# wearepal/qBOLD-VI

Measured on AMD Instinct MI355X. Metric: voxel-ELBO evals/sec, higher is better.
Workload: dtype f32; 1 GPU; 1048576 synthetic voxels/GPU x 11 tau, S=32 likelihood draws, K=70 KL draws, encoder U=60, L=2 (optimal.yaml), fused qbold_vi_fwd, tissue integral: table; encoder arithmetic: operands split in two f16 halves, three MFMA passes (hi.hi, hi.lo, lo.hi), f32 accumulate: float32-grade (~22 significant bits), |x| < 65504; sampling, forward model and ELBO sums: f32; global_voxels=1048576, parallelism=voxel-shard x1, collective=none

## Files before the change

### include/qbold_hip.h

```cpp
#ifndef QBOLD_HIP_H
#define QBOLD_HIP_H

#include <stdint.h>

#ifdef __cplusplus
extern "C" {
#endif

#define QBOLD_MAX_T 64
#define QBOLD_ABI_VERSION 5

typedef enum {
    QBOLD_OK = 0,
    QBOLD_ERR_INVALID = -1,
    QBOLD_ERR_HIP = -2,
    QBOLD_ERR_UNSUPPORTED = -3,
    QBOLD_ERR_NO_DEVICE = -4
} qbold_status;

typedef struct {
    double gamma, b0, dchi, te, r2t, tr, ti, t1b, hct;
    double tau_start, tau_end, tau_step;
    int32_t full_model;
    int32_t include_blood;
// ... 73 lines not shown
#define QBOLD_KSEL_ALL (4 | 8 | 256 | 512 | 2048 | 4096 | 8192 | 16384 | 32768 | 65536 | 131072 | 262144 | 524288 | 1048576 | 2097152 | 4194304 | 8388608)
int qbold_ctx_set_kernel_selection(qbold_ctx* ctx, int mask);
int qbold_ctx_table_eval(const qbold_ctx* ctx, const float* host_x, float* host_F, float* host_dF,
                         int64_t n);

int qbold_signal_fwd(const qbold_ctx* ctx, const float* oef_dbv, float* signal, int64_t V,
                     void* stream);
int qbold_signal_fwd_ex(const qbold_ctx* ctx, const float* oef_dbv, const float* hct,
                        const float* alt_oef_dbv, const int32_t* from_index, float* signal, int64_t V,
                        void* stream);
int qbold_signal_bwd(const qbold_ctx* ctx, const float* oef_dbv, const float* grad_signal,
                     float* grad_oef_dbv, int64_t V, void* stream);

int64_t qbold_encoder_num_params(const qbold_encoder_shape* shape);
int64_t qbold_encoder_packed_floats(const qbold_encoder_shape* shape);
int qbold_encoder_pack(const qbold_ctx* ctx, const qbold_encoder_shape* shape,
                       const float* weights, float* packed, void* stream);
int qbold_encoder_fwd(const qbold_ctx* ctx, const qbold_encoder_shape* shape, const float* packed,
                      const float* x, float* out1, float* out2, float* sigma, int64_t N,
                      void* stream);

int64_t qbold_encoder_wide_packed_floats(const qbold_encoder_shape* shape);
int64_t qbold_encoder_wide_workspace_floats(const qbold_encoder_shape* shape, int64_t N);
int qbold_encoder_wide_pack(const qbold_ctx* ctx, const qbold_encoder_shape* shape, const float* weights,
                            float* packed, void* stream);
int qbold_encoder_wide_fwd(const qbold_ctx* ctx, const qbold_encoder_shape* shape, const float* packed,
                           const float* x, int stream_sel, float* workspace, float* out_q,
                           float* out_log_sigma, int64_t N, void* stream);

int64_t qbold_encoder_fused_packed_floats(const qbold_encoder_shape* shape);
int qbold_encoder_fused_pack(const qbold_ctx* ctx, const qbold_encoder_shape* shape, const float* weights,
                             float* packed, void* stream);
int qbold_encoder_fused_fwd(const qbold_ctx* ctx, const qbold_encoder_shape* shape, const float* packed,
                            const float* x, float* out_q, float* out_log_sigma, int64_t N, void* stream);

int qbold_reparam(const qbold_ctx* ctx, const float* q, const float* z, float* oef_dbv, int64_t N,
                  void* stream);
int qbold_logit_mvn_nlogp(const qbold_ctx* ctx, const float* y, const float* params, float* out,
                          int64_t N, void* stream);
int qbold_kl_mog(const qbold_ctx* ctx, const float* q, const float* comps, int M, const float* z, uint64_t seed,
                 int64_t voxel0, float* kl, int64_t N, void* stream);
int qbold_squared_whitened_residual(const float* obs, const float* mean, const float* oef_log_std,
                                    const float* dbv_log_std, const float* oef_dbv_cov, float* out, int64_t N,
                                    void* stream);
int qbold_posterior_moments(const qbold_ctx* ctx, const float* q, const float* z, int n_samples,
                            uint64_t seed, int64_t voxel0, float* means, float* vars, int64_t N,
                            void* stream);

int qbold_normalise(const qbold_ctx* ctx, const float* x, float* out, int64_t N, void* stream);

int qbold_wls_fit(const qbold_ctx* ctx, const float* signals, double tau_min, float* out, int64_t N,
                  void* stream);

typedef enum {
    QBOLD_TRANSFORM_STD = 0,
    QBOLD_TRANSFORM_OFFDIAG = 1,
    QBOLD_INV_TRANSFORM_STD = 2,
    QBOLD_FORWARD_TRANSFORM = 3,
    QBOLD_BACKWARDS_TRANSFORM = 4,
    QBOLD_BACKWARDS_TRANSFORM_LOGIT = 5,
    QBOLD_EXP = 6
} qbold_transform_op;
int qbold_transform(const qbold_ctx* ctx, int op, const float* in, float* out, int64_t n,
                    void* stream);

int qbold_nll_fwd(const qbold_ctx* ctx, const float* x, const float* mask, const float* pred,
                  const float* sigma, float* nll, int64_t N, int S, void* stream);

int qbold_kl_fwd(const qbold_ctx* ctx, const float* q, const float* prior, const float* zk, int K,
                 uint64_t seed, int64_t voxel0, float* kl, int64_t N, void* stream);
int qbold_kl_closed(const qbold_ctx* ctx, const float* q, const float* prior, float* kl, int64_t N,
                    void* stream);
int qbold_kl_diag(const qbold_ctx* ctx, const float* q, const float* prior, const float* mask, float* kl_v,
                  float* g_q, double* sums, void* workspace, int64_t N, void* stream);

int qbold_normals(const qbold_ctx* ctx, uint64_t seed, uint32_t stream_id, int64_t voxel0, int n,
                  float* z, int64_t N, void* stream);

int64_t qbold_noise_workspace_bytes(const qbold_ctx* ctx);
int qbold_signal_add_noise(const qbold_ctx* ctx, float* signal, const float* norm_snr_host,
                           float snr_lo, float snr_hi, uint64_t seed, int64_t voxel0,
                           void* workspace, int64_t V, void* stream);

int64_t qbold_elbo_workspace_bytes(const qbold_ctx* ctx);

int qbold_elbo_fwd(const qbold_ctx* ctx, const float* x, const float* mask, const float* q,
                   const float* prior, const float* sigma, const float* zs, const float* zk, int S,
                   int K, uint64_t seed, int64_t voxel0, float* nll_kl, double* sums,
                   void* workspace, int64_t N, void* stream);

int qbold_elbo_fwd_logsigma(const qbold_ctx* ctx, const float* x, const float* mask, const float* q,
                            const float* prior, const float* log_sigma, int S, int K, uint64_t seed, int64_t voxel0,
                            float* nll_kl, double* sums, void* workspace, int64_t N, void* stream);

int64_t qbold_vi_workspace_bytes(const qbold_ctx* ctx, const qbold_encoder_shape* shape, int64_t N);
int qbold_vi_fwd(const qbold_ctx* ctx, const qbold_encoder_shape* shape, const float* packed,
                 const float* x, const float* mask, const float* prior, int S, int K, uint64_t seed,
                 int64_t voxel0, float* q_out, float* nll_kl, double* sums, void* workspace,
                 int64_t N, void* stream);

#define QBOLD_IW_MAX_K (1 << 30)
int qbold_log_evidence_fwd(const qbold_ctx* ctx, const float* x, const float* mask, const float* q,
                           const float* prior, const float* sigma, const float* z, int K, uint64_t seed,
                           int64_t voxel0, float* out, float* is_means, double* sums, void* workspace,
                           int64_t N, void* stream);

int qbold_log_evidence_bwd(const qbold_ctx* ctx, const float* x, const float* mask, const float* q,
                           const float* prior, const float* log_sigma, const float* z, int K, uint64_t seed,
                           int64_t voxel0, float* g_q, float* g_log_sigma, float* out, double* sums,
                           void* workspace, int64_t N, void* stream);

int qbold_log_evidence_draws(const qbold_ctx* ctx, const float* x, const float* mask, const float* q,
                             const float* prior, const float* sigma, const float* z, int K, uint64_t seed,
                             int64_t voxel0, float* log_w, float* theta, int64_t N, void* stream);

#define QBOLD_PSIS_MIN_K 25
#define QBOLD_PSIS_MAX_K 1024
#define QBOLD_PSIS_MAX_C 8
int qbold_psis(const qbold_ctx* ctx, const float* log_w, const float* theta, int C, const float* mask, int K,
               float* out, float* means, float* weights, int64_t N, void* stream);

typedef struct {
    int optimizer;
    float lr, lr_final, beta1, beta2, eps;
} qbold_refine_cfg;
int qbold_refine_posterior(const qbold_ctx* ctx, const float* x, const float* mask, const float* q_in,
                           const float* prior, const float* sigma, const float* z, int steps, int S,
                           const qbold_refine_cfg* cfg, uint64_t seed, int64_t voxel0,
                           float* q_out, float* loss, int64_t N, void* stream);

int64_t qbold_refine_spatial_workspace_bytes(const qbold_ctx* ctx, const qbold_geometry* geom);
int qbold_refine_posterior_spatial(const qbold_ctx* ctx, const float* x, const float* mask, const float* q_in,
                                   const float* prior, const float* sigma, const float* z,
                                   const qbold_geometry* geom, float tv_weight, int steps, int S,
                                   const qbold_refine_cfg* cfg, uint64_t seed, int64_t voxel0,
                                   float* q_out, float* loss, void* workspace, void* stream);

typedef struct {
    int coarse, fine, locate, gh;
    float span, cut, level_lo, level_hi;
} qbold_grid_cfg;
#define QBOLD_GRID_OUT 17
int qbold_posterior_grid(const qbold_ctx* ctx, const float* x, const float* mask, const float* prior,
                         const float* sigma, const float* q, const qbold_grid_cfg* cfg, float* out, float* box,
                         double* sums, void* workspace, int64_t N, void* stream);

#define QBOLD_PPC_OUT 6
int qbold_posterior_predictive(const qbold_ctx* ctx, const float* x, const float* mask, const float* q,
                               const float* sigma, const float* z, int L, uint64_t seed, int64_t voxel0,
                               float* out, float* curves, double* sums, void* workspace, int64_t N, void* stream);

int qbold_elbo_bwd(const qbold_ctx* ctx, const float* x, const float* mask, const float* q,
                   const float* prior, const float* log_sigma, int S, int K, uint64_t seed,
                   int64_t voxel0, float* g_q, float* g_log_sigma, float* nll_kl, double* sums,
                   void* workspace, int64_t N, void* stream);

int64_t qbold_train_workspace_floats(const qbold_encoder_shape* shape, int64_t N);
int qbold_encoder_train_fwd(const qbold_ctx* ctx, const qbold_encoder_shape* shape, const float* weights,
                            const float* x, int stream_sel, float* workspace, float* out_q,
                            float* out_log_sigma, int64_t N, void* stream);
int qbold_encoder_train_fwd_fused(const qbold_ctx* ctx, const qbold_encoder_shape* shape, const float* packed,
                                  const float* x, int save_all, float* workspace, float* out_q,
                                  float* out_log_sigma, int64_t N, void* stream);
int qbold_encoder_train_bwd_recomputes(const qbold_ctx* ctx, const qbold_encoder_shape* shape, int64_t N);
int qbold_encoder_spatial_fwd(const qbold_ctx* ctx, const qbold_encoder_shape* shape, const float* weights,
                              const float* x, const qbold_geometry* geom, float* workspace, float* out_q,
// ... 26 lines not shown
```

### qbold_vi_amd/csrc/ctx.hip

```cpp
#include <math.h>
#include <stdlib.h>
#include <string.h>

#include <mutex>

#include "qbold_ctx.h"

namespace qb {
static thread_local std::string g_err;
void set_error(const std::string& msg) { g_err = msg; }
int hip_fail(hipError_t e, const char* what) {
    g_err = std::string(what) + ": " + hipGetErrorString(e);
    return QBOLD_ERR_HIP;
}
}

extern "C" int qbold_abi_version(void) { return QBOLD_ABI_VERSION; }
extern "C" const char* qbold_last_error(void) { return qb::g_err.c_str(); }

namespace {

struct Simpson {
    double u[QB_NNODE], w[QB_NNODE], pre[QB_NNODE];
    double h3;
// ... 154 lines not shown
        g[i] = simpson.dF(i * h) * h;
    }
    ctx->h_tab.resize(4 * QB_TAB_SEG);
    for (int i = 0; i < QB_TAB_SEG; ++i) {
        ctx->h_tab[4 * i + 0] = (float)f[i];
        ctx->h_tab[4 * i + 1] = (float)g[i];
        ctx->h_tab[4 * i + 2] = (float)(3.0 * (f[i + 1] - f[i]) - 2.0 * g[i] - g[i + 1]);
        ctx->h_tab[4 * i + 3] = (float)(2.0 * (f[i] - f[i + 1]) + g[i] + g[i + 1]);
    }

    {
        const int se = d.se_idx;
        const float tol = 4e-6f * fabsf(tstep);
        bool mirrors = se >= 0 && se < T && fabsf(d.taus[se]) <= tol;
        for (int j = 1; mirrors && se - j >= 0 && se + j < T; ++j) {
            const float ta = fabsf(d.taus[se - j]), tb = fabsf(d.taus[se + j]);
            const float ba = d.blood_B[se - j], bb = d.blood_B[se + j];
            mirrors = fabsf(ta - tb) <= tol && fabsf(ba - bb) <= 4e-6f * fmaxf(fabsf(ba), fabsf(bb));
        }
        ctx->grid_mirrors = mirrors;
    }

    {
        const int nseg = qb::gtab_segs(T), se = d.se_idx;
        const bool proto = (T == 11 && se == 2) || (T == 24 && se == 7) || (T == 64 && se == 12);
        if (nseg > 0 && proto && ctx->grid_mirrors && P->full_model) {
            const int J = qb::gtab_taus(T, se);
            ctx->h_gtab.resize((size_t)4 * J * nseg);
            const double hh = (double)QB_GT_OEF_RANGE / nseg;
            std::vector<double> gf(nseg + 1), gg(nseg + 1);
            for (int j = 1; j <= J; ++j) {
                const double tau = fabs((double)(se + j < T ? d.taus[se + j] : d.taus[se - j]));
                const double k = tau * (double)d.dw_coef;
                for (int i = 0; i <= nseg; ++i) {
                    const double oef = (double)QB_GT_OEF_MIN + hh * i;
                    gf[i] = simpson.F(k * oef);
                    gg[i] = simpson.dF(k * oef) * k * hh;
                }
                const double* cf[4] = {nullptr, nullptr, nullptr, nullptr};
                std::vector<double> c0(nseg), c1(nseg), c2(nseg), c3(nseg);
                for (int i = 0; i < nseg; ++i) {
                    c0[i] = gf[i];
                    c1[i] = gg[i];
                    c2[i] = 3.0 * (gf[i + 1] - gf[i]) - 2.0 * gg[i] - gg[i + 1];
                    c3[i] = 2.0 * (gf[i] - gf[i + 1]) + gg[i] + gg[i + 1];
                }
                cf[0] = c0.data(); cf[1] = c1.data(); cf[2] = c2.data(); cf[3] = c3.data();
                if (qb::gtab_paired(T, se)) {
                    const int p = (j - 1) / 2, m = (j - 1) & 1;
                    float* rowA = &ctx->h_gtab[(size_t)4 * (2 * p) * nseg];
                    float* rowB = &ctx->h_gtab[(size_t)4 * (2 * p + 1) * nseg];
                    for (int i = 0; i < nseg; ++i) {
                        rowA[4 * i + 0 + m] = (float)cf[0][i];
                        rowA[4 * i + 2 + m] = (float)cf[1][i];
                        rowB[4 * i + 0 + m] = (float)cf[2][i];
                        rowB[4 * i + 2 + m] = (float)cf[3][i];
                    }
                } else {
                    float* row = &ctx->h_gtab[(size_t)4 * (j - 1) * nseg];
                    for (int i = 0; i < nseg; ++i)
                        for (int q = 0; q < 4; ++q) row[4 * i + q] = (float)cf[q][i];
                }
            }
            ctx->gtab_ok = true;
        }
    }

    if (device < 0) {
        *out = ctx;
        return QBOLD_OK;
    }
    int prev_device = -1;
    (void)hipGetDevice(&prev_device);
    hipError_t e = hipSetDevice(device);
    if (e == hipSuccess) e = hipMalloc((void**)&ctx->d_tab, sizeof(float) * 4 * QB_TAB_SEG);
    if (e == hipSuccess)
        e = hipMemcpy(ctx->d_tab, ctx->h_tab.data(), sizeof(float) * 4 * QB_TAB_SEG,
                      hipMemcpyHostToDevice);
    if (e == hipSuccess && ctx->gtab_ok) {
        e = hipMalloc((void**)&ctx->d_gtab, sizeof(float) * ctx->h_gtab.size());
        if (e == hipSuccess)
            e = hipMemcpy(ctx->d_gtab, ctx->h_gtab.data(), sizeof(float) * ctx->h_gtab.size(), hipMemcpyHostToDevice);
    }
    if (e == hipSuccess) {
        hipDeviceProp_t prop;
        if (hipGetDeviceProperties(&prop, device) == hipSuccess && prop.multiProcessorCount > 0)
            ctx->num_cus = prop.multiProcessorCount;
    }
    if (prev_device >= 0 && prev_device != device) (void)hipSetDevice(prev_device);
    if (e != hipSuccess) {
        if (ctx->d_tab) (void)hipFree(ctx->d_tab);
        if (ctx->d_gtab) (void)hipFree(ctx->d_gtab);
        delete ctx;
        return qb::hip_fail(e, "qbold_ctx_create: device setup");
    }
    *out = ctx;
    return QBOLD_OK;
}

extern "C" void qbold_ctx_destroy(qbold_ctx* ctx) {
    if (!ctx) return;
    if (ctx->d_tab) (void)hipFree(ctx->d_tab);
    if (ctx->d_gtab) (void)hipFree(ctx->d_gtab);
    delete ctx;
}

extern "C" int qbold_ctx_num_taus(const qbold_ctx* ctx) { return ctx ? ctx->dev.T : QBOLD_ERR_INVALID; }
extern "C" int qbold_ctx_se_idx(const qbold_ctx* ctx) { return ctx ? ctx->dev.se_idx : QBOLD_ERR_INVALID; }

extern "C" int qbold_ctx_taus(const qbold_ctx* ctx, float* host_out) {
    QB_REQUIRE(ctx && host_out, "qbold_ctx_taus: null argument");
    memcpy(host_out, ctx->dev.taus, sizeof(float) * ctx->dev.T);
    return QBOLD_OK;
}

extern "C" int qbold_ctx_set_tissue_mode(qbold_ctx* ctx, int mode) {
    QB_REQUIRE(ctx, "qbold_ctx_set_tissue_mode: null ctx");
    QB_REQUIRE(mode == QBOLD_TISSUE_TABLE || mode == QBOLD_TISSUE_LITERAL,
               "qbold_ctx_set_tissue_mode: unknown mode");
    ctx->dev.tissue_mode = mode;
    return QBOLD_OK;
}
extern "C" int qbold_ctx_set_grad_node0(qbold_ctx* ctx, int on) {
    QB_REQUIRE(ctx, "qbold_ctx_set_grad_node0: null ctx");
    ctx->dev.dF_node0 = on ? ctx->dF_node0_ref : 0.0f;
    return QBOLD_OK;
}
extern "C" int qbold_ctx_set_kernel_selection(qbold_ctx* ctx, int mask) {
    QB_REQUIRE(ctx, "qbold_ctx_set_kernel_selection: null ctx");
    QB_REQUIRE((mask & ~QBOLD_KSEL_ALL) == 0, "qbold_ctx_set_kernel_selection: unknown bit");
    ctx->kernel_sel = mask;
    return QBOLD_OK;
}
extern "C" int qbold_ctx_tissue_mode(const qbold_ctx* ctx) {
    return ctx ? ctx->dev.tissue_mode : QBOLD_ERR_INVALID;
}

extern "C" int qbold_ctx_table_eval(const qbold_ctx* ctx, const float* hx, float* hF, float* hdF,
                                    int64_t n) {
    QB_REQUIRE(ctx && hx && hF, "qbold_ctx_table_eval: null argument");
    const QbDev& c = ctx->dev;
    for (int64_t k = 0; k < n; ++k) {
        float ax = fabsf(hx[k]);
        if (ax > c.tab_xmax) ax = c.tab_xmax;
        float u = ax * c.tab_inv_h;
        int i = (int)u;
        if (i > QB_TAB_SEG - 1) i = QB_TAB_SEG - 1;
        float f = u - (float)i;
        const float* q = &ctx->h_tab[4 * i];
        hF[k] = fmaf(fmaf(fmaf(q[3], f, q[2]), f, q[1]), f, q[0]);
        if (hdF) {
            float dd = fmaf(fmaf(3.0f * q[3], f, 2.0f * q[2]), f, q[1]) * c.tab_inv_h + c.dF_node0 * ax;
            hdF[k] = hx[k] < 0 ? -dd : dd;
        }
    }
    return QBOLD_OK;
}
```

### qbold_vi_amd/csrc/elbo_bwd_kernels.hip

```cpp
#include "elbo_core.h"
#include "qbold_ctx.h"
#ifndef QB_BWD_WHITENED
#define QB_BWD_WHITENED 1
#endif

namespace qb {
bool elbo_fast_path(const qbold_ctx* ctx);
int elbo_grid(const qbold_ctx* ctx);
}

namespace {

constexpr int kBlock = 256;

struct FwdGrad {
    float s, ds_doef, ds_ddbv;
};

__device__ __forceinline__ FwdGrad fwd_signal_grad(const qb::FwdLds* L, const QbDev& c,
                                                   const qb::FwdFast& v, float oef, float dbv, int t) {
    const float us = fmaf((float)t, v.ub, v.ua);
    const float u = fabsf(us);
    const int i = min((int)u, QB_TAB_SEG - 1);
    const float f = u - (float)i;
    const float4 k = L->tab[i];
    const float F = fmaf(fmaf(fmaf(k.w, f, k.z), f, k.y), f, k.x);
    const float ax = u * (1.0f / c.tab_inv_h);
    const float dF = fmaf(fmaf(3.0f * k.w, f, 2.0f * k.z), f, k.y) * c.tab_inv_h + c.dF_node0 * ax;
    const float e1 = qb::exp2f_(v.nd * F);
    const float e2 = qb::exp2f_(v.ng * c.blood_B[t]);
    const float tissue = v.tissue_w * e1, blood = v.blood_w * e2;
    FwdGrad g;
    g.s = tissue + blood;
    const float inv_oef = qb::rcpf_(oef);
    g.ds_doef = -dbv * dF * ax * inv_oef * tissue +
                (2.0f * QB_LN2) * v.ng * c.blood_B[t] * inv_oef * blood;
    const float dbw = c.include_blood ? c.m_bld_nb : 1.0f;
    g.ds_ddbv = -F * tissue - dbw * c.e_te_r2t * e1 + (c.include_blood ? dbw * c.e_r2b_te * e2 : 0.0f);
    return g;
}

template <int T, int SE, int LPV>
__global__ __launch_bounds__(kBlock) void elbo_bwd_kernel(
    QbDev c, const float4* __restrict__ g_tab, const float* __restrict__ x,
    const float* __restrict__ mask, const float* __restrict__ q, const float* __restrict__ prior,
    const float* __restrict__ log_sigma, int S, int K, uint64_t seed, int64_t voxel0,
    float* __restrict__ g_q, float* __restrict__ g_ls, float2* __restrict__ nll_kl,
    double* __restrict__ partials, int64_t N) {
    __shared__ qb::FwdLds L;
    __shared__ double red[3 * (kBlock / 64)];
    qb::fwd_lds_fill(&L, g_tab, false);
    __syncthreads();

    constexpr int kVoxPerBlock = kBlock / LPV, kVoxPerWave = 64 / LPV;
    const int lane = threadIdx.x & 63, wave = threadIdx.x >> 6;
    const int part = LPV == 1 ? 0 : lane >> 4;
    auto voxel_sum = [](float x) { return LPV == 1 ? x : qb::voxel_sum(x); };
    float s_nll = 0.0f, s_kl = 0.0f, s_m = 0.0f;
    const int64_t ntile = (N + kVoxPerBlock - 1) / kVoxPerBlock;
    for (int64_t tile = blockIdx.x; tile < ntile; tile += gridDim.x) {
        const int64_t v = tile * kVoxPerBlock + wave * kVoxPerWave + (LPV == 1 ? lane : lane & 15);
        if (v < N) {
            float xv[T], lsv[T], qv[5], pv[5];
#pragma unroll
            for (int t = 0; t < T; ++t) {
                xv[t] = x[v * T + t];
                lsv[t] = log_sigma[v * T + t];
            }
#pragma unroll
            for (int i = 0; i < 5; ++i) {
                qv[i] = q[v * 5 + i];
                pv[i] = prior[v * 5 + i];
            }
            const float m = mask ? mask[v] : 1.0f;
            qb::VoxelLik<T> lik;
            qb::prepare_lik<T, SE, true>(c, xv, lsv, m, lik);
            const qb::LogitMvn qm = qb::make_mvn(qv), pm = qb::make_mvn(pv);
            const uint64_t vox = (uint64_t)(voxel0 + v);

            float g_mu_o = 0.0f, g_so = 0.0f, g_mu_d = 0.0f, g_sd = 0.0f, g_c = 0.0f;
            float gls[T];
#pragma unroll
            for (int t = 0; t < T; ++t) gls[t] = 0.0f;
            float nll_sum = 0.0f, kl_sum = 0.0f;
            int n_lik = 0, n_kl = 0;

            for (int g = part; 4 * g < S; g += LPV) {
                const int cnt = S - 4 * g < 4 ? S - 4 * g : 4;
                n_lik += cnt;
                qb::DrawQuad dq;
                dq.load(seed, vox, (uint32_t)g, qb::STREAM_LIK);
#pragma unroll 1
                for (int d = 0; d < cnt; ++d) {
                    float z0, z1;
                    dq.next(z0, z1);
                    float a, b;
                    qb::reparam_logits(qm, z0, z1, a, b);
                    const float sa = qb::sigmoidf_(a), sb = qb::sigmoidf_(b);
                    const float oef = sa * QB_OEF_RANGE + QB_MIN_OEF;
                    const float dbv = sb * QB_DBV_RANGE + QB_MIN_DBV;
                    const qb::FwdFast fv = qb::fwd_fast(c, oef, dbv);
                    float sig[T];
#pragma unroll
                    for (int t = 0; t < T; ++t) sig[t] = qb::fwd_signal_fast(&L, c, fv, t);
                    const float inv_np = qb::rcpf_(qb::se_norm<T, SE>(c, sig));
                    float acc = 0.0f, a1 = 0.0f;
                    float gy[T];
#pragma unroll
                    for (int t = 0; t < T; ++t) {
                        float yp = sig[t] * inv_np, dyp = 1.0f;
                        if (c.predict_log) {
                            dyp = m > 0.0f ? qb::rcpf_(yp) : 0.0f;
                            yp = m > 0.0f ? __logf(yp) : 0.0f;
                        }
                        const float r = (lik.yt[t] - yp) * lik.inv_s[t];
                        float dr = r;
                        if (c.use_student_t) {
                            const float w = (c.st_df + 1.0f) * qb::rcpf_(fmaf(r, r, c.st_df));
                            acc += (c.st_df + 1.0f) * log1pf(r * r * qb::rcpf_(c.st_df)) - 2.0f * c.st_const;
                            dr = w * r;
                        } else {
                            acc = fmaf(r, r, acc);
                        }
                        gls[t] += 1.0f - dr * r;
                        gy[t] = -dr * lik.inv_s[t] * dyp;
                        a1 = fmaf(gy[t], sig[t], a1);
                    }
                    nll_sum += acc;
                    a1 *= inv_np * inv_np;
                    float g_oef = 0.0f, g_dbv = 0.0f;
#pragma unroll
// ... 54 lines not shown
                const float nk = (float)n_kl;
                const float dmu_o = qm.mu_o - pm.mu_o, dmu_d = qm.mu_d - pm.mu_d;
                const float d0 = dmu_o * pm.i_so, m00 = qm.e_so * pm.i_so;
                const float d1 = fmaf(dmu_d, pm.i_sd, dmu_o * pm.i_bl);
                const float m10 = fmaf(qm.c, pm.i_sd, qm.e_so * pm.i_bl), m11 = qm.e_sd * pm.i_sd;
                const float sw0 = nk * d0 * d0 + 2.0f * d0 * m00 * s0 + m00 * m00 * s00;
                const float sw1 = nk * d1 * d1 + 2.0f * d1 * (m10 * s0 + m11 * s1) + m10 * m10 * s00 +
                                  2.0f * m10 * m11 * s01 + m11 * m11 * s11;
                kl_sum = (sw0 + sw1) - (s00 + s11);
                const float A0 = d0 * pm.i_so + d1 * pm.i_bl;
                const float A1 = m00 * pm.i_so + m10 * pm.i_bl - qm.i_so;
                const float A2 = m11 * pm.i_bl - qm.i_bl;
                const float B0 = d1 * pm.i_sd, B1 = m10 * pm.i_sd, B2 = m11 * pm.i_sd - qm.i_sd;
                k_mu_o = A0 * nk + A1 * s0 + A2 * s1;
                k_so = (A0 * s0 + A1 * s00 + A2 * s01) * qm.e_so;
                k_mu_d = B0 * nk + B1 * s0 + B2 * s1;
                k_c = B0 * s0 + B1 * s00 + B2 * s01;
                k_sd = (B0 * s1 + B1 * s01 + B2 * s11) * qm.e_sd;
            } else
            for (int g = part; 4 * g < K; g += LPV) {
                const int cnt = K - 4 * g < 4 ? K - 4 * g : 4;
                n_kl += cnt;
                qb::DrawQuad dq;
                dq.load(seed, vox, (uint32_t)g, qb::STREAM_KL);
#pragma unroll 1
                for (int d = 0; d < cnt; ++d) {
                    float z0, z1;
                    dq.next(z0, z1);
                    float a, b;
                    qb::reparam_logits(qm, z0, z1, a, b);
                    const float l0 = qb::clampf_(a, -QB_LOGIT_CLIP, QB_LOGIT_CLIP);
                    const float l1 = qb::clampf_(b, -QB_LOGIT_CLIP, QB_LOGIT_CLIP);
                    const float rq0 = l0 - qm.mu_o, rq1 = l1 - qm.mu_d;
                    const float rp0 = l0 - pm.mu_o, rp1 = l1 - pm.mu_d;
                    const float wq0 = rq0 * qm.i_so, wq1 = fmaf(rq1, qm.i_sd, rq0 * qm.i_bl);
                    const float wp0 = rp0 * pm.i_so, wp1 = fmaf(rp1, pm.i_sd, rp0 * pm.i_bl);
                    kl_sum += fmaf(wp0, wp0, wp1 * wp1) - fmaf(wq0, wq0, wq1 * wq1);
                    const float ga = (wp0 * pm.i_so + wp1 * pm.i_bl) - (wq0 * qm.i_so + wq1 * qm.i_bl);
                    const float gb = wp1 * pm.i_sd - wq1 * qm.i_sd;
                    k_mu_o += ga;
                    k_so = fmaf(ga, z0 * qm.e_so, k_so);
                    k_mu_d += gb;
                    k_c = fmaf(gb, z0, k_c);
                    k_sd = fmaf(gb, z1 * qm.e_sd, k_sd);
                }
            }
            kl_sum = fmaf(0.5f, kl_sum, (float)n_kl * ((pm.s_o + pm.s_d) - (qm.s_o + qm.s_d)));
            if (K > 0) {
                const float wk = (m > 0.0f ? 1.0f : 0.0f) / (float)K;
                g_mu_o = fmaf(wk, k_mu_o, g_mu_o);
                g_so = fmaf(wk, k_so, g_so);
                g_mu_d = fmaf(wk, k_mu_d, g_mu_d);
                g_sd = fmaf(wk, k_sd, g_sd);
                g_c = fmaf(wk, k_c, g_c);
            }
            g_mu_o = voxel_sum(g_mu_o);
            g_so = voxel_sum(g_so);
            g_mu_d = voxel_sum(g_mu_d);
            g_sd = voxel_sum(g_sd);
            g_c = voxel_sum(g_c);
#pragma unroll
            for (int t = 0; t < T; ++t) gls[t] = voxel_sum(gls[t]);
            const float nll = voxel_sum(nll_sum) * inv_S;
            const float kl = K > 0 ? voxel_sum(kl_sum) / (float)K : 0.0f;
            if (part == 0) {
                const float th1 = (qm.s_o + 1.0f) * (1.0f / 3.0f), th3 = (qm.s_d + 1.0f) * (1.0f / 3.0f);
                const float th4 = qm.c * 7.38905609893065f;
                g_q[v * 5 + 0] = g_mu_o;
                g_q[v * 5 + 1] = g_so * 3.0f * (1.0f - th1 * th1);
                g_q[v * 5 + 2] = g_mu_d;
                g_q[v * 5 + 3] = g_sd * 3.0f * (1.0f - th3 * th3);
                g_q[v * 5 + 4] = g_c * 0.1353352832366127f * (1.0f - th4 * th4);
                if (nll_kl) nll_kl[v] = make_float2(nll, kl);
                s_nll += nll * m;
                s_kl += m > 0.0f ? kl : 0.0f;
                s_m += m;
            }
            if (part == (LPV == 1 ? 0 : 1)) {
#pragma unroll
                for (int t = 0; t < T; ++t) g_ls[v * T + t] = gls[t];
            }
        }
    }
    qb::block_partials(red, s_nll, s_kl, s_m, partials);
}

constexpr int kGenBlock = 128;
constexpr int gen_rows(int lpv) { return lpv == 1 ? 2 : 3; }
static_assert(sizeof(qb::FwdLds) + sizeof(float) * gen_rows(QB_LANES_PER_VOXEL) * QB_MAX_T * kGenBlock <= 160 * 1024,
              "elbo_bwd_generic_kernel: table + rows exceed the LDS");

struct GenSig {
    float s, F, e1, e2, u, f, B;
    float4 k;
};
__device__ __forceinline__ GenSig gen_signal(const qb::FwdLds* L, const qb::FwdFast& v, int t) {
    GenSig g;
    g.u = fabsf(fmaf((float)t, v.ub, v.ua));
    const int i = (int)g.u;
    g.f = __builtin_amdgcn_fractf(g.u);
    g.k = L->tab[i];
    g.F = fmaf(fmaf(fmaf(g.k.w, g.f, g.k.z), g.f, g.k.y), g.f, g.k.x);
    g.e1 = qb::exp2f_(v.nd * g.F);
    g.B = L->blood_B[t];
    g.e2 = qb::exp2f_(v.ng * g.B);
    g.s = fmaf(v.tissue_w, g.e1, v.blood_w * g.e2);
    return g;
}

template <int LPV>
__global__ __launch_bounds__(kGenBlock) void elbo_bwd_generic_kernel(
    QbDev c, const float4* __restrict__ g_tab, const float* __restrict__ x,
    const float* __restrict__ mask, const float* __restrict__ q, const float* __restrict__ prior,
    const float* __restrict__ log_sigma, int S, int K, int kl_per_wave, uint64_t seed, int64_t voxel0,
    float* __restrict__ g_q, float* __restrict__ g_ls, float2* __restrict__ nll_kl,
    double* __restrict__ partials, int64_t N) {
    extern __shared__ __align__(16) unsigned char smem[];
    qb::FwdLds* L = reinterpret_cast<qb::FwdLds*>(smem);
    __shared__ double red[3 * (kGenBlock / 64)];
    const int T = c.T, se = c.se_idx;
    float* yt = reinterpret_cast<float*>(smem + sizeof(qb::FwdLds)) + threadIdx.x;
    float* is = yt + T * kGenBlock;
    float* gl = is + T * kGenBlock;
    qb::fwd_lds_fill(L, g_tab, false);
    if (threadIdx.x < QB_MAX_T) L->blood_B[threadIdx.x] = c.blood_B[threadIdx.x];
    __syncthreads();

    constexpr int kVoxPerBlock = kGenBlock / LPV, kVoxPerWave = 64 / LPV;
    const int lane = threadIdx.x & 63, wave = threadIdx.x >> 6;
    const int part = LPV == 1 ? 0 : lane >> 4;
    auto voxel_sum = [](float x) { return LPV == 1 ? x : qb::voxel_sum(x); };
    const int w_lo = c.multi_norm ? se - 1 : se, w_hi = c.multi_norm ? se + 1 : se;
    const float w_se = c.multi_norm ? 1.0f / 3.0f : 1.0f;
    const float dbw = c.include_blood ? c.m_bld_nb : 1.0f;
    const float n0 = c.dF_node0 / (c.tab_inv_h * c.tab_inv_h);
    float s_nll = 0.0f, s_kl = 0.0f, s_m = 0.0f;
    const int64_t ntile = (N + kVoxPerBlock - 1) / kVoxPerBlock;
    for (int64_t tile = blockIdx.x; tile < ntile; tile += gridDim.x) {
        const int64_t v = tile * kVoxPerBlock + wave * kVoxPerWave + (LPV == 1 ? lane : lane & 15);
        if (v < N) {
            const float* xv = x + v * T;
            const float* lv = log_sigma + v * T;
            float qv[5], pv[5];
#pragma unroll
            for (int i = 0; i < 5; ++i) {
                qv[i] = q[v * 5 + i];
                pv[i] = prior[v * 5 + i];
            }
            const float m = mask ? mask[v] : 1.0f;
            const float nt = c.multi_norm ? (xv[se - 1] + xv[se] + xv[se + 1]) / 3.0f + 1e-3f : xv[se] + 1e-3f;
            const float inv_nt = qb::rcpf_(nt);
            float ls = 0.0f;
            for (int t = 0; t < T; ++t) {
                const float l = lv[t];
                yt[t * kGenBlock] = xv[t] * inv_nt;
                is[t * kGenBlock] = qb::exp2f_(-QB_LOG2E * l);
                if (LPV > 1) gl[t * kGenBlock] = 0.0f;
                ls += l;
            }
            const float log_s_sum = ls + (float)T * 0.9189385332046727f;
            const qb::LogitMvn qm = qb::make_mvn(qv), pm = qb::make_mvn(pv);
            const uint64_t vox = (uint64_t)(voxel0 + v);
            const float inv_S = 1.0f / (float)S;
            const float wn = m * inv_S;
            float* gv = g_ls + v * T;

            float g_mu_o = 0.0f, g_so = 0.0f, g_mu_d = 0.0f, g_sd = 0.0f, g_c = 0.0f;
            float nll_sum = 0.0f, kl_sum = 0.0f;
            int n_lik = 0, n_kl = 0;

            for (int g = part; 4 * g < S; g += LPV) {
                const int cnt = S - 4 * g < 4 ? S - 4 * g : 4;
                n_lik += cnt;
                qb::DrawQuad dq;
                dq.load(seed, vox, (uint32_t)g, qb::STREAM_LIK);
#pragma unroll 1
                for (int d = 0; d < cnt; ++d) {
                    float z0, z1;
                    dq.next(z0, z1);
                    float a, b;
                    qb::reparam_logits(qm, z0, z1, a, b);
                    const float sa = qb::sigmoidf_(a), sb = qb::sigmoidf_(b);
                    const float oef = sa * QB_OEF_RANGE + QB_MIN_OEF;
                    const float dbv = sb * QB_DBV_RANGE + QB_MIN_DBV;
                    const qb::FwdFast fv = qb::fwd_fast(c, oef, dbv);
                    const float inv_oef = qb::rcpf_(oef);
                    float np_ = gen_signal(L, fv, se).s;
                    if (c.multi_norm) np_ = (gen_signal(L, fv, se - 1).s + np_ + gen_signal(L, fv, se + 1).s) / 3.0f;
                    const float inv_np = qb::rcpf_(np_ + 1e-3f);
                    const float ko = -dbv * inv_oef, kb = (2.0f * QB_LN2) * fv.ng * inv_oef;
                    const float kd1 = dbw * c.e_te_r2t, kd2 = c.include_blood ? dbw * c.e_r2b_te : 0.0f;
                    float acc = 0.0f, a1 = 0.0f, go = 0.0f, gd = 0.0f, wo = 0.0f, wd = 0.0f;
                    for (int t = 0; t < T; ++t) {
                        const GenSig sg = gen_signal(L, fv, t);
                        const float inv_s = is[t * kGenBlock];
                        float r;
                        {
#pragma clang fp contract(off)
                            const float yp = sg.s * inv_np;
// ... 61 lines not shown
                const float nk = (float)n_kl;
                const float dmu_o = qm.mu_o - pm.mu_o, dmu_d = qm.mu_d - pm.mu_d;
                const float d0 = dmu_o * pm.i_so, m00 = qm.e_so * pm.i_so;
                const float d1 = fmaf(dmu_d, pm.i_sd, dmu_o * pm.i_bl);
                const float m10 = fmaf(qm.c, pm.i_sd, qm.e_so * pm.i_bl), m11 = qm.e_sd * pm.i_sd;
                const float sw0 = nk * d0 * d0 + 2.0f * d0 * m00 * s0 + m00 * m00 * s00;
                const float sw1 = nk * d1 * d1 + 2.0f * d1 * (m10 * s0 + m11 * s1) + m10 * m10 * s00 +
                                  2.0f * m10 * m11 * s01 + m11 * m11 * s11;
                kl_sum = (sw0 + sw1) - (s00 + s11);
                const float A0 = d0 * pm.i_so + d1 * pm.i_bl;
                const float A1 = m00 * pm.i_so + m10 * pm.i_bl - qm.i_so;
                const float A2 = m11 * pm.i_bl - qm.i_bl;
                const float B0 = d1 * pm.i_sd, B1 = m10 * pm.i_sd, B2 = m11 * pm.i_sd - qm.i_sd;
                k_mu_o = A0 * nk + A1 * s0 + A2 * s1;
                k_so = (A0 * s0 + A1 * s00 + A2 * s01) * qm.e_so;
                k_mu_d = B0 * nk + B1 * s0 + B2 * s1;
                k_c = B0 * s0 + B1 * s00 + B2 * s01;
                k_sd = (B0 * s1 + B1 * s01 + B2 * s11) * qm.e_sd;
            } else
            for (int g = part; 4 * g < K; g += LPV) {
                const int cnt = K - 4 * g < 4 ? K - 4 * g : 4;
                n_kl += cnt;
                qb::DrawQuad dq;
                dq.load(seed, vox, (uint32_t)g, qb::STREAM_KL);
#pragma unroll 1
                for (int d = 0; d < cnt; ++d) {
                    float z0, z1;
                    dq.next(z0, z1);
                    float a, b;
                    qb::reparam_logits(qm, z0, z1, a, b);
                    const float l0 = qb::clampf_(a, -QB_LOGIT_CLIP, QB_LOGIT_CLIP);
                    const float l1 = qb::clampf_(b, -QB_LOGIT_CLIP, QB_LOGIT_CLIP);
                    const float rq0 = l0 - qm.mu_o, rq1 = l1 - qm.mu_d;
                    const float rp0 = l0 - pm.mu_o, rp1 = l1 - pm.mu_d;
                    const float wq0 = rq0 * qm.i_so, wq1 = fmaf(rq1, qm.i_sd, rq0 * qm.i_bl);
                    const float wp0 = rp0 * pm.i_so, wp1 = fmaf(rp1, pm.i_sd, rp0 * pm.i_bl);
                    kl_sum += fmaf(wp0, wp0, wp1 * wp1) - fmaf(wq0, wq0, wq1 * wq1);
                    const float ga = (wp0 * pm.i_so + wp1 * pm.i_bl) - (wq0 * qm.i_so + wq1 * qm.i_bl);
                    const float gb = wp1 * pm.i_sd - wq1 * qm.i_sd;
                    k_mu_o += ga;
                    k_so = fmaf(ga, z0 * qm.e_so, k_so);
                    k_mu_d += gb;
                    k_c = fmaf(gb, z0, k_c);
                    k_sd = fmaf(gb, z1 * qm.e_sd, k_sd);
                }
            }
            kl_sum = fmaf(0.5f, kl_sum, (float)n_kl * ((pm.s_o + pm.s_d) - (qm.s_o + qm.s_d)));
            if (K > 0) {
                const float wk = (m > 0.0f ? 1.0f : 0.0f) / (float)K;
                g_mu_o = fmaf(wk, k_mu_o, g_mu_o);
                g_so = fmaf(wk, k_so, g_so);
                g_mu_d = fmaf(wk, k_mu_d, g_mu_d);
                g_sd = fmaf(wk, k_sd, g_sd);
                g_c = fmaf(wk, k_c, g_c);
            }
            g_mu_o = voxel_sum(g_mu_o);
            g_so = voxel_sum(g_so);
            g_mu_d = voxel_sum(g_mu_d);
            g_sd = voxel_sum(g_sd);
            g_c = voxel_sum(g_c);
            if (LPV > 1) {
                for (int t = 0; t < T; ++t) {
                    const float gt = voxel_sum(gl[t * kGenBlock] * wn);
                    if ((t & (LPV - 1)) == part) gv[t] = gt;
                }
            }
            const float nll = voxel_sum(nll_sum) * inv_S;
            const float kl = K > 0 ? voxel_sum(kl_sum) / (float)K : 0.0f;
            if (part == 0) {
                const float th1 = (qm.s_o + 1.0f) * (1.0f / 3.0f), th3 = (qm.s_d + 1.0f) * (1.0f / 3.0f);
                const float th4 = qm.c * 7.38905609893065f;
                g_q[v * 5 + 0] = g_mu_o;
                g_q[v * 5 + 1] = g_so * 3.0f * (1.0f - th1 * th1);
                g_q[v * 5 + 2] = g_mu_d;
                g_q[v * 5 + 3] = g_sd * 3.0f * (1.0f - th3 * th3);
                g_q[v * 5 + 4] = g_c * 0.1353352832366127f * (1.0f - th4 * th4);
                if (nll_kl) nll_kl[v] = make_float2(nll, kl);
                s_nll += nll * m;
                s_kl += m > 0.0f ? kl : 0.0f;
                s_m += m;
            }
        }
    }
    qb::block_partials(red, s_nll, s_kl, s_m, partials);
}

}

extern "C" int qbold_elbo_bwd(const qbold_ctx* ctx, const float* x, const float* mask, const float* q,
                              const float* prior, const float* log_sigma, int S, int K, uint64_t seed,
                              int64_t voxel0, float* g_q, float* g_log_sigma, float* nll_kl,
                              double* sums, void* workspace, int64_t N, void* stream) {
    QB_NEED_DEVICE(ctx);
    QB_REQUIRE(N >= 0 && S >= 1 && K >= 0, "qbold_elbo_bwd: need N >= 0, S >= 1, K >= 0");
    QB_REQUIRE(sums && workspace, "qbold_elbo_bwd: null sums/workspace");
    QB_REQUIRE(N == 0 || (x && q && prior && log_sigma && g_q && g_log_sigma),
               "qbold_elbo_bwd: null buffer");
    if (!(ctx->dev.full_model && ctx->dev.tissue_mode == QBOLD_TISSUE_TABLE)) {
        qb::set_error("qbold_elbo_bwd: gradients are built for the full signal model in table mode "
                      "(Gaussian or Student-t likelihood, linear or log data, either normalisation)");
        return QBOLD_ERR_UNSUPPORTED;
    }
    hipStream_t s = (hipStream_t)stream;
    double* partials = reinterpret_cast<double*>(workspace);
    const int lpv = S <= 2 ? 1 : QB_LANES_PER_VOXEL;
    const int vpb = kBlock / lpv;
    const int64_t ntile = (N + vpb - 1) / vpb;
    const int grid = (int)(ntile < qb::elbo_grid(ctx) ? (ntile > 0 ? ntile : 1) : qb::elbo_grid(ctx));
    float2* out = reinterpret_cast<float2*>(nll_kl);
    const bool spec_T = ctx->dev.T == 11 || ctx->dev.T == 24;
    if (!spec_T && !qb::elbo_fast_path(ctx)) {
        qb::set_error("qbold_elbo_bwd: for T other than 11 / 24 only the optimal.yaml configuration (table mode, "
                      "Gaussian likelihood, linear data) is built");
        return QBOLD_ERR_UNSUPPORTED;
    }
    if (!spec_T || ((ctx->kernel_sel & QBOLD_KSEL_ELBO_BWD_GENERIC) && qb::elbo_fast_path(ctx))) {
        const int T = ctx->dev.T;
        QB_REQUIRE(T >= 1 && T <= QB_MAX_T, "qbold_elbo_bwd: need 1 <= T <= 64");
        const int gvpb = kGenBlock / lpv;
        const int64_t gtile = (N + gvpb - 1) / gvpb;
        const int ggrid = (int)(gtile < qb::elbo_grid(ctx) ? (gtile > 0 ? gtile : 1) : qb::elbo_grid(ctx));
        const size_t smem = sizeof(qb::FwdLds) + sizeof(float) * gen_rows(lpv) * (size_t)T * kGenBlock;
        auto kern = lpv == 1 ? elbo_bwd_generic_kernel<1> : elbo_bwd_generic_kernel<QB_LANES_PER_VOXEL>;
        if (smem > 64 * 1024)
            QB_HIP(hipFuncSetAttribute(reinterpret_cast<const void*>(kern), hipFuncAttributeMaxDynamicSharedMemorySize,
                                       (int)smem));
        hipLaunchKernelGGL(kern, dim3(ggrid), dim3(kGenBlock), smem, s, ctx->dev, ctx->d_tab, x, mask, q, prior, log_sigma,
                           S, K, spec_T ? 1 : 0, seed, voxel0, g_q, g_log_sigma, out, partials, N);
        QB_HIP(hipGetLastError());
        hipLaunchKernelGGL(qb::reduce_partials_kernel, dim3(1), dim3(192), 0, s, partials, ggrid, sums);
        QB_HIP(hipGetLastError());
        return QBOLD_OK;
    }
#define QB_LAUNCH_BWD(TT, SEC)                                                                                          \
    do {                                                                                                                \
        if (lpv == 1)                                                                                                   \
            hipLaunchKernelGGL((elbo_bwd_kernel<TT, SEC, 1>), dim3(grid), dim3(kBlock), 0, s, ctx->dev, ctx->d_tab, x,   \
                               mask, q, prior, log_sigma, S, K, seed, voxel0, g_q, g_log_sigma, out, partials, N);      \
        else                                                                                                            \
            hipLaunchKernelGGL((elbo_bwd_kernel<TT, SEC, QB_LANES_PER_VOXEL>), dim3(grid), dim3(kBlock), 0, s, ctx->dev, \
                               ctx->d_tab, x, mask, q, prior, log_sigma, S, K, seed, voxel0, g_q, g_log_sigma, out,     \
                               partials, N);                                                                            \
    } while (0)
    if (ctx->dev.T == 24) {
        QB_LAUNCH_BWD(24, -1);
    } else if (ctx->dev.T != 11) {
        qb::set_error("qbold_elbo_bwd: kernels are built for T = 11 or 24 taus");
        return QBOLD_ERR_UNSUPPORTED;
    } else if (ctx->dev.se_idx == 2 && !ctx->dev.multi_norm) {
        QB_LAUNCH_BWD(11, 2);
    } else {
        QB_LAUNCH_BWD(11, -1);
    }
#undef QB_LAUNCH_BWD
    QB_HIP(hipGetLastError());
    hipLaunchKernelGGL(qb::reduce_partials_kernel, dim3(1), dim3(192), 0, s, partials, grid, sums);
    QB_HIP(hipGetLastError());
    return QBOLD_OK;
}
```

### qbold_vi_amd/csrc/elbo_core.h

```cpp
#pragma once
#ifndef QB_PRIO_LIK
#define QB_PRIO_LIK 1
#endif
#ifndef QB_LIK_BARRIER
#define QB_LIK_BARRIER 2
#endif
#ifndef QB_GT_DEPTH
#define QB_GT_DEPTH 8
#endif
#ifndef QB_GT_DEPTH_LONG
#define QB_GT_DEPTH_LONG 2
#endif
#ifndef QB_X_DEPTH
#define QB_X_DEPTH 2
#endif
#ifndef QB_PRIO_KL
#define QB_PRIO_KL 2
#endif
#ifndef QB_PRIO_AFTER
#define QB_PRIO_AFTER 0
#endif

#include "qbold_dev.h"

// ... 372 lines not shown
                    dq.load(seed, vox, g, STREAM_LIK);
                    g += QB_LANES_PER_VOXEL;
                }
                dq.next(z0, z1);
            }
            float a, b, oef = 0.0f, dbv = 0.0f;
            reparam_logits(q, z0, z1, a, b);
            if constexpr (!(FAST && IsGtLds<LDS>::value)) forward_transform(a, b, oef, dbv);
            if constexpr (FAST && IsGtLds<LDS>::value) {
                static_assert(!IsGtLds<LDS>::value || MIR, "the per-tau table scores merged mirror pairs");
                nll_sum += sample_sq_fast<T, SE>(L, c, lik, sigmoidf_(a), sigmoidf_(b));
            } else if constexpr (FAST) {
                nll_sum += sample_sq_fast<T, SE, MIR>(L, c, lik, oef, dbv);
            } else {
                nll_sum += sample_nll<T, SE, LITERAL>(L, c, lik, oef, dbv);
            }
        }
    }
    if (FAST) {
        nll_sum = fmaf(0.5f, nll_sum, (float)n_lik * lik.log_s_sum);
    }
    float pv[5];
#pragma unroll
    for (int k = 0; k < 5; ++k) pv[k] = prior_row[k];
    const LogitMvn prior = make_mvn(pv);
    __builtin_amdgcn_s_setprio(QB_PRIO_KL);
    if constexpr (FAST) {
        LogitMvn qk;
        qk.mu_o = q.mu_o; qk.mu_d = q.mu_d; qk.c = q.c; qk.e_so = q.e_so; qk.e_sd = q.e_sd;
        qk.s_o = q_s_sum; qk.s_d = 0.0f;
        qk.i_so = rcpf_(q.e_so);
        qk.i_sd = rcpf_(q.e_sd);
        qk.i_bl = -(qk.i_so * qk.i_sd) * q.c;
        kl_sum = kl_draws_fast(qk, prior, K, zk, seed, vox, part, n_kl);
    } else {
        for (int j = part; 2 * j < K; j += QB_LANES_PER_VOXEL) {
            float z[4];
            const bool two = 2 * j + 1 < K;
            n_kl += two ? 2 : 1;
            if (zk) {
                z[0] = zk[4 * j];
                z[1] = zk[4 * j + 1];
                z[2] = two ? zk[4 * j + 2] : 0.0f;
                z[3] = two ? zk[4 * j + 3] : 0.0f;
            } else {
                normals4(seed, vox, (uint32_t)j, STREAM_KL, z);
            }
#pragma unroll
            for (int d = 0; d < 2; ++d) {
                if (d == 1 && !two) break;
                float a, b, oef, dbv;
                reparam_logits(q, z[2 * d], z[2 * d + 1], a, b);
                forward_transform(a, b, oef, dbv);
                const LogitObs o = make_obs(oef, dbv);
                kl_sum += nlogp(o, prior) - nlogp(o, q);
            }
        }
    }
    __builtin_amdgcn_s_setprio(QB_PRIO_AFTER);
    if (FAST) {
        kl_sum = fmaf(0.5f, kl_sum, (float)n_kl * ((prior.s_o + prior.s_d) - q_s_sum));
    }
}

__device__ __forceinline__ void block_partials(double* red, float s_nll, float s_kl, float s_m,
                                               double* __restrict__ partials) {
    const int lane = threadIdx.x & 63, wave = threadIdx.x >> 6, nw = blockDim.x >> 6;
    s_nll = wave_sum(s_nll);
    s_kl = wave_sum(s_kl);
    s_m = wave_sum(s_m);
    if (lane == 0) {
        red[3 * wave + 0] = (double)s_nll;
        red[3 * wave + 1] = (double)s_kl;
        red[3 * wave + 2] = (double)s_m;
    }
    __syncthreads();
    if (threadIdx.x < 3) {
        double a = 0.0;
        for (int w = 0; w < nw; ++w) a += red[3 * w + threadIdx.x];
        partials[3 * blockIdx.x + threadIdx.x] = a;
    }
}

static __global__ void reduce_partials_kernel(const double* __restrict__ partials, int nblocks,
                                       double* __restrict__ sums) {
    __shared__ double sh[192];
    const int k = threadIdx.x / 64, lane = threadIdx.x & 63;
    double a = 0.0;
    for (int b = lane; b < nblocks; b += 64) a += partials[3 * b + k];
    sh[threadIdx.x] = a;
    __syncthreads();
    if (lane == 0) {
        double t = 0.0;
        for (int i = 0; i < 64; ++i) t += sh[64 * k + i];
        sums[k] = t;
    }
}

}
```

### qbold_vi_amd/csrc/elbo_kernels.hip

```cpp
#include <cmath>

#include "elbo_core.h"
#include "qbold_ctx.h"

namespace {

constexpr int kBlock = 256;
constexpr int kVoxPerBlock = kBlock / QB_LANES_PER_VOXEL;

template <int T, int SE, bool GT>
struct ElboLds { using type = qb::FwdLds; };
template <int T, int SE>
struct ElboLds<T, SE, true> { using type = qb::GtLds<T, SE>; };

template <int T, int SE, bool FAST, bool LITERAL, bool GT = false, bool MIR = false>
__global__ __launch_bounds__(kBlock) void elbo_fwd_kernel(
    QbDev c, const float4* __restrict__ g_tab, const float* __restrict__ x,
    const float* __restrict__ mask, const float* __restrict__ q, const float* __restrict__ prior,
    const float* __restrict__ sigma, const float* __restrict__ zs, const float* __restrict__ zk,
    int S, int K, uint64_t seed, int64_t voxel0, float2* __restrict__ nll_kl,
    double* __restrict__ partials, int64_t N) {
    static_assert(!GT || (FAST && SE >= 0 && qb::gtab_segs(T) > 0), "GT needs the fast path with a compile-time spin echo");
    static_assert(!MIR || (FAST && SE >= 0), "merged mirror pairs: fast path with a compile-time spin echo");
    constexpr bool kMir = GT || MIR;
    using Lds = typename ElboLds<T, SE, GT>::type;
    __shared__ Lds L;
    __shared__ double red[3 * (kBlock / 64)];
    if constexpr (qb::IsGtLds<Lds>::value) {
        qb::gt_lds_fill(&L, g_tab, c);
    } else {
        qb::fwd_lds_fill(&L, g_tab, true);
        if (threadIdx.x < QB_MAX_T) L.blood_B[threadIdx.x] = c.blood_B[threadIdx.x];
    }
    __syncthreads();

    const int lane = threadIdx.x & 63, wave = threadIdx.x >> 6;
    const int part = lane >> 4;
    float s_nll = 0.0f, s_kl = 0.0f, s_m = 0.0f;
    const int64_t ntile = (N + kVoxPerBlock - 1) / kVoxPerBlock;
    for (int64_t tile = blockIdx.x; tile < ntile; tile += gridDim.x) {
        const int64_t v = tile * kVoxPerBlock + wave * QB_VOX_PER_WAVE + (lane & 15);
        if (v < N) {
            float xv[T], sv[T], qv[5];
#pragma unroll
            for (int t = 0; t < T; ++t) {
                xv[t] = x[v * T + t];
                sv[t] = sigma[v * T + t];
            }
#pragma unroll
            for (int i = 0; i < 5; ++i) qv[i] = q[v * 5 + i];
            const float m = mask ? mask[v] : 1.0f;
            qb::VoxelLik<T> lik;
            qb::prepare_lik<T, SE, false, (FAST && SE >= 0), FAST, kMir>(c, xv, sv, m, lik);
            const qb::LogitMvn qm = qb::make_mvn(qv);
            float nll_part, kl_part;
            qb::voxel_mc_sums<T, SE, FAST, LITERAL, kMir>(&L, c, lik, qm, prior + v * 5, S, K, zs ? zs + v * S * 2 : nullptr,
                                          zk ? zk + v * K * 2 : nullptr, seed,
                                          (uint64_t)(voxel0 + v), part, nll_part, kl_part);
            const float nll = qb::voxel_sum(nll_part) / (float)S;
            const float kl = K > 0 ? qb::voxel_sum(kl_part) / (float)K : 0.0f;
            if (part == 0) {
                if (nll_kl) nll_kl[v] = make_float2(nll, kl);
                s_nll += nll * m;
                s_kl += m > 0.0f ? kl : 0.0f;
                s_m += m;
            }
        }
    }
    qb::block_partials(red, s_nll, s_kl, s_m, partials);
}

constexpr int kGenBlock = 128;
constexpr int kGenVox = kGenBlock / QB_LANES_PER_VOXEL;

__device__ __forceinline__ double wave_sum_d(double v) {
#pragma unroll
    for (int o = 32; o > 0; o >>= 1) v += __shfl_xor(v, o, 64);
    return v;
}
__device__ __forceinline__ void block_partials_d(double* red, double a, double b, double m,
                                                 double* __restrict__ partials) {
    const int lane = threadIdx.x & 63, wave = threadIdx.x >> 6, nw = blockDim.x >> 6;
    a = wave_sum_d(a);
    b = wave_sum_d(b);
    m = wave_sum_d(m);
    if (lane == 0) {
        red[3 * wave + 0] = a;
        red[3 * wave + 1] = b;
        red[3 * wave + 2] = m;
    }
    __syncthreads();
    if (threadIdx.x < 3) {
        double acc = 0.0;
        for (int w = 0; w < nw; ++w) acc += red[3 * w + threadIdx.x];
        partials[3 * blockIdx.x + threadIdx.x] = acc;
    }
}

__global__ __launch_bounds__(kGenBlock) void elbo_fwd_generic_kernel(
    QbDev c, const float4* __restrict__ g_tab, const float* __restrict__ x,
    const float* __restrict__ mask, const float* __restrict__ q, const float* __restrict__ prior,
    const float* __restrict__ sigma, const float* __restrict__ zs, const float* __restrict__ zk,
    int S, int K, uint64_t seed, int64_t voxel0, float2* __restrict__ nll_kl,
    double* __restrict__ partials, int64_t N) {
    extern __shared__ __align__(16) unsigned char smem[];
    qb::FwdLds* L = reinterpret_cast<qb::FwdLds*>(smem);
    float* yt = reinterpret_cast<float*>(smem + sizeof(qb::FwdLds));
    float* is = yt + QB_MAX_T * kGenVox;
    __shared__ double red[3 * (kGenBlock / 64)];
    qb::fwd_lds_fill(L, g_tab, false);
    if (threadIdx.x < QB_MAX_T) L->blood_B[threadIdx.x] = c.blood_B[threadIdx.x];
    __syncthreads();

    const int T = c.T, se = c.se_idx;
    const bool mirrored = !c.multi_norm && fmaf((float)se, c.tauh_step, c.tauh0) == 0.0f;
    const int lane = threadIdx.x & 63, wave = threadIdx.x >> 6;
    const int part = lane >> 4;
    const int vl = wave * QB_VOX_PER_WAVE + (lane & 15);
    double s_nll = 0.0, s_kl = 0.0, s_m = 0.0;
    const int64_t ntile = (N + kGenVox - 1) / kGenVox;
    for (int64_t tile = blockIdx.x; tile < ntile; tile += gridDim.x) {
        const int64_t v = tile * kGenVox + vl;
        const bool live = v < N;
        const int64_t vc = live ? v : N - 1;
        const float* xv = x + vc * T;
        const float* sv = sigma + vc * T;
        const float nt = c.multi_norm ? (xv[se - 1] + xv[se] + xv[se + 1]) / 3.0f + 1e-3f : xv[se] + 1e-3f;
        const float inv_nt = qb::rcpf_(nt);
        float ls = 0.0f;
        __syncthreads();
        for (int t = part; t < T; t += QB_LANES_PER_VOXEL) {
            yt[t * kGenVox + vl] = xv[t] * inv_nt;
            is[t * kGenVox + vl] = qb::rcpf_(sv[t]);
            ls += QB_LN2 * qb::log2f_(sv[t]);
        }
        const float log_s_sum = qb::voxel_sum(ls) + (float)T * 0.9189385332046727f;
        __syncthreads();
        if (live) {
            float qv[5];
#pragma unroll
            for (int i = 0; i < 5; ++i) qv[i] = q[v * 5 + i];
            const float m = mask ? mask[v] : 1.0f;
            const qb::LogitMvn qm = qb::make_mvn(qv);
            const uint64_t vox = (uint64_t)(voxel0 + v);
            const float* zsv = zs ? zs + v * S * 2 : nullptr;
            const float* zkv = zk ? zk + v * K * 2 : nullptr;
            float nll_sum = 0.0f, kl_sum = 0.0f;
            int n_lik = 0, n_kl = 0;
            for (int g = part; 4 * g < S; g += QB_LANES_PER_VOXEL) {
                const int cnt = S - 4 * g < 4 ? S - 4 * g : 4;
                n_lik += cnt;
                qb::DrawQuad dq;
                if (!zsv) dq.load(seed, vox, (uint32_t)g, qb::STREAM_LIK);
#pragma unroll 1
                for (int d = 0; d < cnt; ++d) {
                    float z0, z1;
                    if (zsv) {
                        z0 = zsv[2 * (4 * g + d)];
                        z1 = zsv[2 * (4 * g + d) + 1];
                    } else {
                        dq.next(z0, z1);
                    }
                    float a, b, oef, dbv;
                    qb::reparam_logits(qm, z0, z1, a, b);
                    qb::forward_transform(a, b, oef, dbv);
                    const qb::FwdFast fv = qb::fwd_fast(c, oef, dbv);
                    if (mirrored) {
                        const float s_se = fmaf(fv.tissue_w, 1.0f, fv.blood_w * qb::exp2f_(fv.ng * L->blood_B[se]));
                        const float inv_np = qb::rcpf_(s_se + 1e-3f);
                        const float lt = qb::log2f_(fv.tissue_w * inv_np), lb = qb::log2f_(fv.blood_w * inv_np);
                        auto signal = [&](int t) {
                            const float u = fabsf(fmaf((float)t, fv.ub, fv.ua));
                            const float4 kk = L->tab[(int)u];
                            const float f = __builtin_amdgcn_fractf(u);
                            const float F = fmaf(fmaf(fmaf(kk.w, f, kk.z), f, kk.y), f, kk.x);
                            return qb::exp2f_(fmaf(fv.nd, F, lt)) + qb::exp2f_(fmaf(fv.ng, L->blood_B[t], lb));
                        };
                        float acc = 0.0f;
                        auto residual = [&](int t, float yh) {
                            const float r = (yt[t * kGenVox + vl] - yh) * is[t * kGenVox + vl];
                            acc = fmaf(r, r, acc);
                        };
                        residual(se, s_se * inv_np);
                        for (int t = se + 1; t < T; ++t) {
                            const float yh = signal(t);
                            residual(t, yh);
                            if (2 * se - t >= 0) residual(2 * se - t, yh);
                        }
                        for (int t = 0; t < 2 * se - (T - 1); ++t) residual(t, signal(t));
                        nll_sum += acc;
                        continue;
                    }
                    float np_ = qb::fwd_signal_fast(L, c, fv, se);
                    if (c.multi_norm)
                        np_ = (np_ + qb::fwd_signal_fast(L, c, fv, se - 1) + qb::fwd_signal_fast(L, c, fv, se + 1)) / 3.0f;
                    const float inv_np = qb::rcpf_(np_ + 1e-3f);
                    float acc = 0.0f;
                    for (int t = 0; t < T; ++t) {
                        const float st = qb::fwd_signal_fast(L, c, fv, t);
                        const float r = fmaf(-st, inv_np, yt[t * kGenVox + vl]) * is[t * kGenVox + vl];
                        acc = fmaf(r, r, acc);
                    }
                    nll_sum += acc;
                }
            }
            nll_sum = fmaf(0.5f, nll_sum, (float)n_lik * log_s_sum);
            float pv[5];
#pragma unroll
            for (int i = 0; i < 5; ++i) pv[i] = prior[v * 5 + i];
            const qb::LogitMvn pm = qb::make_mvn(pv);
            kl_sum = qb::kl_draws_fast(qm, pm, K, zkv, seed, vox, part, n_kl);
            kl_sum = fmaf(0.5f, kl_sum, (float)n_kl * ((pm.s_o + pm.s_d) - (qm.s_o + qm.s_d)));
            const float nll = qb::voxel_sum(nll_sum) / (float)S;
            const float kl = K > 0 ? qb::voxel_sum(kl_sum) / (float)K : 0.0f;
            if (part == 0) {
                if (nll_kl) nll_kl[v] = make_float2(nll, kl);
                s_nll += (double)nll * (double)m;
                s_kl += m > 0.0f ? (double)kl : 0.0;
                s_m += (double)m;
            }
        }
    }
    block_partials_d(red, s_nll, s_kl, s_m, partials);
}

#ifndef QB_LDS_PIPE
#define QB_LDS_PIPE 1
#endif
#ifndef QB_LDS_DEPTH
#define QB_LDS_DEPTH 2
#endif
constexpr int kLdsBlock = 256;
constexpr int kLdsVox = kLdsBlock / QB_LANES_PER_VOXEL;

template <int T, int SE, bool LOGSIG>
__global__ __launch_bounds__(kLdsBlock) void elbo_fwd_lds_kernel(
    QbDev c, const float4* __restrict__ g_tab, const float* __restrict__ x,
    const float* __restrict__ mask, const float* __restrict__ q, const float* __restrict__ prior,
    const float* __restrict__ sigma, const float* __restrict__ zs, const float* __restrict__ zk,
    int S, int K, uint64_t seed, int64_t voxel0, float2* __restrict__ nll_kl,
    double* __restrict__ partials, int64_t N) {
    static_assert(T % 16 == 0 && SE >= 0 && SE < T, "a lane owns T / 4 taus as float4 loads");
    __shared__ qb::FwdLds L;
    __shared__ float2 dat[T * kLdsVox];
    __shared__ double red[3 * (kLdsBlock / 64)];
    qb::fwd_lds_fill(&L, g_tab, false);
    if (threadIdx.x < QB_MAX_T) L.blood_B[threadIdx.x] = c.blood_B[threadIdx.x];

    const int lane = threadIdx.x & 63, wave = threadIdx.x >> 6;
    const int part = lane >> 4;
    const int vl = wave * QB_VOX_PER_WAVE + (lane & 15);
    float2* my = dat + vl;
    float s_nll = 0.0f, s_kl = 0.0f, s_m = 0.0f;
    const int64_t ntile = (N + kLdsVox - 1) / kLdsVox;
    for (int64_t tile = blockIdx.x; tile < ntile; tile += gridDim.x) {
        const int64_t v = tile * kLdsVox + vl;
        const bool live = v < N;
        const int64_t vc = live ? v : N - 1;
        const float4* xq = reinterpret_cast<const float4*>(x + vc * T) + (T / 16) * part;
        const float4* sq = reinterpret_cast<const float4*>(sigma + vc * T) + (T / 16) * part;
        const float inv_nt = qb::rcpf_(x[vc * T + SE] + 1e-3f);
        float ls = 0.0f;
        __syncthreads();
#pragma unroll
        for (int k4 = 0; k4 < T / 16; ++k4) {
            const float4 xx = xq[k4], ss = sq[k4];
            const float xa[4] = {xx.x, xx.y, xx.z, xx.w}, sa[4] = {ss.x, ss.y, ss.z, ss.w};
#pragma unroll
            for (int e = 0; e < 4; ++e) {
                float is;
                if (LOGSIG) {
                    is = qb::exp2f_(-QB_LOG2E * sa[e]);
                    ls += sa[e];
                } else {
                    is = qb::rcpf_(sa[e]);
                    ls += QB_LN2 * qb::log2f_(sa[e]);
                }
                my[((T / 4) * part + 4 * k4 + e) * kLdsVox] = make_float2(xa[e] * inv_nt * is, is);
            }
        }
        __syncthreads();
        float dsum = 0.0f;
#pragma unroll
        for (int j = 1; j <= SE && SE + j < T; ++j) {
            if (((j - 1) & 3) == part) {
                const float2 p1 = my[(SE + j) * kLdsVox], p2 = my[(SE - j) * kLdsVox];
                const float pp = fmaf(p1.y, p1.y, p2.y * p2.y);
                const float ip = __builtin_amdgcn_rsqf(pp);
                const float cr = fmaf(p1.x, p2.y, -(p2.x * p1.y)) * ip;
                my[(SE + j) * kLdsVox] = make_float2(fmaf(p1.x, p1.y, p2.x * p2.y) * ip, pp * ip);
                dsum = fmaf(cr, cr, dsum);
            }
        }
        const float log_s_sum = qb::voxel_sum(fmaf(0.5f, dsum, ls)) + (float)T * 0.9189385332046727f;
        __syncthreads();
        if (live) {
            float qv[5];
#pragma unroll
            for (int i = 0; i < 5; ++i) qv[i] = q[v * 5 + i];
            const float m = mask ? mask[v] : 1.0f;
            const qb::LogitMvn qm = qb::make_mvn(qv);
            const uint64_t vox = (uint64_t)(voxel0 + v);
            const float* zsv = zs ? zs + v * S * 2 : nullptr;
            const float* zkv = zk ? zk + v * K * 2 : nullptr;
            float nll_sum = 0.0f, kl_sum = 0.0f;
            int n_lik = 0, n_kl = 0;
            __builtin_amdgcn_s_setprio(QB_PRIO_LIK);
            for (int g = part; 4 * g < S; g += QB_LANES_PER_VOXEL) {
                const int cnt = S - 4 * g < 4 ? S - 4 * g : 4;
                n_lik += cnt;
                qb::DrawQuad dq;
                if (!zsv) dq.load(seed, vox, (uint32_t)g, qb::STREAM_LIK);
#pragma unroll 1
                for (int d = 0; d < cnt; ++d) {
                    float z0, z1;
                    if (zsv) {
                        z0 = zsv[2 * (4 * g + d)];
                        z1 = zsv[2 * (4 * g + d) + 1];
                    } else {
                        dq.next(z0, z1);
                    }
                    float a, b, oef, dbv;
                    qb::reparam_logits(qm, z0, z1, a, b);
                    qb::forward_transform(a, b, oef, dbv);
// ... 5 lines not shown
#if QB_LDS_PIPE
                    struct Stage {
                        float4 kk;
                        float f, bb;
                        float2 d0;
                    };
                    auto issue = [&](int t) -> Stage {
                        Stage st;
                        const float u = fabsf(fmaf((float)t, fv.ub, fv.ua));
                        st.kk = L.tab[(int)u];
                        st.f = __builtin_amdgcn_fractf(u);
                        st.bb = L.blood_B[t];
                        st.d0 = my[t * kLdsVox];
                        return st;
                    };
                    auto finish = [&](int t, const Stage& st) {
                        const float F = fmaf(fmaf(fmaf(st.kk.w, st.f, st.kk.z), st.f, st.kk.y), st.f, st.kk.x);
                        const float yh = qb::exp2f_(fmaf(fv.nd, F, lt)) + qb::exp2f_(fmaf(fv.ng, st.bb, lb));
                        const float r = fmaf(-yh, st.d0.y, st.d0.x);
                        acc = fmaf(r, r, acc);
                    };
                    {
                        const float2 dd = my[SE * kLdsVox];
                        const float r = fmaf(-(s_se * inv_np), dd.y, dd.x);
                        acc = fmaf(r, r, acc);
                    }
                    static_assert(2 * SE - (T - 1) <= 0, "the pipelined form covers protocols whose taus below the "
                                                         "spin echo all have a mirror partner");
                    constexpr int D = QB_LDS_DEPTH;
                    Stage ring[D + 1];
#pragma unroll
                    for (int k = 0; k < D; ++k) ring[k] = issue(SE + 1 + k);
#pragma unroll
                    for (int t = SE + 1; t < T; ++t) {
                        if (t + D < T) ring[(t - SE - 1 + D) % (D + 1)] = issue(t + D);
                        __builtin_amdgcn_sched_barrier(0);
                        finish(t, ring[(t - SE - 1) % (D + 1)]);
                        __builtin_amdgcn_sched_barrier(0);
                    }
#else
                    auto signal = [&](int t) -> float {
                        const float u = fabsf(fmaf((float)t, fv.ub, fv.ua));
                        const float4 kk = L.tab[(int)u];
                        const float f = __builtin_amdgcn_fractf(u);
                        const float F = fmaf(fmaf(fmaf(kk.w, f, kk.z), f, kk.y), f, kk.x);
                        return qb::exp2f_(fmaf(fv.nd, F, lt)) + qb::exp2f_(fmaf(fv.ng, L.blood_B[t], lb));
                    };
                    auto residual = [&](int t, float yh) {
                        const float2 dd = my[t * kLdsVox];
                        const float r = fmaf(-yh, dd.y, dd.x);
                        acc = fmaf(r, r, acc);
                    };
                    residual(SE, s_se * inv_np);
#pragma unroll
                    for (int t = SE + 1; t < T; ++t) {
                        residual(t, signal(t));
                        if (((t - SE) % QB_LIK_BARRIER) == 0) asm volatile("" ::: "memory");
                    }
#pragma unroll
                    for (int t = 0; t < 2 * SE - (T - 1); ++t) residual(t, signal(t));
#endif
                    nll_sum += acc;
                }
            }
            nll_sum = fmaf(0.5f, nll_sum, (float)n_lik * log_s_sum);
            float pv[5];
#pragma unroll
            for (int i = 0; i < 5; ++i) pv[i] = prior[v * 5 + i];
            const qb::LogitMvn pm = qb::make_mvn(pv);
            __builtin_amdgcn_s_setprio(QB_PRIO_KL);
            kl_sum = qb::kl_draws_fast(qm, pm, K, zkv, seed, vox, part, n_kl);
            __builtin_amdgcn_s_setprio(QB_PRIO_AFTER);
            kl_sum = fmaf(0.5f, kl_sum, (float)n_kl * ((pm.s_o + pm.s_d) - (qm.s_o + qm.s_d)));
            const float nll = qb::voxel_sum(nll_sum) / (float)S;
            const float kl = K > 0 ? qb::voxel_sum(kl_sum) / (float)K : 0.0f;
            if (part == 0) {
                if (nll_kl) nll_kl[v] = make_float2(nll, kl);
                s_nll += nll * m;
                s_kl += m > 0.0f ? kl : 0.0f;
                s_m += m;
            }
        }
    }
    qb::block_partials(red, s_nll, s_kl, s_m, partials);
}

constexpr int kGtBlock = 1024;
constexpr int kGtVox = kGtBlock / QB_LANES_PER_VOXEL;

template <int T, int SE, bool LOGSIG>
__global__ __launch_bounds__(kGtBlock) void elbo_fwd_gt64_kernel(
    QbDev c, const float4* __restrict__ g_gtab, const float* __restrict__ x,
    const float* __restrict__ mask, const float* __restrict__ q, const float* __restrict__ prior,
    const float* __restrict__ sigma, int S, int K, uint64_t seed, int64_t voxel0, float2* __restrict__ nll_kl,
    double* __restrict__ partials, int64_t N) {
    static_assert(T == 64 && SE == 12, "lane ownership of the taus below is written out for the 64-tau protocol");
    constexpr int NSEG = qb::gtab_segs(T), J = qb::gtab_taus(T, SE), NROW = T - SE;
    static_assert(J == NROW - 1 && NSEG > 0, "one table row set per evaluated tau above the spin echo");
    extern __shared__ __align__(16) unsigned char smem[];
    float4* gtab = reinterpret_cast<float4*>(smem);
    float* bloodB = reinterpret_cast<float*>(smem + sizeof(float4) * J * NSEG);
    float2* dat = reinterpret_cast<float2*>(smem + sizeof(float4) * J * NSEG + sizeof(float) * T);
    double* red = reinterpret_cast<double*>(smem + sizeof(float4) * J * NSEG + sizeof(float) * T +
                                            sizeof(float2) * NROW * kGtVox);
    for (int i = threadIdx.x; i < J * NSEG; i += kGtBlock) gtab[i] = g_gtab[i];
    if (threadIdx.x < T) bloodB[threadIdx.x] = c.blood_B[threadIdx.x];

    const int lane = threadIdx.x & 63, wave = threadIdx.x >> 6;
    const int part = lane >> 4;
    const int vl = wave * QB_VOX_PER_WAVE + (lane & 15);
    float2* my = dat + vl;
    float s_nll = 0.0f, s_kl = 0.0f, s_m = 0.0f;
    const int64_t ntile = (N + kGtVox - 1) / kGtVox;
    for (int64_t tile = blockIdx.x; tile < ntile; tile += gridDim.x) {
        const int64_t v = tile * kGtVox + vl;
        const bool live = v < N;
        const int64_t vc = live ? v : N - 1;
        const float inv_nt = qb::rcpf_(x[vc * T + SE] + 1e-3f);
        float a[16], sg[16], ls = 0.0f;
        {
            const float4* xq = reinterpret_cast<const float4*>(x + vc * T) + 4 * part;
            const float4* sq = reinterpret_cast<const float4*>(sigma + vc * T) + 4 * part;
#pragma unroll
            for (int k4 = 0; k4 < 4; ++k4) {
                const float4 xx = xq[k4], ss = sq[k4];
                const float xa[4] = {xx.x, xx.y, xx.z, xx.w}, sa[4] = {ss.x, ss.y, ss.z, ss.w};
#pragma unroll
                for (int e = 0; e < 4; ++e) {
                    float is;
                    if (LOGSIG) {
                        is = qb::exp2f_(-QB_LOG2E * sa[e]);
                        ls += sa[e];
                    } else {
                        is = qb::rcpf_(sa[e]);
                        ls += QB_LN2 * qb::log2f_(sa[e]);
                    }
                    a[4 * k4 + e] = xa[e] * inv_nt * is;
                    sg[4 * k4 + e] = is;
                }
            }
        }
        float am[9], sm[9];
        if (part == 1) {
#pragma unroll
            for (int t = 0; t < 9; ++t) {
                const float sv = sigma[vc * T + t];
                const float is = LOGSIG ? qb::exp2f_(-QB_LOG2E * sv) : qb::rcpf_(sv);
                am[t] = x[vc * T + t] * inv_nt * is;
                sm[t] = is;
            }
        }
        __syncthreads();
        float dsum = 0.0f;
        auto merged = [&](float a1, float s1, float a2, float s2) {
            const float pp = fmaf(s1, s1, s2 * s2);
            const float ip = __builtin_amdgcn_rsqf(pp);
            const float cr = fmaf(a1, s2, -(a2 * s1)) * ip;
            dsum = fmaf(cr, cr, dsum);
            return make_float2(fmaf(a1, s1, a2 * s2) * ip, pp * ip);
        };
        if (part == 0) {
            my[0 * kGtVox] = make_float2(a[12], sg[12]);
#pragma unroll
            for (int j = 1; j <= 3; ++j) my[j * kGtVox] = merged(a[12 + j], sg[12 + j], a[12 - j], sg[12 - j]);
        } else if (part == 1) {
#pragma unroll
            for (int k = 0; k < 16; ++k) {
                const int t = 16 + k;
                my[(t - SE) * kGtVox] = t <= 2 * SE ? merged(a[k], sg[k], am[2 * SE - t >= 0 && 2 * SE - t < 9 ? 2 * SE - t : 0],
                                                             sm[2 * SE - t >= 0 && 2 * SE - t < 9 ? 2 * SE - t : 0])
                                                    : make_float2(a[k], sg[k]);
            }
        } else {
#pragma unroll
            for (int k = 0; k < 16; ++k) my[(16 * part + k - SE) * kGtVox] = make_float2(a[k], sg[k]);
        }
        const float log_s_sum = qb::voxel_sum(fmaf(0.5f, dsum, ls)) + (float)T * 0.9189385332046727f;
        __syncthreads();
// ... 7 lines not shown
            int n_kl = 0;
            __builtin_amdgcn_s_setprio(QB_PRIO_LIK);
            const int calls = S > 4 * part ? (S - 4 * part + 15) / 16 : 0;
            const int last = calls > 0 ? S - 4 * (part + 4 * (calls - 1)) : 0;
            const int n_lik = calls > 0 ? 4 * (calls - 1) + (last < 4 ? last : 4) : 0;
            qb::DrawQuad dq;
            uint32_t g = (uint32_t)part;
#pragma unroll 1
            for (int i = 0; i < n_lik; ++i) {
                if ((i & 3) == 0) {
                    dq.load(seed, vox, g, qb::STREAM_LIK);
                    g += QB_LANES_PER_VOXEL;
                }
                float z0, z1, la, lb_;
                dq.next(z0, z1);
                qb::reparam_logits(qm, z0, z1, la, lb_);
                const float sa = qb::sigmoidf_(la), sb = qb::sigmoidf_(lb_);
                const qb::FwdFast fv = qb::fwd_fast_sig(c, sa, sb);
                const float s_se = fmaf(fv.tissue_w, 1.0f, fv.blood_w * qb::exp2f_(fv.ng * bloodB[SE]));
                const float inv_np = qb::rcpf_(s_se + 1e-3f);
                const float lt = qb::log2f_(fv.tissue_w * inv_np), lb = qb::log2f_(fv.blood_w * inv_np);
                const float cg = fminf(sa * (float)NSEG, (float)NSEG - 0.0009765625f);
                const float f = __builtin_amdgcn_fractf(cg);
                const float4* row = gtab + (int)cg;
                float acc;
                {
                    const float2 dd = my[0];
                    const float r = fmaf(-(s_se * inv_np), dd.y, dd.x);
                    acc = r * r;
                }
                struct Stage {
                    float4 kk;
                    float bb;
                    float2 d0;
                };
                auto issue = [&](int e) -> Stage {
                    Stage st;
                    st.kk = row[(e - 1) * NSEG];
                    st.bb = bloodB[SE + e];
                    st.d0 = my[e * kGtVox];
                    return st;
                };
                auto finish = [&](const Stage& st) {
                    const float F = fmaf(fmaf(fmaf(st.kk.w, f, st.kk.z), f, st.kk.y), f, st.kk.x);
                    const float yh = qb::exp2f_(fmaf(fv.nd, F, lt)) + qb::exp2f_(fmaf(fv.ng, st.bb, lb));
                    const float r = fmaf(-yh, st.d0.y, st.d0.x);
                    acc = fmaf(r, r, acc);
                };
                if (qb_phase_fence()) {
                    constexpr int D = QB_LDS_DEPTH;
                    Stage ring[D + 1];
#pragma unroll
                    for (int k = 0; k < D; ++k) ring[k] = issue(1 + k);
#pragma unroll
                    for (int e = 1; e < NROW; ++e) {
                        if (e + D < NROW) ring[(e - 1 + D) % (D + 1)] = issue(e + D);
                        __builtin_amdgcn_sched_barrier(0);
                        finish(ring[(e - 1) % (D + 1)]);
                        __builtin_amdgcn_sched_barrier(0);
                    }
                }
                nll_sum += acc;
            }
            nll_sum = fmaf(0.5f, nll_sum, (float)n_lik * log_s_sum);
            float pv[5];
#pragma unroll
            for (int i = 0; i < 5; ++i) pv[i] = prior[v * 5 + i];
            const qb::LogitMvn pm = qb::make_mvn(pv);
            __builtin_amdgcn_s_setprio(QB_PRIO_KL);
            kl_sum = qb::kl_draws_fast(qm, pm, K, nullptr, seed, vox, part, n_kl);
            __builtin_amdgcn_s_setprio(QB_PRIO_AFTER);
            kl_sum = fmaf(0.5f, kl_sum, (float)n_kl * ((pm.s_o + pm.s_d) - (qm.s_o + qm.s_d)));
            const float nll = qb::voxel_sum(nll_sum) / (float)S;
            const float kl = K > 0 ? qb::voxel_sum(kl_sum) / (float)K : 0.0f;
            if (part == 0) {
                const float m = mask ? mask[v] : 1.0f;
                if (nll_kl) nll_kl[v] = make_float2(nll, kl);
                s_nll += nll * m;
                s_kl += m > 0.0f ? kl : 0.0f;
                s_m += m;
            }
        }
    }
    qb::block_partials(red, s_nll, s_kl, s_m, partials);
}

__global__ void reparam_kernel(const float* __restrict__ q, const float2* __restrict__ z,
                               float2* __restrict__ out, int64_t N) {
    for (int64_t i = blockIdx.x * (int64_t)blockDim.x + threadIdx.x; i < N;
         i += (int64_t)gridDim.x * blockDim.x) {
        float p[5];
#pragma unroll
        for (int k = 0; k < 5; ++k) p[k] = q[i * 5 + k];
        const qb::LogitMvn m = qb::make_mvn(p);
        const float2 zz = z[i];
        float a, b, oef, dbv;
        qb::reparam_logits(m, zz.x, zz.y, a, b);
        qb::forward_transform(a, b, oef, dbv);
        out[i] = make_float2(oef, dbv);
    }
}

__global__ void nlogp_kernel(const float2* __restrict__ y, const float* __restrict__ params,
                             float* __restrict__ out, int64_t N) {
    for (int64_t i = blockIdx.x * (int64_t)blockDim.x + threadIdx.x; i < N;
         i += (int64_t)gridDim.x * blockDim.x) {
        float p[5];
#pragma unroll
        for (int k = 0; k < 5; ++k) p[k] = params[i * 5 + k];
        const qb::LogitMvn m = qb::make_mvn(p);
        const float2 yy = y[i];
        out[i] = qb::nlogp(qb::make_obs(yy.x, yy.y), m);
    }
}

__global__ void moments_kernel(QbDev c, const float* __restrict__ q, const float* __restrict__ z,
                               int n, uint64_t seed, int64_t voxel0, float* __restrict__ means,
                               float* __restrict__ vars, int64_t N) {
    for (int64_t i = blockIdx.x * (int64_t)blockDim.x + threadIdx.x; i < N;
         i += (int64_t)gridDim.x * blockDim.x) {
        float p[5];
#pragma unroll
        for (int k = 0; k < 5; ++k) p[k] = q[i * 5 + k];
        const qb::LogitMvn m = qb::make_mvn(p);
        const float* zi = z ? z + i * n * 2 : nullptr;
        float mo = 0.0f, md = 0.0f, mr = 0.0f, vo = 0.0f, vd = 0.0f, vr = 0.0f;
        for (int pass = 0; pass < 2; ++pass) {
            float ao = 0.0f, ad = 0.0f, ar = 0.0f;
            for (int j = 0; 2 * j < n; ++j) {
                float zz[4];
                const bool two = 2 * j + 1 < n;
                if (zi) {
                    zz[0] = zi[4 * j];
                    zz[1] = zi[4 * j + 1];
                    zz[2] = two ? zi[4 * j + 2] : 0.0f;
                    zz[3] = two ? zi[4 * j + 3] : 0.0f;
                } else {
                    qb::normals4(seed, (uint64_t)(voxel0 + i), (uint32_t)j, qb::STREAM_MOMENTS, zz);
                }
                for (int d = 0; d < (two ? 2 : 1); ++d) {
                    float a, b, oef, dbv;
                    qb::reparam_logits(m, zz[2 * d], zz[2 * d + 1], a, b);
                    qb::forward_transform(a, b, oef, dbv);
                    const float r2p = (c.dw_coef * oef) * dbv;
                    if (pass == 0) {
                        ao += oef;
                        ad += dbv;
                        ar += r2p;
                    } else {
                        ao += (oef - mo) * (oef - mo);
                        ad += (dbv - md) * (dbv - md);
                        ar += (r2p - mr) * (r2p - mr);
                    }
                }
            }
            const float inv = 1.0f / (float)n;
            if (pass == 0) {
                mo = ao * inv;
                md = ad * inv;
                mr = ar * inv;
                if (!vars) break;
            } else {
                vo = ao * inv;
                vd = ad * inv;
                vr = ar * inv;
            }
        }
// ... 37 lines not shown
                    qb::normals4(seed, (uint64_t)(voxel0 + i), (uint32_t)j, qb::STREAM_R2P, zz);
                }
                for (int d = 0; d < (two ? 2 : 1); ++d) {
                    const float z0 = zz[2 * d], z1 = zz[2 * d + 1];
                    float a, b, oef, dbv;
                    qb::reparam_logits(m, z0, z1, a, b);
                    qb::forward_transform(a, b, oef, dbv);
                    const float r = (c.dw_coef * oef) * dbv;
                    if (pass == 0) {
                        acc += r;
                    } else if (pass == 1) {
                        acc += (r - mean) * (r - mean);
                    } else {
                        const float gr = A + B * (r - mean);
                        const float uo = oef - QB_MIN_OEF, ud = dbv - QB_MIN_DBV;
                        const float da = gr * c.dw_coef * dbv * uo * (1.0f - uo * (1.0f / QB_OEF_RANGE));
                        const float db = gr * c.dw_coef * oef * ud * (1.0f - ud * (1.0f / QB_DBV_RANGE));
                        G[0] += da;
                        G[1] += da * z0 * m.e_so;
                        G[2] += db;
                        G[3] += db * z1 * m.e_sd;
                        G[4] += db * z0;
                    }
                }
            }
            if (pass == 0) {
                mean = acc * inv_n;
            } else if (pass == 1) {
                var = acc * inv_n;
                const float iv = 1.0f / var, dy = y - mean;
                A = -dy * iv * inv_n;
                B = (1.0f - dy * dy * iv) * iv * inv_n;
                if (loss_v) loss_v[i] += 0.5f * __logf(var) + 0.5f * dy * dy * iv;
                if (!g_q) break;
            }
        }
        if (g_q) {
            const float th1 = (m.s_o + 1.0f) * (1.0f / 3.0f), th3 = (m.s_d + 1.0f) * (1.0f / 3.0f);
            const float th4 = m.c * 7.38905609893065f;
            float* g = g_q + i * 5;
            g[0] += scale * G[0];
            g[1] += scale * G[1] * 3.0f * (1.0f - th1 * th1);
            g[2] += scale * G[2];
            g[3] += scale * G[3] * 3.0f * (1.0f - th3 * th3);
            g[4] += scale * G[4] * 0.1353352832366127f * (1.0f - th4 * th4);
        }
    }
}

int ew_grid(const qbold_ctx* ctx, int64_t N, int block) {
    int64_t nb = (N + block - 1) / block;
    int64_t cap = (int64_t)ctx->num_cus * 8;
    return (int)(nb < cap ? (nb > 0 ? nb : 1) : cap);
}

}

namespace qb {
int elbo_grid(const qbold_ctx* ctx) { return ctx->num_cus * 4; }
bool elbo_fast_path(const qbold_ctx* ctx) {
    const QbDev& d = ctx->dev;
    return d.full_model && d.tissue_mode == QBOLD_TISSUE_TABLE && !d.predict_log && !d.use_student_t;
}
}

extern "C" int64_t qbold_elbo_workspace_bytes(const qbold_ctx* ctx) {
    if (!ctx) return QBOLD_ERR_INVALID;
    return (int64_t)sizeof(double) * 3 * (int64_t)qb::elbo_grid(ctx);
}

namespace qb {
bool elbo_logsigma_path(const qbold_ctx* ctx) {
    return ctx->dev.T == 64 && elbo_fast_path(ctx) && ctx->dev.se_idx == 12 && !ctx->dev.multi_norm &&
           !(ctx->kernel_sel & 4) && std::fabs(std::fmaf(12.0f, ctx->dev.tauh_step, ctx->dev.tauh0)) < 1e-6f;
}
}

namespace qb {
int elbo_fwd_launch(const qbold_ctx* ctx, const float* x, const float* mask, const float* q,
                    const float* prior, const float* sigma, bool sigma_is_log, const float* zs,
                    const float* zk, int S, int K, uint64_t seed, int64_t voxel0, float* nll_kl,
                    double* sums, void* workspace, int64_t N, hipStream_t s) {
    double* partials = reinterpret_cast<double*>(workspace);
    const int64_t ntile = (N + kVoxPerBlock - 1) / kVoxPerBlock;
    int grid = (int)(ntile < qb::elbo_grid(ctx) ? (ntile > 0 ? ntile : 1) : qb::elbo_grid(ctx));
    const bool lit = ctx->dev.tissue_mode == QBOLD_TISSUE_LITERAL;
    float2* out = reinterpret_cast<float2*>(nll_kl);
#define QB_LAUNCH_ELBO(TT, SE, FAST, LIT)                                                        \
    hipLaunchKernelGGL((elbo_fwd_kernel<TT, SE, FAST, LIT>), dim3(grid), dim3(kBlock), 0, s,      \
                       ctx->dev, ctx->d_tab, x, mask, q, prior, sigma, zs, zk, S, K, seed, voxel0, \
                       out, partials, N)
#define QB_LAUNCH_ELBO_MIR(TT, SE)                                                               \
    hipLaunchKernelGGL((elbo_fwd_kernel<TT, SE, true, false, false, true>), dim3(grid), dim3(kBlock), 0, s, \
                       ctx->dev, ctx->d_tab, x, mask, q, prior, sigma, zs, zk, S, K, seed, voxel0, \
                       out, partials, N)
#define QB_LAUNCH_ELBO_GT(TT, SE)                                                                \
    hipLaunchKernelGGL((elbo_fwd_kernel<TT, SE, true, false, (qb::gtab_segs(TT) > 0)>), dim3(grid), dim3(kBlock), 0, s, \
                       ctx->dev, ctx->d_gtab, x, mask, q, prior, sigma, zs, zk, S, K, seed, voxel0, \
                       out, partials, N)
    const bool gt = ctx->gtab_ok && !(ctx->kernel_sel & 8) && qb::gtab_segs(ctx->dev.T) > 0;
    const bool fast = qb::elbo_fast_path(ctx);
    const bool lds64 = qb::elbo_logsigma_path(ctx);
    if (sigma_is_log && !lds64) {
        qb::set_error("elbo_fwd_launch: log-sigma input is built for the 64-tau protocol with tau = 0 at index 12 "
                      "(table mode, Gaussian likelihood, one-image normalisation)");
        return QBOLD_ERR_UNSUPPORTED;
    }
    if (lds64) {
        QB_REQUIRE(reinterpret_cast<uintptr_t>(x) % 16 == 0 && reinterpret_cast<uintptr_t>(sigma) % 16 == 0,
                   "qbold_elbo_fwd (64-tau protocol): x and sigma must be 16-byte aligned");
        if (ctx->gtab_ok && qb::gtab_segs(64) > 0 && !(ctx->kernel_sel & 8) && !zs && !zk) {
            constexpr size_t smem = sizeof(float4) * qb::gtab_taus(64, 12) * qb::gtab_segs(64) + sizeof(float) * 64 +
                                    sizeof(float2) * (64 - 12) * kGtVox + sizeof(double) * 3 * (kGtBlock / 64);
            static_assert(smem <= 160 * 1024, "table + data rows exceed the LDS");
            const int64_t nt = (N + kGtVox - 1) / kGtVox;
            grid = (int)(nt < ctx->num_cus ? (nt > 0 ? nt : 1) : ctx->num_cus);
            auto kern = sigma_is_log ? elbo_fwd_gt64_kernel<64, 12, true> : elbo_fwd_gt64_kernel<64, 12, false>;
            QB_HIP(hipFuncSetAttribute(reinterpret_cast<const void*>(kern), hipFuncAttributeMaxDynamicSharedMemorySize,
                                       (int)smem));
            hipLaunchKernelGGL(kern, dim3(grid), dim3(kGtBlock), smem, s, ctx->dev, ctx->d_gtab, x, mask, q, prior, sigma,
                               S, K, seed, voxel0, out, partials, N);
            QB_HIP(hipGetLastError());
            hipLaunchKernelGGL(qb::reduce_partials_kernel, dim3(1), dim3(192), 0, s, partials, grid, sums);
            QB_HIP(hipGetLastError());
            return QBOLD_OK;
        }
        const int64_t gt = (N + kLdsVox - 1) / kLdsVox;
        grid = (int)(gt < qb::elbo_grid(ctx) ? (gt > 0 ? gt : 1) : qb::elbo_grid(ctx));
        if (sigma_is_log)
            hipLaunchKernelGGL((elbo_fwd_lds_kernel<64, 12, true>), dim3(grid), dim3(kLdsBlock), 0, s, ctx->dev,
                               ctx->d_tab, x, mask, q, prior, sigma, zs, zk, S, K, seed, voxel0, out, partials, N);
        else
            hipLaunchKernelGGL((elbo_fwd_lds_kernel<64, 12, false>), dim3(grid), dim3(kLdsBlock), 0, s, ctx->dev,
                               ctx->d_tab, x, mask, q, prior, sigma, zs, zk, S, K, seed, voxel0, out, partials, N);
    } else switch (ctx->dev.T) {
        case 11:
            if (fast && ctx->dev.se_idx == 2 && !ctx->dev.multi_norm && gt) QB_LAUNCH_ELBO_GT(11, 2);
            else if (fast && ctx->dev.se_idx == 2 && !ctx->dev.multi_norm && ctx->grid_mirrors) QB_LAUNCH_ELBO_MIR(11, 2);
            else if (fast && ctx->dev.se_idx == 2 && !ctx->dev.multi_norm) QB_LAUNCH_ELBO(11, 2, true, false);
            else if (fast) QB_LAUNCH_ELBO(11, -1, true, false);
            else if (lit && ctx->dev.se_idx == 2 && !ctx->dev.multi_norm) QB_LAUNCH_ELBO(11, 2, false, true);
            else if (lit) QB_LAUNCH_ELBO(11, -1, false, true);
            else QB_LAUNCH_ELBO(11, -1, false, false);
            break;
        case 24:
            if (fast && ctx->dev.se_idx == 7 && !ctx->dev.multi_norm && gt) QB_LAUNCH_ELBO_GT(24, 7);
            else if (fast && ctx->dev.se_idx == 7 && !ctx->dev.multi_norm && ctx->grid_mirrors) QB_LAUNCH_ELBO_MIR(24, 7);
            else if (fast && ctx->dev.se_idx == 7 && !ctx->dev.multi_norm) QB_LAUNCH_ELBO(24, 7, true, false);
            else if (fast) QB_LAUNCH_ELBO(24, -1, true, false);
            else if (lit && ctx->dev.se_idx == 7 && !ctx->dev.multi_norm) QB_LAUNCH_ELBO(24, 7, false, true);
            else if (lit) QB_LAUNCH_ELBO(24, -1, false, true);
            else QB_LAUNCH_ELBO(24, -1, false, false);
            break;
        default: {
            if (!fast) {
                qb::set_error("qbold_elbo_fwd: for T other than 11 / 24 only the optimal.yaml "
                              "configuration (table mode, Gaussian likelihood, linear data) is built");
                return QBOLD_ERR_UNSUPPORTED;
            }
            const int64_t gt = (N + kGenVox - 1) / kGenVox;
            grid = (int)(gt < qb::elbo_grid(ctx) ? (gt > 0 ? gt : 1) : qb::elbo_grid(ctx));
            const size_t smem = sizeof(qb::FwdLds) + sizeof(float) * 2 * QB_MAX_T * kGenVox;
            hipLaunchKernelGGL(elbo_fwd_generic_kernel, dim3(grid), dim3(kGenBlock), smem, s, ctx->dev,
                               ctx->d_tab, x, mask, q, prior, sigma, zs, zk, S, K, seed, voxel0, out,
                               partials, N);
        }
    }
#undef QB_LAUNCH_ELBO
#undef QB_LAUNCH_ELBO_MIR
#undef QB_LAUNCH_ELBO_GT
    QB_HIP(hipGetLastError());
    hipLaunchKernelGGL(qb::reduce_partials_kernel, dim3(1), dim3(192), 0, s, partials, grid, sums);
    QB_HIP(hipGetLastError());
    return QBOLD_OK;
}
}

extern "C" int qbold_elbo_fwd(const qbold_ctx* ctx, const float* x, const float* mask, const float* q,
                              const float* prior, const float* sigma, const float* zs,
                              const float* zk, int S, int K, uint64_t seed, int64_t voxel0,
                              float* nll_kl, double* sums, void* workspace, int64_t N, void* stream) {
    QB_NEED_DEVICE(ctx);
    QB_REQUIRE(N >= 0 && S >= 1 && K >= 0, "qbold_elbo_fwd: need N >= 0, S >= 1, K >= 0");
    QB_REQUIRE(sums && workspace, "qbold_elbo_fwd: null sums/workspace");
    QB_REQUIRE(N == 0 || (x && q && prior && sigma), "qbold_elbo_fwd: null input buffer");
    return qb::elbo_fwd_launch(ctx, x, mask, q, prior, sigma, false, zs, zk, S, K, seed, voxel0, nll_kl, sums,
                               workspace, N, (hipStream_t)stream);
}

extern "C" int qbold_elbo_fwd_logsigma(const qbold_ctx* ctx, const float* x, const float* mask, const float* q,
                                       const float* prior, const float* log_sigma, int S, int K, uint64_t seed,
                                       int64_t voxel0, float* nll_kl, double* sums, void* workspace, int64_t N,
                                       void* stream) {
    QB_NEED_DEVICE(ctx);
    QB_REQUIRE(N >= 0 && S >= 1 && K >= 0, "qbold_elbo_fwd_logsigma: need N >= 0, S >= 1, K >= 0");
    QB_REQUIRE(sums && workspace, "qbold_elbo_fwd_logsigma: null sums/workspace");
    QB_REQUIRE(N == 0 || (x && q && prior && log_sigma), "qbold_elbo_fwd_logsigma: null input buffer");
    return qb::elbo_fwd_launch(ctx, x, mask, q, prior, log_sigma, true, nullptr, nullptr, S, K, seed, voxel0, nll_kl,
                               sums, workspace, N, (hipStream_t)stream);
}

__global__ __launch_bounds__(256) void kl_diag_kernel(const float* __restrict__ q, const float* __restrict__ prior,
                                                      const float* __restrict__ mask, float* __restrict__ kl_v,
                                                      float* __restrict__ g_q, double* __restrict__ partials,
                                                      int64_t N) {
    __shared__ double red[3 * 4];
    float s_kl = 0.0f, s_m = 0.0f;
    for (int64_t v = blockIdx.x * (int64_t)blockDim.x + threadIdx.x; v < N;
         v += (int64_t)gridDim.x * blockDim.x) {
        float qv[5], pv[5];
#pragma unroll
        for (int k = 0; k < 5; ++k) {
            qv[k] = q[v * 5 + k];
            pv[k] = prior[v * 5 + k];
        }
        const float m = mask ? mask[v] : 1.0f;
        const float sqo = qb::transform_std(qv[1]), sqd = qb::transform_std(qv[3]);
        const float spo = qb::transform_std(pv[1]), spd = qb::transform_std(pv[3]);
        const float ipo = __expf(-spo), ipd = __expf(-spd);
        const float do_ = sqo - spo, dd = sqd - spd;
        const float ro = (qv[0] - pv[0]) * ipo, rd = (qv[2] - pv[2]) * ipd;
        const float eo = expm1f(2.0f * do_), ed = expm1f(2.0f * dd);
        const float kl = (0.5f * ro * ro + 0.5f * eo - do_) + (0.5f * rd * rd + 0.5f * ed - dd);
        if (kl_v) kl_v[v] = kl;
        if (m > 0.0f) s_kl += kl;
        s_m += m;
        if (g_q && m > 0.0f) {
            const float to = (sqo + 1.0f) * (1.0f / 3.0f), td = (sqd + 1.0f) * (1.0f / 3.0f);
            g_q[v * 5 + 0] += ro * ipo;
            g_q[v * 5 + 1] += eo * 3.0f * (1.0f - to * to);
            g_q[v * 5 + 2] += rd * ipd;
            g_q[v * 5 + 3] += ed * 3.0f * (1.0f - td * td);
        }
    }
    qb::block_partials(red, 0.0f, s_kl, s_m, partials);
}

extern "C" int qbold_kl_diag(const qbold_ctx* ctx, const float* q, const float* prior, const float* mask,
                             float* kl_v, float* g_q, double* sums, void* workspace, int64_t N,
                             void* stream) {
    QB_NEED_DEVICE(ctx);
    QB_REQUIRE(N >= 0 && sums && workspace, "qbold_kl_diag: null sums/workspace");
    QB_REQUIRE(N == 0 || (q && prior), "qbold_kl_diag: null buffer");
    hipStream_t s = (hipStream_t)stream;
    double* partials = reinterpret_cast<double*>(workspace);
    const int64_t nb = (N + 255) / 256;
    const int grid = (int)(nb < qb::elbo_grid(ctx) ? (nb > 0 ? nb : 1) : qb::elbo_grid(ctx));
    hipLaunchKernelGGL(kl_diag_kernel, dim3(grid), dim3(256), 0, s, q, prior, mask, kl_v, g_q, partials, N);
    QB_HIP(hipGetLastError());
    hipLaunchKernelGGL(qb::reduce_partials_kernel, dim3(1), dim3(192), 0, s, partials, grid, sums);
    QB_HIP(hipGetLastError());
    return QBOLD_OK;
}

constexpr int kMaxMog = 16;
__global__ __launch_bounds__(256) void kl_mog_kernel(const float* __restrict__ q, const float* __restrict__ comps, int M,
                                                     const float* __restrict__ z, uint64_t seed, int64_t voxel0,
                                                     float* __restrict__ kl_v, int64_t N) {
    __shared__ float cm[kMaxMog][4];
    __shared__ float cs[kMaxMog];
    if (threadIdx.x < M) {
        const float so = qb::transform_std(comps[4 * threadIdx.x + 1]), sd = qb::transform_std(comps[4 * threadIdx.x + 3]);
        cm[threadIdx.x][0] = comps[4 * threadIdx.x + 0];
        cm[threadIdx.x][1] = __expf(-so);
        cm[threadIdx.x][2] = comps[4 * threadIdx.x + 2];
        cm[threadIdx.x][3] = __expf(-sd);
        cs[threadIdx.x] = so + sd;
    }
    __syncthreads();
    const float inv_m = 1.0f / (float)M;
    for (int64_t v = blockIdx.x * (int64_t)blockDim.x + threadIdx.x; v < N; v += (int64_t)gridDim.x * blockDim.x) {
        float z0, z1;
        if (z) {
            z0 = z[2 * v];
            z1 = z[2 * v + 1];
        } else {
            float zz[4];
            qb::normals4(seed, (uint64_t)(voxel0 + v), 0u, 4u, zz);
            z0 = zz[0];
            z1 = zz[1];
        }
        const float so = qb::transform_std(q[v * 5 + 1]), sd = qb::transform_std(q[v * 5 + 3]);
        const float xo = fmaf(z0, __expf(so), q[v * 5 + 0]), xd = fmaf(z1, __expf(sd), q[v * 5 + 2]);
        float acc = 0.0f;
        for (int c = 0; c < M; ++c) {
            const float ro = (xo - cm[c][0]) * cm[c][1], rd = (xd - cm[c][2]) * cm[c][3];
            acc += cs[c] + 0.5f * fmaf(ro, ro, rd * rd);
        }
        kl_v[v] = fmaf(acc, inv_m, -(so + sd));
    }
}

extern "C" int qbold_kl_mog(const qbold_ctx* ctx, const float* q, const float* comps, int M, const float* z,
                            uint64_t seed, int64_t voxel0, float* kl_v, int64_t N, void* stream) {
    QB_NEED_DEVICE(ctx);
    if (N == 0) return QBOLD_OK;
    QB_REQUIRE(N > 0 && q && comps && kl_v && M >= 1 && M <= kMaxMog, "qbold_kl_mog: bad argument (1 <= M <= 16)");
    hipLaunchKernelGGL(kl_mog_kernel, dim3(ew_grid(ctx, N, 256)), dim3(256), 0, (hipStream_t)stream, q, comps, M, z, seed,
                       voxel0, kl_v, N);
    QB_HIP(hipGetLastError());
    return QBOLD_OK;
}

extern "C" int qbold_reparam(const qbold_ctx* ctx, const float* q, const float* z, float* oef_dbv,
                             int64_t N, void* stream) {
    QB_NEED_DEVICE(ctx);
    if (N == 0) return QBOLD_OK;
    QB_REQUIRE(N > 0 && q && z && oef_dbv, "qbold_reparam: bad argument");
    hipLaunchKernelGGL(reparam_kernel, dim3(ew_grid(ctx, N, 256)), dim3(256), 0, (hipStream_t)stream,
                       q, reinterpret_cast<const float2*>(z), reinterpret_cast<float2*>(oef_dbv), N);
    QB_HIP(hipGetLastError());
    return QBOLD_OK;
}

extern "C" int qbold_logit_mvn_nlogp(const qbold_ctx* ctx, const float* y, const float* params,
                                     float* out, int64_t N, void* stream) {
    QB_NEED_DEVICE(ctx);
    if (N == 0) return QBOLD_OK;
    QB_REQUIRE(N > 0 && y && params && out, "qbold_logit_mvn_nlogp: bad argument");
    hipLaunchKernelGGL(nlogp_kernel, dim3(ew_grid(ctx, N, 256)), dim3(256), 0, (hipStream_t)stream,
                       reinterpret_cast<const float2*>(y), params, out, N);
    QB_HIP(hipGetLastError());
    return QBOLD_OK;
}

__global__ void swr_kernel(const float2* __restrict__ obs, const float2* __restrict__ mean, const float* __restrict__ so,
                           const float* __restrict__ sd, const float* __restrict__ cov, float* __restrict__ out,
                           int64_t N) {
    for (int64_t i = (int64_t)blockIdx.x * blockDim.x + threadIdx.x; i < N; i += (int64_t)gridDim.x * blockDim.x) {
        const float2 o = obs[i], m = mean[i];
        const float a = so[i], b = sd[i];
        const float inv_tl = __expf(-a), inv_br = __expf(-b);
        const float inv_bl = __expf(-a - b) * cov[i] * -1.0f;
// ... 45 lines not shown
```

### qbold_vi_amd/csrc/grid_kernels.hip

```cpp
#include <cmath>

#include "elbo_core.h"
#include "qbold_ctx.h"

namespace qb {
bool elbo_fast_path(const qbold_ctx* ctx);
int elbo_grid(const qbold_ctx* ctx);
}

namespace {

constexpr int kBlock = 256;
constexpr int kWaves = kBlock / QB_WAVE;
constexpr int kMaxN = 256;
constexpr int kMaxChunks = kMaxN / QB_WAVE;
constexpr int kMaxGh = 32;
constexpr float kLog2Pi = 1.8378770664093453f;

struct GhRule {
    int n;
    float t[kMaxGh], w[kMaxGh];
};

struct GridArgs {
// ... 353 lines not shown
    o.v[12] = dbv_of(qb1);
    o.v[13] = oef_of(fmaf((float)(bidx / n), ha, bx.a0));
    o.v[14] = dbv_of(fmaf((float)(bidx % n), hb, bx.b0));
    o.v[15] = Sr * iZ;
    o.v[16] = fabsf(logf(Z) - logf(4.0f * Se));
    o.v[1] = NAN;
    if (has_q && gh.n > 0) o.v[1] = -gh_expected_nll(ev, qm, gh) - kl_closed(qm, pm);
    o.box = bx;
}


template <int T, int SE, bool FAST, bool LITERAL, bool MIR, class LDS>
struct RegEval {
    const LDS* L;
    const QbDev* c;
    const qb::VoxelLik<T>* lik;
    __device__ __forceinline__ float log_lik(float a, float b) const {
        if constexpr (FAST && qb::IsGtLds<LDS>::value) {
            return -fmaf(0.5f, qb::sample_sq_fast<T, SE>(L, *c, *lik, qb::sigmoidf_(a), qb::sigmoidf_(b)),
                         lik->log_s_sum);
        } else {
            float oef, dbv;
            qb::forward_transform(a, b, oef, dbv);
            if constexpr (FAST) return -fmaf(0.5f, qb::sample_sq_fast<T, SE, MIR>(L, *c, *lik, oef, dbv), lik->log_s_sum);
            else return -qb::sample_nll<T, SE, LITERAL>(L, *c, *lik, oef, dbv);
        }
    }
};

template <int T, int SE, bool GT>
struct GridLds { using type = qb::FwdLds; };
template <int T, int SE>
struct GridLds<T, SE, true> { using type = qb::GtLds<T, SE>; };

__device__ __forceinline__ void store_voxel(const GridOut& o, bool live, int64_t v, float m, float* __restrict__ out,
                                            float* __restrict__ box, double& s_lp, double& s_el, double& s_m) {
    const int lane = threadIdx.x & 63;
    if (lane < QBOLD_GRID_OUT) {
        float val = NAN;
#pragma unroll
        for (int i = 0; i < QBOLD_GRID_OUT; ++i)
            if (i == lane) val = o.v[i];
        out[v * QBOLD_GRID_OUT + lane] = live ? val : NAN;
    }
    if (box && lane < 4) {
        const float bv = lane == 0 ? o.box.a0 : lane == 1 ? o.box.a1 : lane == 2 ? o.box.b0 : o.box.b1;
        box[v * 4 + lane] = live ? bv : NAN;
    }
    if (live && lane == 0) {
        s_lp += (double)m * -(double)o.v[0];
        if (o.v[1] == o.v[1]) s_el += (double)m * -(double)o.v[1];
        s_m += (double)m;
    }
}

__device__ __forceinline__ double wave_sum_d(double v) {
#pragma unroll
    for (int o = 32; o > 0; o >>= 1) v += __shfl_xor(v, o, 64);
    return v;
}
__device__ __forceinline__ void block_partials_d(double* red, double a, double b, double m,
                                                 double* __restrict__ partials) {
    const int lane = threadIdx.x & 63, wave = threadIdx.x >> 6;
    a = wave_sum_d(a);
    b = wave_sum_d(b);
    m = wave_sum_d(m);
    if (lane == 0) {
        red[3 * wave + 0] = a;
        red[3 * wave + 1] = b;
        red[3 * wave + 2] = m;
    }
    __syncthreads();
    if (threadIdx.x < 3) {
        double s = 0.0;
        for (int w = 0; w < kWaves; ++w) s += red[3 * w + threadIdx.x];
        partials[3 * blockIdx.x + threadIdx.x] = s;
    }
}

template <int T, int SE, bool FAST, bool LITERAL, bool GT = false, bool MIR = false>
__global__ __launch_bounds__(kBlock) void grid_kernel(
    QbDev c, const float4* __restrict__ g_tab, const float* __restrict__ x, const float* __restrict__ mask,
    const float* __restrict__ prior, const float* __restrict__ sigma, const float* __restrict__ q, GridArgs ga,
    GhRule gh, float* __restrict__ out, float* __restrict__ box, double* __restrict__ partials, int64_t N) {
    static_assert(!GT || (FAST && SE >= 0 && qb::gtab_segs(T) > 0), "GT needs the fast path with a compile-time spin echo");
    static_assert(!MIR || (FAST && SE >= 0), "merged mirror pairs: fast path with a compile-time spin echo");
    constexpr bool kMir = GT || MIR;
    using Lds = typename GridLds<T, SE, GT>::type;
    __shared__ Lds L;
    __shared__ float rows[kWaves][2][kMaxN];
    __shared__ double red[3 * kWaves];
    if constexpr (qb::IsGtLds<Lds>::value) {
        qb::gt_lds_fill(&L, g_tab, c);
    } else {
        qb::fwd_lds_fill(&L, g_tab, true);
        if (threadIdx.x < QB_MAX_T) L.blood_B[threadIdx.x] = c.blood_B[threadIdx.x];
    }
    __syncthreads();
    const int wave = threadIdx.x >> 6;
    double s_lp = 0.0, s_el = 0.0, s_m = 0.0;
    for (int64_t v = (int64_t)blockIdx.x * kWaves + wave; v < N; v += (int64_t)gridDim.x * kWaves) {
        const float m = mask ? mask[v] : 1.0f;
        const bool live = m > 0.0f;
        GridOut o;
        if (live) {
            float xv[T], sv[T], pv[5], qv[5];
#pragma unroll
            for (int t = 0; t < T; ++t) {
                xv[t] = x[v * T + t];
                sv[t] = sigma[v * T + t];
            }
#pragma unroll
            for (int i = 0; i < 5; ++i) {
                pv[i] = prior[v * 5 + i];
                qv[i] = q ? q[v * 5 + i] : 0.0f;
            }
            qb::VoxelLik<T> lik;
            qb::prepare_lik<T, SE, false, (FAST && SE >= 0), FAST, kMir>(c, xv, sv, m, lik);
            const qb::LogitMvn pm = qb::make_mvn(pv), qm = qb::make_mvn(qv);
            const RegEval<T, SE, FAST, LITERAL, kMir, Lds> ev{&L, &c, &lik};
            grid_voxel(ev, c, pm, qm, q != nullptr, ga, gh, rows[wave][0], rows[wave][1], o);
        }
        store_voxel(o, live, v, m, out, box, s_lp, s_el, s_m);
    }
    block_partials_d(red, s_lp, s_el, s_m, partials);
}

struct GenEval {
    const qb::FwdLds* L;
    const QbDev* c;
    const float* yt;
    const float* is;
    float log_s_sum;
    int T, se;
    bool mirrored;
    __device__ __forceinline__ float log_lik(float a, float b) const {
        float oef, dbv;
        qb::forward_transform(a, b, oef, dbv);
        const qb::FwdFast fv = qb::fwd_fast(*c, oef, dbv);
        float acc = 0.0f;
        if (mirrored) {
            const float s_se = fmaf(fv.tissue_w, 1.0f, fv.blood_w * qb::exp2f_(fv.ng * L->blood_B[se]));
            const float inv_np = qb::rcpf_(s_se + 1e-3f);
            const float lt = qb::log2f_(fv.tissue_w * inv_np), lb = qb::log2f_(fv.blood_w * inv_np);
            auto signal = [&](int t) {
                const float u = fabsf(fmaf((float)t, fv.ub, fv.ua));
                const float4 kk = L->tab[(int)u];
                const float f = __builtin_amdgcn_fractf(u);
                const float F = fmaf(fmaf(fmaf(kk.w, f, kk.z), f, kk.y), f, kk.x);
                return qb::exp2f_(fmaf(fv.nd, F, lt)) + qb::exp2f_(fmaf(fv.ng, L->blood_B[t], lb));
            };
            auto residual = [&](int t, float yh) {
                const float r = (yt[t] - yh) * is[t];
                acc = fmaf(r, r, acc);
            };
            residual(se, s_se * inv_np);
            for (int t = se + 1; t < T; ++t) {
                const float yh = signal(t);
                residual(t, yh);
                if (2 * se - t >= 0) residual(2 * se - t, yh);
            }
            for (int t = 0; t < 2 * se - (T - 1); ++t) residual(t, signal(t));
        } else {
            float np_ = qb::fwd_signal_fast(L, *c, fv, se);
            if (c->multi_norm)
                np_ = (np_ + qb::fwd_signal_fast(L, *c, fv, se - 1) + qb::fwd_signal_fast(L, *c, fv, se + 1)) / 3.0f;
            const float inv_np = qb::rcpf_(np_ + 1e-3f);
            for (int t = 0; t < T; ++t) {
                const float st = qb::fwd_signal_fast(L, *c, fv, t);
                const float r = fmaf(-st, inv_np, yt[t]) * is[t];
                acc = fmaf(r, r, acc);
            }
        }
        return -fmaf(0.5f, acc, log_s_sum);
    }
};

__global__ __launch_bounds__(kBlock) void grid_generic_kernel(
    QbDev c, const float4* __restrict__ g_tab, const float* __restrict__ x, const float* __restrict__ mask,
    const float* __restrict__ prior, const float* __restrict__ sigma, const float* __restrict__ q, GridArgs ga,
    GhRule gh, float* __restrict__ out, float* __restrict__ box, double* __restrict__ partials, int64_t N) {
    __shared__ qb::FwdLds L;
    __shared__ float rows[kWaves][2][kMaxN];
    __shared__ float yts[kWaves][2][QB_MAX_T];
    __shared__ double red[3 * kWaves];
    qb::fwd_lds_fill(&L, g_tab, false);
    if (threadIdx.x < QB_MAX_T) L.blood_B[threadIdx.x] = c.blood_B[threadIdx.x];
    __syncthreads();
    const int T = c.T, se = c.se_idx;
    const bool mirrored = !c.multi_norm && fmaf((float)se, c.tauh_step, c.tauh0) == 0.0f;
    const int lane = threadIdx.x & 63, wave = threadIdx.x >> 6;
    float* yt = yts[wave][0];
    float* is = yts[wave][1];
    double s_lp = 0.0, s_el = 0.0, s_m = 0.0;
    for (int64_t v = (int64_t)blockIdx.x * kWaves + wave; v < N; v += (int64_t)gridDim.x * kWaves) {
        const float m = mask ? mask[v] : 1.0f;
        const bool live = m > 0.0f;
        GridOut o;
        if (live) {
            const float* xv = x + v * T;
            const float* sv = sigma + v * T;
            const float nt = c.multi_norm ? (xv[se - 1] + xv[se] + xv[se + 1]) / 3.0f + 1e-3f : xv[se] + 1e-3f;
            const float inv_nt = qb::rcpf_(nt);
            float ls = 0.0f;
            if (lane < T) {
                yt[lane] = xv[lane] * inv_nt;
                is[lane] = qb::rcpf_(sv[lane]);
                ls = QB_LN2 * qb::log2f_(sv[lane]);
            }
            wave_lds_sync();
            const float log_s_sum = wave_sum(ls) + (float)T * 0.9189385332046727f;
            float pv[5], qv[5];
#pragma unroll
            for (int i = 0; i < 5; ++i) {
                pv[i] = prior[v * 5 + i];
                qv[i] = q ? q[v * 5 + i] : 0.0f;
            }
            const qb::LogitMvn pm = qb::make_mvn(pv), qm = qb::make_mvn(qv);
            const GenEval ev{&L, &c, yt, is, log_s_sum, T, se, mirrored};
            grid_voxel(ev, c, pm, qm, q != nullptr, ga, gh, rows[wave][0], rows[wave][1], o);
            wave_lds_sync();
        }
        store_voxel(o, live, v, m, out, box, s_lp, s_el, s_m);
    }
    block_partials_d(red, s_lp, s_el, s_m, partials);
}

void gauss_hermite(int n, GhRule& r) {
    r.n = n;
    const double pim4 = 0.7511255444649425;
    const int m = (n + 1) / 2;
    double z = 0.0;
    for (int i = 0; i < m; ++i) {
        if (i == 0) z = std::sqrt(2.0 * n + 1.0) - 1.85575 * std::pow(2.0 * n + 1.0, -0.16667);
        else if (i == 1) z -= 1.14 * std::pow((double)n, 0.426) / z;
        else if (i == 2) z = 1.86 * z - 0.86 * r.t[0];
        else if (i == 3) z = 1.91 * z - 0.91 * r.t[1];
        else z = 2.0 * z - r.t[i - 2];
        double pp = 0.0;
        for (int it = 0; it < 100; ++it) {
            double p1 = pim4, p2 = 0.0;
            for (int j = 1; j <= n; ++j) {
                const double p3 = p2;
                p2 = p1;
                p1 = z * std::sqrt(2.0 / j) * p2 - std::sqrt((j - 1.0) / j) * p3;
            }
            pp = std::sqrt(2.0 * n) * p2;
            const double z1 = z;
            z = z1 - p1 / pp;
            if (std::fabs(z - z1) <= 1e-15 * std::fmax(1.0, std::fabs(z))) {
                p1 = pim4;
                p2 = 0.0;
                for (int j = 1; j <= n; ++j) {
                    const double p3 = p2;
                    p2 = p1;
                    p1 = z * std::sqrt(2.0 / j) * p2 - std::sqrt((j - 1.0) / j) * p3;
                }
                pp = std::sqrt(2.0 * n) * p2;
                break;
            }
        }
        const double w = 2.0 / (pp * pp) / 1.7724538509055159;
        r.t[i] = (float)z;
        r.t[n - 1 - i] = (float)-z;
        r.w[i] = r.w[n - 1 - i] = (float)w;
    }
}

}

extern "C" int qbold_posterior_grid(const qbold_ctx* ctx, const float* x, const float* mask, const float* prior,
                                    const float* sigma, const float* q, const qbold_grid_cfg* cfg, float* out,
                                    float* box, double* sums, void* workspace, int64_t N, void* stream) {
    QB_NEED_DEVICE(ctx);
    QB_REQUIRE(cfg, "qbold_posterior_grid: null cfg");
    QB_REQUIRE(N >= 0, "qbold_posterior_grid: need N >= 0");
    QB_REQUIRE(cfg->coarse % 8 == 0 && cfg->coarse >= 16 && cfg->coarse <= 128,
               "qbold_posterior_grid: coarse must be a multiple of 8 in [16, 128]");
    QB_REQUIRE(cfg->fine % 8 == 0 && cfg->fine >= 16 && cfg->fine <= kMaxN,
               "qbold_posterior_grid: fine must be a multiple of 8 in [16, 256]");
    QB_REQUIRE(cfg->locate >= 1 && cfg->locate <= 4, "qbold_posterior_grid: locate must be in [1, 4]");
    QB_REQUIRE(cfg->gh == 0 || (cfg->gh >= 2 && cfg->gh <= kMaxGh), "qbold_posterior_grid: gh must be 0 or in [2, 32]");
    QB_REQUIRE(cfg->span > 0.0f && cfg->span < INFINITY, "qbold_posterior_grid: need span > 0");
    QB_REQUIRE(cfg->cut >= 10.0f && cfg->cut <= 80.0f, "qbold_posterior_grid: cut must be in [10, 80]");
    QB_REQUIRE(cfg->level_lo > 0.0f && cfg->level_lo < cfg->level_hi && cfg->level_hi < 1.0f,
               "qbold_posterior_grid: need 0 < level_lo < level_hi < 1");
    QB_REQUIRE(out && sums && workspace, "qbold_posterior_grid: null out/sums/workspace");
    QB_REQUIRE(N == 0 || (x && prior && sigma), "qbold_posterior_grid: null input buffer");
    const bool lit = ctx->dev.tissue_mode == QBOLD_TISSUE_LITERAL;
    const bool fast = qb::elbo_fast_path(ctx);
    const int T = ctx->dev.T;
    if (T != 11 && T != 24 && !fast) {
        qb::set_error("qbold_posterior_grid: for T other than 11 / 24 only the optimal.yaml configuration (table "
                      "mode, Gaussian likelihood, linear data) is built");
        return QBOLD_ERR_UNSUPPORTED;
    }
    GridArgs ga{cfg->coarse, cfg->fine, cfg->locate, cfg->span, cfg->cut, cfg->level_lo, cfg->level_hi};
    GhRule gh{};
    if (q && cfg->gh > 0) gauss_hermite(cfg->gh, gh);
    hipStream_t s = (hipStream_t)stream;
    double* partials = reinterpret_cast<double*>(workspace);
    const int64_t nblk = (N + kWaves - 1) / kWaves;
    const int grid = (int)(nblk < qb::elbo_grid(ctx) ? (nblk > 0 ? nblk : 1) : qb::elbo_grid(ctx));
    const bool gt = ctx->gtab_ok && !(ctx->kernel_sel & 8) && qb::gtab_segs(T) > 0;
#define QB_GRID_ARGS ctx->dev, ctx->d_tab, x, mask, prior, sigma, q, ga, gh, out, box, partials, N
#define QB_LAUNCH_GRID(TT, SE, FAST, LIT) \
    hipLaunchKernelGGL((grid_kernel<TT, SE, FAST, LIT>), dim3(grid), dim3(kBlock), 0, s, QB_GRID_ARGS)
#define QB_LAUNCH_GRID_MIR(TT, SE) \
    hipLaunchKernelGGL((grid_kernel<TT, SE, true, false, false, true>), dim3(grid), dim3(kBlock), 0, s, QB_GRID_ARGS)
#define QB_LAUNCH_GRID_GT(TT, SE)                                                                                    \
    hipLaunchKernelGGL((grid_kernel<TT, SE, true, false, (qb::gtab_segs(TT) > 0)>), dim3(grid), dim3(kBlock), 0, s, \
                       ctx->dev, ctx->d_gtab, x, mask, prior, sigma, q, ga, gh, out, box, partials, N)
    switch (T) {
        case 11:
            if (fast && ctx->dev.se_idx == 2 && !ctx->dev.multi_norm && gt) QB_LAUNCH_GRID_GT(11, 2);
            else if (fast && ctx->dev.se_idx == 2 && !ctx->dev.multi_norm && ctx->grid_mirrors) QB_LAUNCH_GRID_MIR(11, 2);
            else if (fast && ctx->dev.se_idx == 2 && !ctx->dev.multi_norm) QB_LAUNCH_GRID(11, 2, true, false);
            else if (fast) QB_LAUNCH_GRID(11, -1, true, false);
            else if (lit && ctx->dev.se_idx == 2 && !ctx->dev.multi_norm) QB_LAUNCH_GRID(11, 2, false, true);
            else if (lit) QB_LAUNCH_GRID(11, -1, false, true);
            else QB_LAUNCH_GRID(11, -1, false, false);
            break;
        case 24:
            if (fast && ctx->dev.se_idx == 7 && !ctx->dev.multi_norm && gt) QB_LAUNCH_GRID_GT(24, 7);
            else if (fast && ctx->dev.se_idx == 7 && !ctx->dev.multi_norm && ctx->grid_mirrors) QB_LAUNCH_GRID_MIR(24, 7);
            else if (fast && ctx->dev.se_idx == 7 && !ctx->dev.multi_norm) QB_LAUNCH_GRID(24, 7, true, false);
            else if (fast) QB_LAUNCH_GRID(24, -1, true, false);
            else if (lit && ctx->dev.se_idx == 7 && !ctx->dev.multi_norm) QB_LAUNCH_GRID(24, 7, false, true);
            else if (lit) QB_LAUNCH_GRID(24, -1, false, true);
            else QB_LAUNCH_GRID(24, -1, false, false);
            break;
        default:
            hipLaunchKernelGGL(grid_generic_kernel, dim3(grid), dim3(kBlock), 0, s, QB_GRID_ARGS);
    }
#undef QB_LAUNCH_GRID
#undef QB_LAUNCH_GRID_MIR
#undef QB_LAUNCH_GRID_GT
#undef QB_GRID_ARGS
    QB_HIP(hipGetLastError());
    hipLaunchKernelGGL(qb::reduce_partials_kernel, dim3(1), dim3(192), 0, s, partials, grid, sums);
    QB_HIP(hipGetLastError());
    return QBOLD_OK;
}
```

### qbold_vi_amd/csrc/iw_bwd_kernels.hip

```cpp
#include <cmath>

#include "elbo_core.h"
#include "qbold_ctx.h"

#ifndef QB_IW_BWD_LPV1_MAX_K
#define QB_IW_BWD_LPV1_MAX_K 32
#endif

namespace qb {
int elbo_grid(const qbold_ctx* ctx);
}

namespace {

constexpr uint32_t kStreamIw = 6u;
constexpr int kBlock = 256;

struct FwdGrad {
    float s, ds_doef, ds_ddbv;
};

__device__ __forceinline__ FwdGrad fwd_signal_grad(const qb::FwdLds* L, const QbDev& c,
                                                   const qb::FwdFast& v, float oef, float dbv, int t) {
    const float us = fmaf((float)t, v.ub, v.ua);
// ... 88 lines not shown
        if (c.predict_log) {
            dyp = m > 0.0f ? qb::rcpf_(yp) : 0.0f;
            yp = m > 0.0f ? __logf(yp) : 0.0f;
        }
        const float r = (lik.yt[t] - yp) * lik.inv_s[t];
        float dr = r;
        if (c.use_student_t) {
            const float w = (c.st_df + 1.0f) * qb::rcpf_(fmaf(r, r, c.st_df));
            sq += (c.st_df + 1.0f) * log1pf(r * r * qb::rcpf_(c.st_df)) - 2.0f * c.st_const;
            dr = w * r;
        } else {
            sq = fmaf(r, r, sq);
        }
        dls[t] = 1.0f - dr * r;
        gy[t] = -dr * lik.inv_s[t] * dyp;
        a1 = fmaf(gy[t], sig[t], a1);
    }
    a1 *= inv_np * inv_np;
    const float lw = -fmaf(0.5f, sq, lik.log_s_sum) - fmaf(0.5f, dswr, kl.cst);
    const float mn = fmaxf(acc.M, lw);
    const float r1 = qb::exp2f_((acc.M - mn) * QB_LOG2E);
    const float e1 = qb::exp2f_((lw - mn) * QB_LOG2E);
    const float r2 = r1 * r1, e2 = e1 * e1;
    acc.M = mn;
    acc.s1 = fmaf(acc.s1, r1, e1);
    acc.s2 = fmaf(acc.s2, r2, e2);
    acc.slw += lw;
#pragma unroll
    for (int t = 0; t < T; ++t) acc.gs[t] = fmaf(acc.gs[t], r1, e1 * dls[t]);
    float g_oef = 0.0f, g_dbv = 0.0f;
#pragma unroll
    for (int t = 0; t < T; ++t) {
        float gs = gy[t] * inv_np;
        if (SE >= 0) {
            if (t == SE) gs -= a1;
        } else if (c.multi_norm) {
            if (t >= c.se_idx - 1 && t <= c.se_idx + 1) gs -= a1 * (1.0f / 3.0f);
        } else if (t == c.se_idx) {
            gs -= a1;
        }
        const FwdGrad fg = fwd_signal_grad(L, c, fv, oef, dbv, t);
        g_oef = fmaf(gs, fg.ds_doef, g_oef);
        g_dbv = fmaf(gs, fg.ds_ddbv, g_dbv);
    }
    const float ha = fmaf(g_oef * QB_OEF_RANGE, sa * (1.0f - sa), ka);
    const float hb = fmaf(g_dbv * QB_DBV_RANGE, sb * (1.0f - sb), kb);
    const float wa = e2 * ha, wb = e2 * hb;
    acc.h[0] = fmaf(acc.h[0], r2, wa);
    acc.h[1] = fmaf(acc.h[1], r2, wa * z0);
    acc.h[2] = fmaf(acc.h[2], r2, wb);
    acc.h[3] = fmaf(acc.h[3], r2, wb * z1);
    acc.h[4] = fmaf(acc.h[4], r2, wb * z0);
}

__device__ __forceinline__ double wave_sum_d(double v) {
#pragma unroll
    for (int o = 32; o > 0; o >>= 1) v += __shfl_xor(v, o, 64);
    return v;
}
__device__ __forceinline__ void block_partials_d(double* red, double a, double b, double m,
                                                 double* __restrict__ partials) {
    const int lane = threadIdx.x & 63, wave = threadIdx.x >> 6, nw = blockDim.x >> 6;
    a = wave_sum_d(a);
    b = wave_sum_d(b);
    m = wave_sum_d(m);
    if (lane == 0) {
        red[3 * wave + 0] = a;
        red[3 * wave + 1] = b;
        red[3 * wave + 2] = m;
    }
    __syncthreads();
    if (threadIdx.x < 3) {
        double s = 0.0;
        for (int w = 0; w < nw; ++w) s += red[3 * w + threadIdx.x];
        partials[3 * blockIdx.x + threadIdx.x] = s;
    }
}

template <int T, int SE, int LPV>
__global__ __launch_bounds__(kBlock) void iw_bwd_kernel(
    QbDev c, const float4* __restrict__ g_tab, const float* __restrict__ x, const float* __restrict__ mask,
    const float* __restrict__ q, const float* __restrict__ prior, const float* __restrict__ log_sigma,
    const float* __restrict__ z, int K, uint64_t seed, int64_t voxel0, float* __restrict__ g_q,
    float* __restrict__ g_ls, float* __restrict__ out, double* __restrict__ partials, int64_t N) {
    __shared__ qb::FwdLds L;
    __shared__ double red[3 * (kBlock / 64)];
    qb::fwd_lds_fill(&L, g_tab, false);
    __syncthreads();

    constexpr int kVoxPerBlock = kBlock / LPV, kVoxPerWave = 64 / LPV;
    const int lane = threadIdx.x & 63, wave = threadIdx.x >> 6;
    const int part = LPV == 1 ? 0 : lane >> 4;
    auto voxel_sum = [](float v) { return LPV == 1 ? v : qb::voxel_sum(v); };
    double s_lp = 0.0, s_el = 0.0, s_m = 0.0;
    const int64_t ntile = (N + kVoxPerBlock - 1) / kVoxPerBlock;
    for (int64_t tile = blockIdx.x; tile < ntile; tile += gridDim.x) {
        const int64_t v = tile * kVoxPerBlock + wave * kVoxPerWave + (LPV == 1 ? lane : lane & 15);
        if (v >= N) continue;
        const float m = mask ? mask[v] : 1.0f;
        const bool in = m > 0.0f;
        if (!in && !out) {
            if (part == 0) {
#pragma unroll
                for (int i = 0; i < 5; ++i) g_q[v * 5 + i] = 0.0f;
            }
            if (part == (LPV == 1 ? 0 : 1)) {
#pragma unroll
                for (int t = 0; t < T; ++t) g_ls[v * T + t] = 0.0f;
            }
            continue;
        }
        float xv[T], lsv[T], qv[5], pv[5];
#pragma unroll
        for (int t = 0; t < T; ++t) {
            xv[t] = x[v * T + t];
            lsv[t] = log_sigma[v * T + t];
        }
#pragma unroll
        for (int i = 0; i < 5; ++i) {
            qv[i] = q[v * 5 + i];
            pv[i] = prior[v * 5 + i];
        }
        qb::VoxelLik<T> lik;
        qb::prepare_lik<T, SE, true>(c, xv, lsv, m, lik);
        const qb::LogitMvn qm = qb::make_mvn(qv), pm = qb::make_mvn(pv);
        const IwKl kl = make_iw_kl(qm, pm);
        const uint64_t vox = (uint64_t)(voxel0 + v);
        const float* zv = z ? z + v * (int64_t)K * 2 : nullptr;
        IwGradAcc<T> acc;
        acc.init();
#pragma unroll 1
        for (int g = part; 4 * g < K; g += LPV) {
            const int cnt = K - 4 * g < 4 ? K - 4 * g : 4;
            qb::DrawQuad dq;
            if (!zv) dq.load(seed, vox, (uint32_t)g, kStreamIw);
#pragma unroll 1
            for (int d = 0; d < cnt; ++d) {
                float z0, z1;
                if (zv) {
                    z0 = zv[2 * (4 * g + d)];
                    z1 = zv[2 * (4 * g + d) + 1];
                } else {
                    dq.next(z0, z1);
                }
                iw_bwd_draw<T, SE>(&L, c, lik, m, qm, pm, kl, z0, z1, acc);
            }
        }
        float Mx = acc.M;
        if (LPV > 1) {
            Mx = fmaxf(Mx, __shfl_xor(Mx, 16, 64));
            Mx = fmaxf(Mx, __shfl_xor(Mx, 32, 64));
        }
        const float f1 = LPV == 1 ? 1.0f : qb::exp2f_((acc.M - Mx) * QB_LOG2E);
        const float f2 = f1 * f1;
        const float s1 = voxel_sum(acc.s1 * f1), s2 = voxel_sum(acc.s2 * f2), slw = voxel_sum(acc.slw);
        float h[5];
#pragma unroll
        for (int i = 0; i < 5; ++i) h[i] = voxel_sum(acc.h[i] * f2);
        const float inv1 = 1.0f / s1;
        const float inv2 = inv1 * inv1;
        if (part == 0) {
            const float th1 = (qm.s_o + 1.0f) * (1.0f / 3.0f), th3 = (qm.s_d + 1.0f) * (1.0f / 3.0f);
            const float th4 = qm.c * 7.38905609893065f;
            const float wq = m * inv2;
            g_q[v * 5 + 0] = in ? wq * h[0] : 0.0f;
            g_q[v * 5 + 1] = in ? wq * (h[1] * qm.e_so) * 3.0f * (1.0f - th1 * th1) : 0.0f;
            g_q[v * 5 + 2] = in ? wq * h[2] : 0.0f;
            g_q[v * 5 + 3] = in ? wq * (h[3] * qm.e_sd) * 3.0f * (1.0f - th3 * th3) : 0.0f;
            g_q[v * 5 + 4] = in ? wq * h[4] * 0.1353352832366127f * (1.0f - th4 * th4) : 0.0f;
            const float lp = Mx + (logf(s1) - logf((float)K));
            const float el = slw / (float)K;
            if (out) {
                out[3 * v + 0] = lp;
                out[3 * v + 1] = el;
                out[3 * v + 2] = (s1 * s1) / s2;
            }
            if (in) {
                s_lp += (double)m * -(double)lp;
                s_el += (double)m * -(double)el;
                s_m += (double)m;
            }
        }
        float gsum[T];
#pragma unroll
        for (int t = 0; t < T; ++t) gsum[t] = voxel_sum(acc.gs[t] * f1);
        if (part == (LPV == 1 ? 0 : 1)) {
            const float ws = m * inv1;
#pragma unroll
            for (int t = 0; t < T; ++t) g_ls[v * T + t] = in ? ws * gsum[t] : 0.0f;
        }
    }
    block_partials_d(red, s_lp, s_el, s_m, partials);
}

}

extern "C" int qbold_log_evidence_bwd(const qbold_ctx* ctx, const float* x, const float* mask, const float* q,
                                      const float* prior, const float* log_sigma, const float* z, int K,
                                      uint64_t seed, int64_t voxel0, float* g_q, float* g_log_sigma, float* out,
                                      double* sums, void* workspace, int64_t N, void* stream) {
    QB_NEED_DEVICE(ctx);
    QB_REQUIRE(N >= 0 && K >= 1 && K <= QBOLD_IW_MAX_K,
               "qbold_log_evidence_bwd: need N >= 0 and 1 <= K <= QBOLD_IW_MAX_K");
    QB_REQUIRE(sums && workspace, "qbold_log_evidence_bwd: null sums/workspace");
    QB_REQUIRE(N == 0 || (x && q && prior && log_sigma && g_q && g_log_sigma),
               "qbold_log_evidence_bwd: null buffer");
    if (!(ctx->dev.full_model && ctx->dev.tissue_mode == QBOLD_TISSUE_TABLE)) {
        qb::set_error("qbold_log_evidence_bwd: gradients are built for the full signal model in table mode "
                      "(qbold_elbo_bwd's configurations)");
        return QBOLD_ERR_UNSUPPORTED;
    }
    if (ctx->dev.T != 11 && ctx->dev.T != 24) {
        qb::set_error("qbold_log_evidence_bwd: kernels are built for T = 11 or 24 taus");
        return QBOLD_ERR_UNSUPPORTED;
    }
    hipStream_t s = (hipStream_t)stream;
    double* partials = reinterpret_cast<double*>(workspace);
    const int lpv = K <= QB_IW_BWD_LPV1_MAX_K ? 1 : QB_LANES_PER_VOXEL;
    const int vpb = kBlock / lpv;
    const int64_t ntile = (N + vpb - 1) / vpb;
    const int grid = (int)(ntile < qb::elbo_grid(ctx) ? (ntile > 0 ? ntile : 1) : qb::elbo_grid(ctx));
#define QB_LAUNCH_IWB(TT, SEC)                                                                                       \
    do {                                                                                                             \
        if (lpv == 1)                                                                                                \
            hipLaunchKernelGGL((iw_bwd_kernel<TT, SEC, 1>), dim3(grid), dim3(kBlock), 0, s, ctx->dev, ctx->d_tab, x,  \
                               mask, q, prior, log_sigma, z, K, seed, voxel0, g_q, g_log_sigma, out, partials, N);   \
        else                                                                                                         \
            hipLaunchKernelGGL((iw_bwd_kernel<TT, SEC, QB_LANES_PER_VOXEL>), dim3(grid), dim3(kBlock), 0, s,         \
                               ctx->dev, ctx->d_tab, x, mask, q, prior, log_sigma, z, K, seed, voxel0, g_q,          \
                               g_log_sigma, out, partials, N);                                                       \
    } while (0)
    if (ctx->dev.T == 24) {
        QB_LAUNCH_IWB(24, -1);
    } else if (ctx->dev.se_idx == 2 && !ctx->dev.multi_norm) {
        QB_LAUNCH_IWB(11, 2);
    } else {
        QB_LAUNCH_IWB(11, -1);
    }
#undef QB_LAUNCH_IWB
    QB_HIP(hipGetLastError());
    hipLaunchKernelGGL(qb::reduce_partials_kernel, dim3(1), dim3(192), 0, s, partials, grid, sums);
    QB_HIP(hipGetLastError());
    return QBOLD_OK;
}
```

### qbold_vi_amd/csrc/iw_kernels.hip

```cpp
#include <cmath>

#include "elbo_core.h"
#include "qbold_ctx.h"

namespace qb {
bool elbo_fast_path(const qbold_ctx* ctx);
int elbo_grid(const qbold_ctx* ctx);
}

namespace {

constexpr uint32_t kStreamIw = 6u;

constexpr int kBlock = 256;
constexpr int kVoxPerBlock = kBlock / QB_LANES_PER_VOXEL;

template <int T, int SE, bool GT>
struct IwLds { using type = qb::FwdLds; };
template <int T, int SE>
struct IwLds<T, SE, true> { using type = qb::GtLds<T, SE>; };

struct IwAcc {
    float m, s1, s2, so, sd, sr, slw;
    __device__ __forceinline__ void init() {
// ... 74 lines not shown
        } else {
            qb::forward_transform(a, b, oef, dbv);
            if constexpr (FAST) nll = fmaf(0.5f, qb::sample_sq_fast<T, SE, MIR>(L, c, lik, oef, dbv), lik.log_s_sum);
            else nll = qb::sample_nll<T, SE, LITERAL>(L, c, lik, oef, dbv);
        }
        float dswr = iw_dswr(kl, z0, z1);
        if (!WHITEN && fmaxf(fabsf(a), fabsf(b)) > QB_LOGIT_CLIP) dswr = qb::kl_swr_diff(q, p, z0, z1);
        acc.add(-nll - fmaf(0.5f, dswr, kl.cst), oef, dbv, (c.dw_coef * oef) * dbv);
    }
}

__device__ __forceinline__ bool iw_whiten(const qb::LogitMvn& q, const float* zv) {
    const float reach = fmaxf(fabsf(q.mu_o) + QB_Z_MAX * q.e_so, fabsf(q.mu_d) + QB_Z_MAX * (fabsf(q.c) + q.e_sd));
    return zv == nullptr && __all(reach < QB_LOGIT_CLIP);
}

struct IwOut {
    float log_p, elbo, ess, mo, md, mr;
};
__device__ __forceinline__ IwOut iw_finish(IwAcc a, int K) {
    float M = fmaxf(a.m, __shfl_xor(a.m, 16, 64));
    M = fmaxf(M, __shfl_xor(M, 32, 64));
    const float f = qb::exp2f_((a.m - M) * QB_LOG2E);
    const float s1 = qb::voxel_sum(a.s1 * f), s2 = qb::voxel_sum(a.s2 * (f * f));
    const float so = qb::voxel_sum(a.so * f), sd = qb::voxel_sum(a.sd * f), sr = qb::voxel_sum(a.sr * f);
    const float slw = qb::voxel_sum(a.slw);
    IwOut o;
    o.log_p = M + (logf(s1) - logf((float)K));
    o.elbo = slw / (float)K;
    o.ess = (s1 * s1) / s2;
    const float inv = 1.0f / s1;
    o.mo = so * inv;
    o.md = sd * inv;
    o.mr = sr * inv;
    return o;
}

__device__ __forceinline__ double wave_sum_d(double v) {
#pragma unroll
    for (int o = 32; o > 0; o >>= 1) v += __shfl_xor(v, o, 64);
    return v;
}
__device__ __forceinline__ void block_partials_d(double* red, double a, double b, double m,
                                                 double* __restrict__ partials) {
    const int lane = threadIdx.x & 63, wave = threadIdx.x >> 6, nw = blockDim.x >> 6;
    a = wave_sum_d(a);
    b = wave_sum_d(b);
    m = wave_sum_d(m);
    if (lane == 0) {
        red[3 * wave + 0] = a;
        red[3 * wave + 1] = b;
        red[3 * wave + 2] = m;
    }
    __syncthreads();
    if (threadIdx.x < 3) {
        double s = 0.0;
        for (int w = 0; w < nw; ++w) s += red[3 * w + threadIdx.x];
        partials[3 * blockIdx.x + threadIdx.x] = s;
    }
}

__device__ __forceinline__ void iw_store(const IwOut& o, int64_t v, float m, float* __restrict__ out,
                                         float* __restrict__ is_means, double& s_lp, double& s_el, double& s_m) {
    out[3 * v + 0] = o.log_p;
    out[3 * v + 1] = o.elbo;
    out[3 * v + 2] = o.ess;
    if (is_means) {
        is_means[3 * v + 0] = o.mo;
        is_means[3 * v + 1] = o.md;
        is_means[3 * v + 2] = o.mr;
    }
    if (m > 0.0f) {
        s_lp += (double)m * -(double)o.log_p;
        s_el += (double)m * -(double)o.elbo;
    }
    s_m += (double)m;
}

template <int T, int SE, bool FAST, bool LITERAL, bool GT = false, bool MIR = false>
__global__ __launch_bounds__(kBlock) void iw_fwd_kernel(
    QbDev c, const float4* __restrict__ g_tab, const float* __restrict__ x, const float* __restrict__ mask,
    const float* __restrict__ q, const float* __restrict__ prior, const float* __restrict__ sigma,
    const float* __restrict__ z, int K, uint64_t seed, int64_t voxel0, float* __restrict__ out,
    float* __restrict__ is_means, double* __restrict__ partials, int64_t N) {
    static_assert(!GT || (FAST && SE >= 0 && qb::gtab_segs(T) > 0), "GT needs the fast path with a compile-time spin echo");
    static_assert(!MIR || (FAST && SE >= 0), "merged mirror pairs: fast path with a compile-time spin echo");
    constexpr bool kMir = GT || MIR;
    using Lds = typename IwLds<T, SE, GT>::type;
    __shared__ Lds L;
    __shared__ double red[3 * (kBlock / 64)];
    if constexpr (qb::IsGtLds<Lds>::value) {
        qb::gt_lds_fill(&L, g_tab, c);
    } else {
        qb::fwd_lds_fill(&L, g_tab, true);
        if (threadIdx.x < QB_MAX_T) L.blood_B[threadIdx.x] = c.blood_B[threadIdx.x];
    }
    __syncthreads();

    const int lane = threadIdx.x & 63, wave = threadIdx.x >> 6;
    const int part = lane >> 4;
    double s_lp = 0.0, s_el = 0.0, s_m = 0.0;
    const int64_t ntile = (N + kVoxPerBlock - 1) / kVoxPerBlock;
    for (int64_t tile = blockIdx.x; tile < ntile; tile += gridDim.x) {
        const int64_t v = tile * kVoxPerBlock + wave * QB_VOX_PER_WAVE + (lane & 15);
        if (v < N) {
            float xv[T], sv[T], qv[5], pv[5];
#pragma unroll
            for (int t = 0; t < T; ++t) {
                xv[t] = x[v * T + t];
                sv[t] = sigma[v * T + t];
            }
#pragma unroll
            for (int i = 0; i < 5; ++i) {
                qv[i] = q[v * 5 + i];
                pv[i] = prior[v * 5 + i];
            }
            const float m = mask ? mask[v] : 1.0f;
            qb::VoxelLik<T> lik;
            qb::prepare_lik<T, SE, false, (FAST && SE >= 0), FAST, kMir>(c, xv, sv, m, lik);
            const qb::LogitMvn qm = qb::make_mvn(qv), pm = qb::make_mvn(pv);
            const IwKl kl = make_iw_kl(qm, pm);
            const float* zv = z ? z + v * (int64_t)K * 2 : nullptr;
            IwAcc acc;
            acc.init();
            const uint64_t vox = (uint64_t)(voxel0 + v);
            __builtin_amdgcn_s_setprio(QB_PRIO_LIK);
            if (iw_whiten(qm, zv))
                iw_draws<T, SE, FAST, LITERAL, kMir, true>(&L, c, lik, qm, pm, kl, K, zv, seed, vox, part, acc);
            else
                iw_draws<T, SE, FAST, LITERAL, kMir, false>(&L, c, lik, qm, pm, kl, K, zv, seed, vox, part, acc);
            __builtin_amdgcn_s_setprio(QB_PRIO_AFTER);
            const IwOut o = iw_finish(acc, K);
            if (part == 0) iw_store(o, v, m, out, is_means, s_lp, s_el, s_m);
        }
    }
    block_partials_d(red, s_lp, s_el, s_m, partials);
}

constexpr int kGenBlock = 128;
constexpr int kGenVox = kGenBlock / QB_LANES_PER_VOXEL;

__device__ __forceinline__ float generic_half_sq(const qb::FwdLds* L, const QbDev& c, const qb::FwdFast& fv,
                                                 const float* yt, const float* is, int vl, int T, int se,
                                                 bool mirrored) {
    float acc = 0.0f;
    if (mirrored) {
        const float s_se = fmaf(fv.tissue_w, 1.0f, fv.blood_w * qb::exp2f_(fv.ng * L->blood_B[se]));
        const float inv_np = qb::rcpf_(s_se + 1e-3f);
        const float lt = qb::log2f_(fv.tissue_w * inv_np), lb = qb::log2f_(fv.blood_w * inv_np);
        auto signal = [&](int t) {
            const float u = fabsf(fmaf((float)t, fv.ub, fv.ua));
            const float4 kk = L->tab[(int)u];
            const float f = __builtin_amdgcn_fractf(u);
            const float F = fmaf(fmaf(fmaf(kk.w, f, kk.z), f, kk.y), f, kk.x);
            return qb::exp2f_(fmaf(fv.nd, F, lt)) + qb::exp2f_(fmaf(fv.ng, L->blood_B[t], lb));
        };
        auto residual = [&](int t, float yh) {
            const float r = (yt[t * kGenVox + vl] - yh) * is[t * kGenVox + vl];
            acc = fmaf(r, r, acc);
        };
        residual(se, s_se * inv_np);
        for (int t = se + 1; t < T; ++t) {
            const float yh = signal(t);
            residual(t, yh);
            if (2 * se - t >= 0) residual(2 * se - t, yh);
        }
        for (int t = 0; t < 2 * se - (T - 1); ++t) residual(t, signal(t));
        return 0.5f * acc;
    }
    float np_ = qb::fwd_signal_fast(L, c, fv, se);
    if (c.multi_norm)
        np_ = (np_ + qb::fwd_signal_fast(L, c, fv, se - 1) + qb::fwd_signal_fast(L, c, fv, se + 1)) / 3.0f;
    const float inv_np = qb::rcpf_(np_ + 1e-3f);
    for (int t = 0; t < T; ++t) {
        const float st = qb::fwd_signal_fast(L, c, fv, t);
        const float r = fmaf(-st, inv_np, yt[t * kGenVox + vl]) * is[t * kGenVox + vl];
        acc = fmaf(r, r, acc);
    }
    return 0.5f * acc;
}

__global__ __launch_bounds__(kGenBlock) void iw_fwd_generic_kernel(
    QbDev c, const float4* __restrict__ g_tab, const float* __restrict__ x, const float* __restrict__ mask,
    const float* __restrict__ q, const float* __restrict__ prior, const float* __restrict__ sigma,
    const float* __restrict__ z, int K, uint64_t seed, int64_t voxel0, float* __restrict__ out,
    float* __restrict__ is_means, double* __restrict__ partials, int64_t N) {
    extern __shared__ __align__(16) unsigned char smem[];
    qb::FwdLds* L = reinterpret_cast<qb::FwdLds*>(smem);
    float* yt = reinterpret_cast<float*>(smem + sizeof(qb::FwdLds));
    float* is = yt + QB_MAX_T * kGenVox;
    __shared__ double red[3 * (kGenBlock / 64)];
    qb::fwd_lds_fill(L, g_tab, false);
    if (threadIdx.x < QB_MAX_T) L->blood_B[threadIdx.x] = c.blood_B[threadIdx.x];
    __syncthreads();

    const int T = c.T, se = c.se_idx;
    const bool mirrored = !c.multi_norm && fmaf((float)se, c.tauh_step, c.tauh0) == 0.0f;
    const int lane = threadIdx.x & 63, wave = threadIdx.x >> 6;
    const int part = lane >> 4;
    const int vl = wave * QB_VOX_PER_WAVE + (lane & 15);
    double s_lp = 0.0, s_el = 0.0, s_m = 0.0;
    const int64_t ntile = (N + kGenVox - 1) / kGenVox;
    for (int64_t tile = blockIdx.x; tile < ntile; tile += gridDim.x) {
        const int64_t v = tile * kGenVox + vl;
        const bool live = v < N;
        const int64_t vc = live ? v : N - 1;
        const float* xv = x + vc * T;
        const float* sv = sigma + vc * T;
        const float nt = c.multi_norm ? (xv[se - 1] + xv[se] + xv[se + 1]) / 3.0f + 1e-3f : xv[se] + 1e-3f;
        const float inv_nt = qb::rcpf_(nt);
        float ls = 0.0f;
        __syncthreads();
        for (int t = part; t < T; t += QB_LANES_PER_VOXEL) {
            yt[t * kGenVox + vl] = xv[t] * inv_nt;
            is[t * kGenVox + vl] = qb::rcpf_(sv[t]);
            ls += QB_LN2 * qb::log2f_(sv[t]);
        }
        const float log_s_sum = qb::voxel_sum(ls) + (float)T * 0.9189385332046727f;
        __syncthreads();
        if (live) {
            float qv[5], pv[5];
#pragma unroll
            for (int i = 0; i < 5; ++i) {
                qv[i] = q[v * 5 + i];
                pv[i] = prior[v * 5 + i];
            }
            const float m = mask ? mask[v] : 1.0f;
            const qb::LogitMvn qm = qb::make_mvn(qv), pm = qb::make_mvn(pv);
            const IwKl kl = make_iw_kl(qm, pm);
            const float* zv = z ? z + v * (int64_t)K * 2 : nullptr;
            const bool whiten = iw_whiten(qm, zv);
            const uint64_t vox = (uint64_t)(voxel0 + v);
            IwAcc acc;
            acc.init();
            const int n = iw_lane_draws(K, part);
            qb::DrawQuad dq;
            uint32_t g = (uint32_t)part;
            for (int i = 0; i < n; ++i) {
                float z0, z1;
                if (zv) {
                    const int draw = 4 * (part + 4 * (i >> 2)) + (i & 3);
                    z0 = zv[2 * draw];
                    z1 = zv[2 * draw + 1];
                } else {
                    if ((i & 3) == 0) {
                        dq.load(seed, vox, g, kStreamIw);
                        g += QB_LANES_PER_VOXEL;
                    }
                    dq.next(z0, z1);
                }
                float a, b, oef, dbv;
                qb::reparam_logits(qm, z0, z1, a, b);
                qb::forward_transform(a, b, oef, dbv);
                const qb::FwdFast fv = qb::fwd_fast(c, oef, dbv);
                const float nll = generic_half_sq(L, c, fv, yt, is, vl, T, se, mirrored) + log_s_sum;
                float dswr = iw_dswr(kl, z0, z1);
                if (!whiten && fmaxf(fabsf(a), fabsf(b)) > QB_LOGIT_CLIP) dswr = qb::kl_swr_diff(qm, pm, z0, z1);
                acc.add(-nll - fmaf(0.5f, dswr, kl.cst), oef, dbv, (c.dw_coef * oef) * dbv);
            }
            const IwOut o = iw_finish(acc, K);
            if (part == 0) iw_store(o, v, m, out, is_means, s_lp, s_el, s_m);
        }
    }
    block_partials_d(red, s_lp, s_el, s_m, partials);
}

}

extern "C" int qbold_log_evidence_fwd(const qbold_ctx* ctx, const float* x, const float* mask, const float* q,
                                      const float* prior, const float* sigma, const float* z, int K, uint64_t seed,
                                      int64_t voxel0, float* out, float* is_means, double* sums, void* workspace,
                                      int64_t N, void* stream) {
    QB_NEED_DEVICE(ctx);
    QB_REQUIRE(N >= 0 && K >= 1 && K <= QBOLD_IW_MAX_K,
               "qbold_log_evidence_fwd: need N >= 0 and 1 <= K <= QBOLD_IW_MAX_K");
    QB_REQUIRE(out && sums && workspace, "qbold_log_evidence_fwd: null out/sums/workspace");
    QB_REQUIRE(N == 0 || (x && q && prior && sigma), "qbold_log_evidence_fwd: null input buffer");
    hipStream_t s = (hipStream_t)stream;
    double* partials = reinterpret_cast<double*>(workspace);
    const int64_t ntile = (N + kVoxPerBlock - 1) / kVoxPerBlock;
    int grid = (int)(ntile < qb::elbo_grid(ctx) ? (ntile > 0 ? ntile : 1) : qb::elbo_grid(ctx));
    const bool lit = ctx->dev.tissue_mode == QBOLD_TISSUE_LITERAL;
    const bool fast = qb::elbo_fast_path(ctx);
    const bool gt = ctx->gtab_ok && !(ctx->kernel_sel & 8) && qb::gtab_segs(ctx->dev.T) > 0;
#define QB_LAUNCH_IW(TT, SE, FAST, LIT)                                                                            \
    hipLaunchKernelGGL((iw_fwd_kernel<TT, SE, FAST, LIT>), dim3(grid), dim3(kBlock), 0, s, ctx->dev, ctx->d_tab, x, \
                       mask, q, prior, sigma, z, K, seed, voxel0, out, is_means, partials, N)
#define QB_LAUNCH_IW_MIR(TT, SE)                                                                                    \
    hipLaunchKernelGGL((iw_fwd_kernel<TT, SE, true, false, false, true>), dim3(grid), dim3(kBlock), 0, s, ctx->dev, \
                       ctx->d_tab, x, mask, q, prior, sigma, z, K, seed, voxel0, out, is_means, partials, N)
#define QB_LAUNCH_IW_GT(TT, SE)                                                                                     \
    hipLaunchKernelGGL((iw_fwd_kernel<TT, SE, true, false, (qb::gtab_segs(TT) > 0)>), dim3(grid), dim3(kBlock), 0, \
                       s, ctx->dev, ctx->d_gtab, x, mask, q, prior, sigma, z, K, seed, voxel0, out, is_means,       \
                       partials, N)
    switch (ctx->dev.T) {
        case 11:
            if (fast && ctx->dev.se_idx == 2 && !ctx->dev.multi_norm && gt) QB_LAUNCH_IW_GT(11, 2);
            else if (fast && ctx->dev.se_idx == 2 && !ctx->dev.multi_norm && ctx->grid_mirrors) QB_LAUNCH_IW_MIR(11, 2);
            else if (fast && ctx->dev.se_idx == 2 && !ctx->dev.multi_norm) QB_LAUNCH_IW(11, 2, true, false);
            else if (fast) QB_LAUNCH_IW(11, -1, true, false);
            else if (lit && ctx->dev.se_idx == 2 && !ctx->dev.multi_norm) QB_LAUNCH_IW(11, 2, false, true);
            else if (lit) QB_LAUNCH_IW(11, -1, false, true);
            else QB_LAUNCH_IW(11, -1, false, false);
            break;
        case 24:
            if (fast && ctx->dev.se_idx == 7 && !ctx->dev.multi_norm && gt) QB_LAUNCH_IW_GT(24, 7);
            else if (fast && ctx->dev.se_idx == 7 && !ctx->dev.multi_norm && ctx->grid_mirrors) QB_LAUNCH_IW_MIR(24, 7);
            else if (fast && ctx->dev.se_idx == 7 && !ctx->dev.multi_norm) QB_LAUNCH_IW(24, 7, true, false);
            else if (fast) QB_LAUNCH_IW(24, -1, true, false);
            else if (lit && ctx->dev.se_idx == 7 && !ctx->dev.multi_norm) QB_LAUNCH_IW(24, 7, false, true);
            else if (lit) QB_LAUNCH_IW(24, -1, false, true);
            else QB_LAUNCH_IW(24, -1, false, false);
            break;
        default: {
            if (!fast) {
                qb::set_error("qbold_log_evidence_fwd: for T other than 11 / 24 only the optimal.yaml "
                              "configuration (table mode, Gaussian likelihood, linear data) is built");
                return QBOLD_ERR_UNSUPPORTED;
            }
            const int64_t gtile = (N + kGenVox - 1) / kGenVox;
            grid = (int)(gtile < qb::elbo_grid(ctx) ? (gtile > 0 ? gtile : 1) : qb::elbo_grid(ctx));
            const size_t smem = sizeof(qb::FwdLds) + sizeof(float) * 2 * QB_MAX_T * kGenVox;
            hipLaunchKernelGGL(iw_fwd_generic_kernel, dim3(grid), dim3(kGenBlock), smem, s, ctx->dev, ctx->d_tab, x,
                               mask, q, prior, sigma, z, K, seed, voxel0, out, is_means, partials, N);
        }
    }
#undef QB_LAUNCH_IW
#undef QB_LAUNCH_IW_MIR
#undef QB_LAUNCH_IW_GT
    QB_HIP(hipGetLastError());
    hipLaunchKernelGGL(qb::reduce_partials_kernel, dim3(1), dim3(192), 0, s, partials, grid, sums);
    QB_HIP(hipGetLastError());
    return QBOLD_OK;
}

namespace {

struct IwRowSink {
    float* __restrict__ lw;
    float* __restrict__ th;
    bool vec;
    float l[4], t[12];
    __device__ __forceinline__ void push(float lwk, float oef, float dbv, float r2p) {
#pragma unroll
        for (int i = 0; i < 3; ++i) l[i] = l[i + 1];
#pragma unroll
        for (int i = 0; i < 9; ++i) t[i] = t[i + 3];
        l[3] = lwk;
        t[9] = oef;
        t[10] = dbv;
        t[11] = r2p;
    }
    __device__ __forceinline__ void flush(int d0, int cnt) {
        if (cnt == 4 && vec) {
            *reinterpret_cast<float4*>(lw + d0) = make_float4(l[0], l[1], l[2], l[3]);
            if (th) {
                float4* p = reinterpret_cast<float4*>(th + 3 * d0);
                p[0] = make_float4(t[0], t[1], t[2], t[3]);
                p[1] = make_float4(t[4], t[5], t[6], t[7]);
                p[2] = make_float4(t[8], t[9], t[10], t[11]);
            }
            return;
        }
#pragma unroll
        for (int i = 0; i < 4; ++i) {
            const int d = d0 + i - (4 - cnt);
            if (i >= 4 - cnt) {
                lw[d] = l[i];
                if (th) {
                    th[3 * d + 0] = t[3 * i + 0];
                    th[3 * d + 1] = t[3 * i + 1];
                    th[3 * d + 2] = t[3 * i + 2];
                }
            }
        }
    }
};

__device__ __forceinline__ void iw_nan_rows(int K, int part, float* __restrict__ lw, float* __restrict__ th) {
    const float nan = __uint_as_float(0x7fc00000u);
    for (int g = part; 4 * g < K; g += QB_LANES_PER_VOXEL)
        for (int d = 4 * g; d < 4 * g + 4 && d < K; ++d) {
            lw[d] = nan;
            if (th) th[3 * d + 0] = th[3 * d + 1] = th[3 * d + 2] = nan;
        }
}

template <int T, int SE, bool FAST, bool MIR, bool WHITEN, class LDS>
__device__ __forceinline__ void iw_draws_to_rows(const LDS* L, const QbDev& c, const qb::VoxelLik<T>& lik,
                                               const qb::LogitMvn& q, const qb::LogitMvn& p, const IwKl& kl, int K,
                                               const float* __restrict__ zv, uint64_t seed, uint64_t vox, int part,
                                               IwRowSink& sink) {
    const int n = iw_lane_draws(K, part);
    qb::DrawQuad dq;
    uint32_t g = (uint32_t)part;
#pragma unroll 1
    for (int i = 0; i < n; ++i) {
        float z0, z1;
        if (zv) {
            const int draw = 4 * (part + 4 * (i >> 2)) + (i & 3);
            z0 = zv[2 * draw];
            z1 = zv[2 * draw + 1];
        } else {
            if ((i & 3) == 0) {
                dq.load(seed, vox, g, kStreamIw);
                g += QB_LANES_PER_VOXEL;
            }
            dq.next(z0, z1);
        }
        float a, b, oef, dbv, nll;
        qb::reparam_logits(q, z0, z1, a, b);
        if constexpr (FAST && qb::IsGtLds<LDS>::value) {
            const float sa = qb::sigmoidf_(a), sb = qb::sigmoidf_(b);
            nll = fmaf(0.5f, qb::sample_sq_fast<T, SE>(L, c, lik, sa, sb), lik.log_s_sum);
// ... 217 lines not shown
```

### qbold_vi_amd/csrc/qbold_ctx.h

```cpp
#pragma once

#include <hip/hip_runtime.h>

#include <string>
#include <vector>

#include "../../include/qbold_hip.h"
#include "qbold_dev.h"

struct qbold_ctx {
    int device = 0;
    qbold_consts consts{};
    qbold_loss_cfg loss{};
    QbDev dev{};
    float4* d_tab = nullptr;
    std::vector<float> h_tab;
    float4* d_gtab = nullptr;
    std::vector<float> h_gtab;
    bool gtab_ok = false;
    bool grid_mirrors = false;
    int num_cus = 256;
    float dF_node0_ref = 0.0f;
    int kernel_sel = 0;
};

namespace qb {
void set_error(const std::string& msg);
int hip_fail(hipError_t e, const char* what);
}

#define QB_HIP(call)                                              \
    do {                                                          \
        hipError_t _e = (call);                                   \
        if (_e != hipSuccess) return qb::hip_fail(_e, #call);     \
    } while (0)

#define QB_NEED_DEVICE(ctx)                                                   \
    do {                                                                      \
        if (!(ctx) || (ctx)->device < 0) {                                    \
            qb::set_error("context has no device (host-only or null)");       \
            return QBOLD_ERR_NO_DEVICE;                                       \
        }                                                                     \
    } while (0)

#define QB_RELU_ONLY(shape, what)                                                                      \
    do {                                                                                               \
        if ((shape) && ((shape)->activation != QBOLD_ACT_RELU || (shape)->layer_norm)) {               \
            qb::set_error(what ": activation 'gelu' and use_layer_norm run through the layer-wise "    \
                               "entry points (qbold_encoder_train_fwd / _bwd, qbold_encoder_spatial_fwd / _bwd)");   \
            return QBOLD_ERR_UNSUPPORTED;                                                              \
        }                                                                                              \
    } while (0)

#define QB_REQUIRE(cond, msg)              \
    do {                                   \
        if (!(cond)) {                     \
            qb::set_error(msg);            \
            return QBOLD_ERR_INVALID;      \
        }                                  \
    } while (0)
```

### qbold_vi_amd/csrc/vi_kernels.hip

```cpp
#include "elbo_core.h"
#ifndef QB_PRIO_TILE_START
#define QB_PRIO_TILE_START 3
#endif
#define QB_ENC_BASE_PRIO 2
#include "encoder_core.h"
#include "qbold_ctx.h"

namespace qb {
int check_encoder_shape(const qbold_ctx* ctx, const qbold_encoder_shape* s);
bool elbo_fast_path(const qbold_ctx* ctx);
bool elbo_logsigma_path(const qbold_ctx* ctx);
int elbo_fwd_launch(const qbold_ctx* ctx, const float* x, const float* mask, const float* q, const float* prior,
                    const float* sigma, bool sigma_is_log, const float* zs, const float* zk, int S, int K,
                    uint64_t seed, int64_t voxel0, float* nll_kl, double* sums, void* workspace, int64_t N,
                    hipStream_t s);
bool wide_fused_supported(const qbold_encoder_shape* s);
int wide_fused_fwd(const qbold_ctx* ctx, const qbold_encoder_shape* shape, const float* packed, const float* x,
                   float* out_q, float* out_log_sigma, int64_t N, hipStream_t s);
}

namespace {

using qb::EncLayout;
using qb::f32x4;

constexpr int kBlock = 1024;
#ifndef QB_VI_BLOCK_24
#define QB_VI_BLOCK_24 768
#endif

template <int T, int SE, bool GT>
struct ViLds { using type = qb::FwdLds; };
template <int T, int SE>
struct ViLds<T, SE, true> { using type = qb::GtLds<T, SE>; };
constexpr size_t kLdsLimit = 160 * 1024;

template <int T, int NL, int SE, bool FAST, bool LITERAL, bool BF, bool GT = false, bool MIR = false, int BLK = kBlock>
__global__ __launch_bounds__(BLK) void vi_fwd_kernel(
    QbDev c, const float4* __restrict__ g_tab, const float* __restrict__ packed,
    const float* __restrict__ x, const float* __restrict__ mask, const float* __restrict__ prior,
    int S, int K, uint64_t seed, int64_t voxel0, float* __restrict__ q_out,
    float2* __restrict__ nll_kl, double* __restrict__ partials, int64_t N) {
    constexpr EncLayout e = qb::make_enc_layout(T, 64, NL);
    static_assert(!GT || (FAST && SE >= 0 && qb::gtab_segs(T) > 0), "GT needs the fast path with a compile-time spin echo");
    static_assert(!MIR || (FAST && SE >= 0), "merged mirror pairs: fast path with a compile-time spin echo");
    constexpr bool kMir = GT || MIR;
    using Lds = typename ViLds<T, SE, GT>::type;
    extern __shared__ __align__(16) unsigned char smem[];
    float* lds_w = reinterpret_cast<float*>(smem);
    Lds* L = reinterpret_cast<Lds*>(smem + sizeof(float) * e.total);
    double* red = reinterpret_cast<double*>(smem + sizeof(float) * e.total + sizeof(Lds));
    constexpr int kWaves = BLK / 64;
    qb::copy_to_lds<BLK>(lds_w, packed, e.total / 4);
    if constexpr (qb::IsGtLds<Lds>::value) {
        qb::gt_lds_fill(L, g_tab, c);
    } else {
        qb::fwd_lds_fill(L, g_tab, true);
        if (threadIdx.x < QB_MAX_T) L->blood_B[threadIdx.x] = c.blood_B[threadIdx.x];
    }
    __syncthreads();

    constexpr int HT = (5 + T + 15) / 16;
    const int lane0 = threadIdx.x & 63, wave = threadIdx.x >> 6;
    float s_nll = 0.0f, s_kl = 0.0f, s_m = 0.0f;
    const int64_t ntile = (N + 15) / 16;
    for (int64_t tile = (int64_t)blockIdx.x * kWaves + wave; tile < ntile;
         tile += (int64_t)gridDim.x * kWaves) {
        int lane = lane0;
        asm volatile("" : "+v"(lane));
        const int g = lane >> 4, i = lane & 15;
        const int64_t v = tile * 16 + i;
        const int64_t vc = v < N ? v : N - 1;
        float o[5 + T];
        float amax = lds_w[e.flag];
        {
            __builtin_amdgcn_s_setprio(QB_PRIO_TILE_START);
            float xv[T], nv[T];
#pragma unroll
            for (int t = 0; t < T; ++t) xv[t] = x[vc * T + t];
            qb::normalise<T, SE>(c, xv, nv);
            __builtin_amdgcn_s_setprio(2);
            f32x4 b[4];
            qb::dense_first<T, BF>(lds_w + e.first_A, lds_w + e.first_b, nv, b, lane);
            if (!QB_ABLATE(c, 1) && qb_phase_fence()) {
                qb::block_stream2<BF, true>(lds_w + e.blk0, b, lane, &amax);
#pragma unroll
                for (int l = 1; l < NL; ++l) qb::block_stream2<BF>(lds_w + e.blk0 + l * e.blk_stride, b, lane, &amax);
            }
            f32x4 hd[HT];
            qb::dense_head<HT, BF>(lds_w + e.head_A, lds_w + e.head_b, b, hd, lane, &amax);
            qb::gather_head<5 + T, HT>(hd, o);
            __builtin_amdgcn_s_setprio(0);
        }
        if (v < N && !QB_ABLATE(c, 2) && qb_phase_fence()) {
            const float* xr = x + v * T;
            asm volatile("" : "+v"(xr));
            float xv[T], sv[T], qv[5];
#pragma unroll
            for (int t = 0; t < T; ++t) xv[t] = xr[t];
#pragma unroll
            for (int k = 0; k < 5; ++k) qv[k] = o[k];
#pragma unroll
            for (int t = 0; t < T; ++t) sv[t] = o[5 + t];
            qb::VoxelLik<T> lik;
            qb::prepare_lik<T, SE, true, (FAST && SE >= 0), FAST, kMir>(c, xv, sv, FAST ? 1.0f : (mask ? mask[v] : 1.0f), lik);
            const qb::LogitMvn qm = qb::make_mvn(qv);
            if (g == 1 && q_out) {
#pragma unroll
                for (int k = 0; k < 5; ++k) q_out[v * 5 + k] = qv[k];
            }
            if (!BF && qb::split_overflowed(amax)) lik.log_s_sum = __builtin_nanf("");
            float nll_part, kl_part;
            qb::voxel_mc_sums<T, SE, FAST, LITERAL, kMir>(L, c, lik, qm, prior + v * 5, S, K, nullptr, nullptr, seed,
                                                    (uint64_t)(voxel0 + v), g, nll_part, kl_part);
            const float nll = qb::voxel_sum(nll_part) / (float)S;
            const float kl = K > 0 ? qb::voxel_sum(kl_part) / (float)K : 0.0f;
            if (g == 0) {
                const float* mp = mask;
                asm volatile("" : "+v"(mp));
                const float m = mp ? mp[v] : 1.0f;
                if (nll_kl) nll_kl[v] = make_float2(nll, kl);
                s_nll += nll * m;
                s_kl += m > 0.0f ? kl : 0.0f;
                s_m += m;
            }
        }
    }
    qb::block_partials(red, s_nll, s_kl, s_m, partials);
}

}

namespace {
inline int64_t align256(int64_t b) { return (b + 255) & ~(int64_t)255; }
bool wide_vi_path(const qbold_ctx* ctx, const qbold_encoder_shape* shape) {
    return qb::wide_fused_supported(shape) && ctx && shape->T == ctx->dev.T && qb::elbo_logsigma_path(ctx);
}
}

extern "C" int64_t qbold_vi_workspace_bytes(const qbold_ctx* ctx, const qbold_encoder_shape* shape, int64_t N) {
    if (!ctx || !shape || N < 0) return QBOLD_ERR_INVALID;
    const int64_t part = align256(qbold_elbo_workspace_bytes(ctx));
    if (!wide_vi_path(ctx, shape)) return part;
    return part + align256(N * (int64_t)shape->T * 4) + align256(N * 5 * 4);
}

extern "C" int qbold_vi_fwd(const qbold_ctx* ctx, const qbold_encoder_shape* shape,
                            const float* packed, const float* x, const float* mask,
                            const float* prior, int S, int K, uint64_t seed, int64_t voxel0,
                            float* q_out, float* nll_kl, double* sums, void* workspace, int64_t N,
                            void* stream) {
    QB_NEED_DEVICE(ctx);
    QB_RELU_ONLY(shape, "qbold_vi_fwd");
    if (wide_vi_path(ctx, shape)) {
        QB_REQUIRE(N >= 0 && S >= 1 && K >= 0, "qbold_vi_fwd: need N >= 0, S >= 1, K >= 0");
        QB_REQUIRE(sums && workspace, "qbold_vi_fwd: null sums/workspace");
        QB_REQUIRE(N == 0 || (packed && x && prior), "qbold_vi_fwd: null input buffer");
        QB_REQUIRE(reinterpret_cast<uintptr_t>(workspace) % 256 == 0 && reinterpret_cast<uintptr_t>(packed) % 16 == 0 &&
                       reinterpret_cast<uintptr_t>(x) % 16 == 0,
                   "qbold_vi_fwd: wide shapes need a 256-byte aligned workspace of qbold_vi_workspace_bytes() and "
                   "16-byte aligned packed / x");
        char* w = reinterpret_cast<char*>(workspace);
        float* ls = reinterpret_cast<float*>(w + align256(qbold_elbo_workspace_bytes(ctx)));
        float* qbuf = q_out ? q_out : reinterpret_cast<float*>(reinterpret_cast<char*>(ls) + align256(N * (int64_t)shape->T * 4));
        if (N > 0) {
            const int rc = qb::wide_fused_fwd(ctx, shape, packed, x, qbuf, ls, N, (hipStream_t)stream);
            if (rc) return rc;
        }
        return qb::elbo_fwd_launch(ctx, x, mask, qbuf, prior, ls, true, nullptr, nullptr, S, K, seed, voxel0, nll_kl,
                                   sums, workspace, N, (hipStream_t)stream);
    }
    int rc = qb::check_encoder_shape(ctx, shape);
    if (rc) return rc;
    QB_REQUIRE(N >= 0 && S >= 1 && K >= 0, "qbold_vi_fwd: need N >= 0, S >= 1, K >= 0");
    QB_REQUIRE(sums && workspace, "qbold_vi_fwd: null sums/workspace");
    QB_REQUIRE(N == 0 || (packed && x && prior), "qbold_vi_fwd: null input buffer");
    hipStream_t s = (hipStream_t)stream;
    double* partials = reinterpret_cast<double*>(workspace);
    const int64_t ntile = (N + 15) / 16;
    const int blk = shape->T == 24 ? QB_VI_BLOCK_24 : kBlock, waves = blk / 64;
    const int64_t nblk = (ntile + waves - 1) / waves;
    const int grid = (int)(nblk < ctx->num_cus ? (nblk > 0 ? nblk : 1) : ctx->num_cus);
    const bool lit = ctx->dev.tissue_mode == QBOLD_TISSUE_LITERAL;
    float2* out = reinterpret_cast<float2*>(nll_kl);
    const bool bf = shape->precision == QBOLD_ENC_BF16;
    QB_REQUIRE(!bf || qb::elbo_fast_path(ctx),
               "qbold_vi_fwd: QBOLD_ENC_BF16 needs the table-mode Gaussian fast path");
#define QB_LAUNCH_VI(TT, NL, SE, FAST, LIT) QB_LAUNCH_VI_GT(TT, NL, SE, FAST, LIT, false, false)
#define QB_LAUNCH_VI_GT(TT, NL, SE, FAST, LIT, GT, MIR)                                              \
    do {                                                                                          \
        using LdsT = typename ViLds<TT, SE, GT>::type;                                             \
        constexpr size_t smem = sizeof(float) * qb::make_enc_layout(TT, 64, NL).total + sizeof(LdsT) + \
                                sizeof(double) * 3 * (kBlock / 64);                                \
        static_assert(smem <= kLdsLimit, "weight image + sampling table exceed the LDS");          \
        const float4* tab = qb::IsGtLds<LdsT>::value ? ctx->d_gtab : ctx->d_tab;                    \
        constexpr int BLKT = TT == 24 ? QB_VI_BLOCK_24 : kBlock;                                   \
        auto k = vi_fwd_kernel<TT, NL, SE, FAST, LIT, false, GT, MIR, BLKT>;                       \
        if constexpr (FAST) { if (bf) k = vi_fwd_kernel<TT, NL, SE, FAST, LIT, true, GT, MIR, BLKT>; }   \
        QB_HIP(hipFuncSetAttribute(reinterpret_cast<const void*>(k),                              \
                                   hipFuncAttributeMaxDynamicSharedMemorySize, (int)smem));       \
        hipLaunchKernelGGL(k, dim3(grid), dim3(BLKT), smem, s, ctx->dev, tab, packed,              \
                           x, mask, prior, S, K, seed, voxel0, q_out, out, partials, N);          \
    } while (0)
    const bool fast = qb::elbo_fast_path(ctx);
#define QB_DISPATCH_VI(TT, NL, SEC)                                               \
    do {                                                                          \
        if (qb::gtab_segs(TT) > 0 && fast && ctx->dev.se_idx == SEC && !ctx->dev.multi_norm && !(ctx->kernel_sel & 4) && ctx->gtab_ok && !(ctx->kernel_sel & 8)) QB_LAUNCH_VI_GT(TT, NL, SEC, true, false, (qb::gtab_segs(TT) > 0), false);   \
        else if (fast && ctx->dev.se_idx == SEC && !ctx->dev.multi_norm && !(ctx->kernel_sel & 4) && ctx->grid_mirrors) QB_LAUNCH_VI_GT(TT, NL, SEC, true, false, false, true);   \
        else if (fast && ctx->dev.se_idx == SEC && !ctx->dev.multi_norm && !(ctx->kernel_sel & 4)) QB_LAUNCH_VI(TT, NL, SEC, true, false);   \
        else if (fast) QB_LAUNCH_VI(TT, NL, -1, true, false);                     \
        else if (lit && ctx->dev.se_idx == SEC && !ctx->dev.multi_norm) QB_LAUNCH_VI(TT, NL, SEC, false, true);   \
        else if (lit) QB_LAUNCH_VI(TT, NL, -1, false, true);                      \
        else QB_LAUNCH_VI(TT, NL, -1, false, false);                              \
    } while (0)
#ifdef QB_VI_PROBE
    if (shape->T == 11 && shape->L == 2) QB_DISPATCH_VI(11, 2, 2);
    else if (shape->T == 24 && shape->L == 2) QB_DISPATCH_VI(24, 2, 7);
#else
    if (shape->T == 11 && shape->L == 1) QB_DISPATCH_VI(11, 1, 2);
    else if (shape->T == 11 && shape->L == 2) QB_DISPATCH_VI(11, 2, 2);
    else if (shape->T == 24 && shape->L == 1) QB_DISPATCH_VI(24, 1, 7);
    else if (shape->T == 24 && shape->L == 2) QB_DISPATCH_VI(24, 2, 7);
#endif
    else {
        qb::set_error("qbold_vi_fwd: kernels are built for T = 11 or 24 taus, L = 1 or 2");
        return QBOLD_ERR_UNSUPPORTED;
    }
#undef QB_DISPATCH_VI
#undef QB_LAUNCH_VI
#undef QB_LAUNCH_VI_GT
    QB_HIP(hipGetLastError());
    hipLaunchKernelGGL(qb::reduce_partials_kernel, dim3(1), dim3(192), 0, s, partials, grid, sums);
    QB_HIP(hipGetLastError());
    return QBOLD_OK;
}
```

Before: 2.532 billion voxel-ELBO evals/s.

## Fuse final partial reduction into main kernels via last-block atomic ticket

```diff
diff --git a/include/qbold_hip.h b/include/qbold_hip.h
--- a/include/qbold_hip.h
+++ b/include/qbold_hip.h
@@ -179,6 +179,7 @@
                            float snr_lo, float snr_hi, uint64_t seed, int64_t voxel0,
                            void* workspace, int64_t V, void* stream);
 
+#define QBOLD_TICKET_RING_SLOTS 256
 int64_t qbold_elbo_workspace_bytes(const qbold_ctx* ctx);
 
 int qbold_elbo_fwd(const qbold_ctx* ctx, const float* x, const float* mask, const float* q,
diff --git a/qbold_vi_amd/csrc/ctx.hip b/qbold_vi_amd/csrc/ctx.hip
--- a/qbold_vi_amd/csrc/ctx.hip
+++ b/qbold_vi_amd/csrc/ctx.hip
@@ -260,6 +260,10 @@
         if (e == hipSuccess)
             e = hipMemcpy(ctx->d_gtab, ctx->h_gtab.data(), sizeof(float) * ctx->h_gtab.size(), hipMemcpyHostToDevice);
     }
+    if (e == hipSuccess) e = hipMalloc((void**)&ctx->d_tickets, sizeof(unsigned) * QB_TICKET_STRIDE * QB_TICKET_SLOTS);
+    if (e == hipSuccess)
+        e = hipMemset(ctx->d_tickets, 0, sizeof(unsigned) * QB_TICKET_STRIDE * QB_TICKET_SLOTS);
+    if (e == hipSuccess) e = hipDeviceSynchronize();
     if (e == hipSuccess) {
         hipDeviceProp_t prop;
         if (hipGetDeviceProperties(&prop, device) == hipSuccess && prop.multiProcessorCount > 0)
@@ -269,6 +273,7 @@
     if (e != hipSuccess) {
         if (ctx->d_tab) (void)hipFree(ctx->d_tab);
         if (ctx->d_gtab) (void)hipFree(ctx->d_gtab);
+        if (ctx->d_tickets) (void)hipFree(ctx->d_tickets);
         delete ctx;
         return qb::hip_fail(e, "qbold_ctx_create: device setup");
     }
@@ -280,6 +285,7 @@
     if (!ctx) return;
     if (ctx->d_tab) (void)hipFree(ctx->d_tab);
     if (ctx->d_gtab) (void)hipFree(ctx->d_gtab);
+    if (ctx->d_tickets) (void)hipFree(ctx->d_tickets);
     delete ctx;
 }
 
diff --git a/qbold_vi_amd/csrc/elbo_bwd_kernels.hip b/qbold_vi_amd/csrc/elbo_bwd_kernels.hip
--- a/qbold_vi_amd/csrc/elbo_bwd_kernels.hip
+++ b/qbold_vi_amd/csrc/elbo_bwd_kernels.hip
@@ -46,7 +46,7 @@
     const float* __restrict__ mask, const float* __restrict__ q, const float* __restrict__ prior,
     const float* __restrict__ log_sigma, int S, int K, uint64_t seed, int64_t voxel0,
     float* __restrict__ g_q, float* __restrict__ g_ls, float2* __restrict__ nll_kl,
-    double* __restrict__ partials, int64_t N) {
+    double* __restrict__ partials, int64_t N, unsigned* ticket, double* sums) {
     __shared__ qb::FwdLds L;
     __shared__ double red[3 * (kBlock / 64)];
     qb::fwd_lds_fill(&L, g_tab, false);
@@ -267,7 +267,7 @@
             }
         }
     }
-    qb::block_partials(red, s_nll, s_kl, s_m, partials);
+    qb::block_partials_finish(red, s_nll, s_kl, s_m, partials, ticket, sums);
 }
 
 constexpr int kGenBlock = 128;
@@ -299,7 +299,7 @@
     const float* __restrict__ mask, const float* __restrict__ q, const float* __restrict__ prior,
     const float* __restrict__ log_sigma, int S, int K, int kl_per_wave, uint64_t seed, int64_t voxel0,
     float* __restrict__ g_q, float* __restrict__ g_ls, float2* __restrict__ nll_kl,
-    double* __restrict__ partials, int64_t N) {
+    double* __restrict__ partials, int64_t N, unsigned* ticket, double* sums) {
     extern __shared__ __align__(16) unsigned char smem[];
     qb::FwdLds* L = reinterpret_cast<qb::FwdLds*>(smem);
     __shared__ double red[3 * (kGenBlock / 64)];
@@ -527,7 +527,7 @@
             }
         }
     }
-    qb::block_partials(red, s_nll, s_kl, s_m, partials);
+    qb::block_partials_finish(red, s_nll, s_kl, s_m, partials, ticket, sums);
 }
 
 }
@@ -548,6 +548,7 @@
     }
     hipStream_t s = (hipStream_t)stream;
     double* partials = reinterpret_cast<double*>(workspace);
+    unsigned* ticket = qb::next_ticket(ctx);
     const int lpv = S <= 2 ? 1 : QB_LANES_PER_VOXEL;
     const int vpb = kBlock / lpv;
     const int64_t ntile = (N + vpb - 1) / vpb;
@@ -571,9 +572,7 @@
             QB_HIP(hipFuncSetAttribute(reinterpret_cast<const void*>(kern), hipFuncAttributeMaxDynamicSharedMemorySize,
                                        (int)smem));
         hipLaunchKernelGGL(kern, dim3(ggrid), dim3(kGenBlock), smem, s, ctx->dev, ctx->d_tab, x, mask, q, prior, log_sigma,
-                           S, K, spec_T ? 1 : 0, seed, voxel0, g_q, g_log_sigma, out, partials, N);
-        QB_HIP(hipGetLastError());
-        hipLaunchKernelGGL(qb::reduce_partials_kernel, dim3(1), dim3(192), 0, s, partials, ggrid, sums);
+                           S, K, spec_T ? 1 : 0, seed, voxel0, g_q, g_log_sigma, out, partials, N, ticket, sums);
         QB_HIP(hipGetLastError());
         return QBOLD_OK;
     }
@@ -581,11 +580,11 @@
     do {                                                                                                                \
         if (lpv == 1)                                                                                                   \
             hipLaunchKernelGGL((elbo_bwd_kernel<TT, SEC, 1>), dim3(grid), dim3(kBlock), 0, s, ctx->dev, ctx->d_tab, x,   \
-                               mask, q, prior, log_sigma, S, K, seed, voxel0, g_q, g_log_sigma, out, partials, N);      \
+                               mask, q, prior, log_sigma, S, K, seed, voxel0, g_q, g_log_sigma, out, partials, N, ticket, sums);      \
         else                                                                                                            \
             hipLaunchKernelGGL((elbo_bwd_kernel<TT, SEC, QB_LANES_PER_VOXEL>), dim3(grid), dim3(kBlock), 0, s, ctx->dev, \
                                ctx->d_tab, x, mask, q, prior, log_sigma, S, K, seed, voxel0, g_q, g_log_sigma, out,     \
-                               partials, N);                                                                            \
+                               partials, N, ticket, sums);                                                                            \
     } while (0)
     if (ctx->dev.T == 24) {
         QB_LAUNCH_BWD(24, -1);
@@ -599,7 +598,5 @@
     }
 #undef QB_LAUNCH_BWD
     QB_HIP(hipGetLastError());
-    hipLaunchKernelGGL(qb::reduce_partials_kernel, dim3(1), dim3(192), 0, s, partials, grid, sums);
-    QB_HIP(hipGetLastError());
     return QBOLD_OK;
 }
diff --git a/qbold_vi_amd/csrc/elbo_core.h b/qbold_vi_amd/csrc/elbo_core.h
--- a/qbold_vi_amd/csrc/elbo_core.h
+++ b/qbold_vi_amd/csrc/elbo_core.h
@@ -478,19 +478,58 @@
     }
 }
 
-static __global__ void reduce_partials_kernel(const double* __restrict__ partials, int nblocks,
-                                       double* __restrict__ sums) {
-    __shared__ double sh[192];
-    const int k = threadIdx.x / 64, lane = threadIdx.x & 63;
-    double a = 0.0;
-    for (int b = lane; b < nblocks; b += 64) a += partials[3 * b + k];
-    sh[threadIdx.x] = a;
+__device__ __forceinline__ void partials_finish(double* red, double* partials, unsigned* ticket, double* sums) {
+    if (threadIdx.x < 3) {
+        __builtin_amdgcn_fence(__ATOMIC_RELEASE, "agent");
+        asm volatile("s_waitcnt vmcnt(0)" ::: "memory");
+    }
     __syncthreads();
-    if (lane == 0) {
-        double t = 0.0;
-        for (int i = 0; i < 64; ++i) t += sh[64 * k + i];
-        sums[k] = t;
-    }
-}
-
-}
+    int* flag = reinterpret_cast<int*>(red);
+    if (threadIdx.x == 0) {
+        const unsigned t = __hip_atomic_fetch_add(ticket, 1u, __ATOMIC_RELAXED, __HIP_MEMORY_SCOPE_AGENT);
+        const bool last = t == gridDim.x - 1;
+        if (last) {
+            __builtin_amdgcn_fence(__ATOMIC_ACQUIRE, "agent");
+            __hip_atomic_store(ticket, 0u, __ATOMIC_RELAXED, __HIP_MEMORY_SCOPE_AGENT);
+            asm volatile("s_waitcnt vmcnt(0)" ::: "memory");
+        }
+        *flag = last ? 1 : 0;
+    }
+    __syncthreads();
+    if (*flag) {
+        const int lane = threadIdx.x & 63, nw = blockDim.x >> 6, nblocks = (int)gridDim.x;
+        for (int k = threadIdx.x >> 6; k < 3; k += nw) {
+            double a = 0.0;
+            for (int b0 = lane; b0 < nblocks; b0 += 256) {
+                double v[4];
+#pragma unroll
+                for (int j = 0; j < 4; ++j) {
+                    const int b = b0 + 64 * j;
+                    v[j] = b < nblocks ? __hip_atomic_load(partials + 3 * b + k, __ATOMIC_RELAXED, __HIP_MEMORY_SCOPE_AGENT)
+                                       : 0.0;
+                }
+#pragma unroll
+                for (int j = 0; j < 4; ++j)
+                    if (b0 + 64 * j < nblocks) a += v[j];
+            }
+            const unsigned long long bits = __builtin_bit_cast(unsigned long long, a);
+            const int lo = (int)(unsigned)bits, hi = (int)(unsigned)(bits >> 32);
+            double t = 0.0;
+#pragma unroll 1
+            for (int i = 0; i < 64; ++i) {
+                const unsigned l = (unsigned)__builtin_amdgcn_readlane(lo, i), h = (unsigned)__builtin_amdgcn_readlane(hi, i);
+                t += __builtin_bit_cast(double, ((unsigned long long)h << 32) | l);
+            }
+            if (lane == 0) sums[k] = t;
+        }
+    }
+}
+
+__device__ __forceinline__ void block_partials_finish(double* red, float s_nll, float s_kl, float s_m,
+                                                      double* __restrict__ partials, unsigned* ticket,
+                                                      double* sums) {
+    block_partials(red, s_nll, s_kl, s_m, partials);
+    partials_finish(red, partials, ticket, sums);
+}
+
+}
diff --git a/qbold_vi_amd/csrc/elbo_kernels.hip b/qbold_vi_amd/csrc/elbo_kernels.hip
--- a/qbold_vi_amd/csrc/elbo_kernels.hip
+++ b/qbold_vi_amd/csrc/elbo_kernels.hip
@@ -19,7 +19,7 @@
     const float* __restrict__ mask, const float* __restrict__ q, const float* __restrict__ prior,
     const float* __restrict__ sigma, const float* __restrict__ zs, const float* __restrict__ zk,
     int S, int K, uint64_t seed, int64_t voxel0, float2* __restrict__ nll_kl,
-    double* __restrict__ partials, int64_t N) {
+    double* __restrict__ partials, int64_t N, unsigned* ticket, double* sums) {
     static_assert(!GT || (FAST && SE >= 0 && qb::gtab_segs(T) > 0), "GT needs the fast path with a compile-time spin echo");
     static_assert(!MIR || (FAST && SE >= 0), "merged mirror pairs: fast path with a compile-time spin echo");
     constexpr bool kMir = GT || MIR;
@@ -67,7 +67,7 @@
             }
         }
     }
-    qb::block_partials(red, s_nll, s_kl, s_m, partials);
+    qb::block_partials_finish(red, s_nll, s_kl, s_m, partials, ticket, sums);
 }
 
 constexpr int kGenBlock = 128;
@@ -102,7 +102,7 @@
     const float* __restrict__ mask, const float* __restrict__ q, const float* __restrict__ prior,
     const float* __restrict__ sigma, const float* __restrict__ zs, const float* __restrict__ zk,
     int S, int K, uint64_t seed, int64_t voxel0, float2* __restrict__ nll_kl,
-    double* __restrict__ partials, int64_t N) {
+    double* __restrict__ partials, int64_t N, unsigned* ticket, double* sums) {
     extern __shared__ __align__(16) unsigned char smem[];
     qb::FwdLds* L = reinterpret_cast<qb::FwdLds*>(smem);
     float* yt = reinterpret_cast<float*>(smem + sizeof(qb::FwdLds));
@@ -222,6 +222,7 @@
         }
     }
     block_partials_d(red, s_nll, s_kl, s_m, partials);
+    qb::partials_finish(red, partials, ticket, sums);
 }
 
 #ifndef QB_LDS_PIPE
@@ -239,7 +240,7 @@
     const float* __restrict__ mask, const float* __restrict__ q, const float* __restrict__ prior,
     const float* __restrict__ sigma, const float* __restrict__ zs, const float* __restrict__ zk,
     int S, int K, uint64_t seed, int64_t voxel0, float2* __restrict__ nll_kl,
-    double* __restrict__ partials, int64_t N) {
+    double* __restrict__ partials, int64_t N, unsigned* ticket, double* sums) {
     static_assert(T % 16 == 0 && SE >= 0 && SE < T, "a lane owns T / 4 taus as float4 loads");
     __shared__ qb::FwdLds L;
     __shared__ float2 dat[T * kLdsVox];
@@ -411,7 +412,7 @@
             }
         }
     }
-    qb::block_partials(red, s_nll, s_kl, s_m, partials);
+    qb::block_partials_finish(red, s_nll, s_kl, s_m, partials, ticket, sums);
 }
 
 constexpr int kGtBlock = 1024;
@@ -422,7 +423,7 @@
     QbDev c, const float4* __restrict__ g_gtab, const float* __restrict__ x,
     const float* __restrict__ mask, const float* __restrict__ q, const float* __restrict__ prior,
     const float* __restrict__ sigma, int S, int K, uint64_t seed, int64_t voxel0, float2* __restrict__ nll_kl,
-    double* __restrict__ partials, int64_t N) {
+    double* __restrict__ partials, int64_t N, unsigned* ticket, double* sums) {
     static_assert(T == 64 && SE == 12, "lane ownership of the taus below is written out for the 64-tau protocol");
     constexpr int NSEG = qb::gtab_segs(T), J = qb::gtab_taus(T, SE), NROW = T - SE;
     static_assert(J == NROW - 1 && NSEG > 0, "one table row set per evaluated tau above the spin echo");
@@ -596,7 +597,7 @@
             }
         }
     }
-    qb::block_partials(red, s_nll, s_kl, s_m, partials);
+    qb::block_partials_finish(red, s_nll, s_kl, s_m, partials, ticket, sums);
 }
 
 __global__ void reparam_kernel(const float* __restrict__ q, const float2* __restrict__ z,
@@ -800,6 +801,7 @@
                     const float* zk, int S, int K, uint64_t seed, int64_t voxel0, float* nll_kl,
                     double* sums, void* workspace, int64_t N, hipStream_t s) {
     double* partials = reinterpret_cast<double*>(workspace);
+    unsigned* ticket = qb::next_ticket(ctx);
     const int64_t ntile = (N + kVoxPerBlock - 1) / kVoxPerBlock;
     int grid = (int)(ntile < qb::elbo_grid(ctx) ? (ntile > 0 ? ntile : 1) : qb::elbo_grid(ctx));
     const bool lit = ctx->dev.tissue_mode == QBOLD_TISSUE_LITERAL;
@@ -807,15 +809,15 @@
 #define QB_LAUNCH_ELBO(TT, SE, FAST, LIT)                                                        \
     hipLaunchKernelGGL((elbo_fwd_kernel<TT, SE, FAST, LIT>), dim3(grid), dim3(kBlock), 0, s,      \
                        ctx->dev, ctx->d_tab, x, mask, q, prior, sigma, zs, zk, S, K, seed, voxel0, \
-                       out, partials, N)
+                       out, partials, N, ticket, sums)
 #define QB_LAUNCH_ELBO_MIR(TT, SE)                                                               \
     hipLaunchKernelGGL((elbo_fwd_kernel<TT, SE, true, false, false, true>), dim3(grid), dim3(kBlock), 0, s, \
                        ctx->dev, ctx->d_tab, x, mask, q, prior, sigma, zs, zk, S, K, seed, voxel0, \
-                       out, partials, N)
+                       out, partials, N, ticket, sums)
 #define QB_LAUNCH_ELBO_GT(TT, SE)                                                                \
     hipLaunchKernelGGL((elbo_fwd_kernel<TT, SE, true, false, (qb::gtab_segs(TT) > 0)>), dim3(grid), dim3(kBlock), 0, s, \
                        ctx->dev, ctx->d_gtab, x, mask, q, prior, sigma, zs, zk, S, K, seed, voxel0, \
-                       out, partials, N)
+                       out, partials, N, ticket, sums)
     const bool gt = ctx->gtab_ok && !(ctx->kernel_sel & 8) && qb::gtab_segs(ctx->dev.T) > 0;
     const bool fast = qb::elbo_fast_path(ctx);
     const bool lds64 = qb::elbo_logsigma_path(ctx);
@@ -837,9 +839,7 @@
             QB_HIP(hipFuncSetAttribute(reinterpret_cast<const void*>(kern), hipFuncAttributeMaxDynamicSharedMemorySize,
                                        (int)smem));
             hipLaunchKernelGGL(kern, dim3(grid), dim3(kGtBlock), smem, s, ctx->dev, ctx->d_gtab, x, mask, q, prior, sigma,
-                               S, K, seed, voxel0, out, partials, N);
-            QB_HIP(hipGetLastError());
-            hipLaunchKernelGGL(qb::reduce_partials_kernel, dim3(1), dim3(192), 0, s, partials, grid, sums);
+                               S, K, seed, voxel0, out, partials, N, ticket, sums);
             QB_HIP(hipGetLastError());
             return QBOLD_OK;
         }
@@ -847,10 +847,10 @@
         grid = (int)(gt < qb::elbo_grid(ctx) ? (gt > 0 ? gt : 1) : qb::elbo_grid(ctx));
         if (sigma_is_log)
             hipLaunchKernelGGL((elbo_fwd_lds_kernel<64, 12, true>), dim3(grid), dim3(kLdsBlock), 0, s, ctx->dev,
-                               ctx->d_tab, x, mask, q, prior, sigma, zs, zk, S, K, seed, voxel0, out, partials, N);
+                               ctx->d_tab, x, mask, q, prior, sigma, zs, zk, S, K, seed, voxel0, out, partials, N, ticket, sums);
         else
             hipLaunchKernelGGL((elbo_fwd_lds_kernel<64, 12, false>), dim3(grid), dim3(kLdsBlock), 0, s, ctx->dev,
-                               ctx->d_tab, x, mask, q, prior, sigma, zs, zk, S, K, seed, voxel0, out, partials, N);
+                               ctx->d_tab, x, mask, q, prior, sigma, zs, zk, S, K, seed, voxel0, out, partials, N, ticket, sums);
     } else switch (ctx->dev.T) {
         case 11:
             if (fast && ctx->dev.se_idx == 2 && !ctx->dev.multi_norm && gt) QB_LAUNCH_ELBO_GT(11, 2);
@@ -881,14 +881,12 @@
             const size_t smem = sizeof(qb::FwdLds) + sizeof(float) * 2 * QB_MAX_T * kGenVox;
             hipLaunchKernelGGL(elbo_fwd_generic_kernel, dim3(grid), dim3(kGenBlock), smem, s, ctx->dev,
                                ctx->d_tab, x, mask, q, prior, sigma, zs, zk, S, K, seed, voxel0, out,
-                               partials, N);
+                               partials, N, ticket, sums);
         }
     }
 #undef QB_LAUNCH_ELBO
 #undef QB_LAUNCH_ELBO_MIR
 #undef QB_LAUNCH_ELBO_GT
-    QB_HIP(hipGetLastError());
-    hipLaunchKernelGGL(qb::reduce_partials_kernel, dim3(1), dim3(192), 0, s, partials, grid, sums);
     QB_HIP(hipGetLastError());
     return QBOLD_OK;
 }
@@ -921,7 +919,7 @@
 __global__ __launch_bounds__(256) void kl_diag_kernel(const float* __restrict__ q, const float* __restrict__ prior,
                                                       const float* __restrict__ mask, float* __restrict__ kl_v,
                                                       float* __restrict__ g_q, double* __restrict__ partials,
-                                                      int64_t N) {
+                                                      int64_t N, unsigned* ticket, double* sums) {
     __shared__ double red[3 * 4];
     float s_kl = 0.0f, s_m = 0.0f;
     for (int64_t v = blockIdx.x * (int64_t)blockDim.x + threadIdx.x; v < N;
@@ -951,7 +949,7 @@
             g_q[v * 5 + 3] += ed * 3.0f * (1.0f - td * td);
         }
     }
-    qb::block_partials(red, 0.0f, s_kl, s_m, partials);
+    qb::block_partials_finish(red, 0.0f, s_kl, s_m, partials, ticket, sums);
 }
 
 extern "C" int qbold_kl_diag(const qbold_ctx* ctx, const float* q, const float* prior, const float* mask,
@@ -964,9 +962,8 @@
     double* partials = reinterpret_cast<double*>(workspace);
     const int64_t nb = (N + 255) / 256;
     const int grid = (int)(nb < qb::elbo_grid(ctx) ? (nb > 0 ? nb : 1) : qb::elbo_grid(ctx));
-    hipLaunchKernelGGL(kl_diag_kernel, dim3(grid), dim3(256), 0, s, q, prior, mask, kl_v, g_q, partials, N);
-    QB_HIP(hipGetLastError());
-    hipLaunchKernelGGL(qb::reduce_partials_kernel, dim3(1), dim3(192), 0, s, partials, grid, sums);
+    hipLaunchKernelGGL(kl_diag_kernel, dim3(grid), dim3(256), 0, s, q, prior, mask, kl_v, g_q, partials, N,
+                       qb::next_ticket(ctx), sums);
     QB_HIP(hipGetLastError());
     return QBOLD_OK;
 }
diff --git a/qbold_vi_amd/csrc/grid_kernels.hip b/qbold_vi_amd/csrc/grid_kernels.hip
--- a/qbold_vi_amd/csrc/grid_kernels.hip
+++ b/qbold_vi_amd/csrc/grid_kernels.hip
@@ -459,7 +459,7 @@
 __global__ __launch_bounds__(kBlock) void grid_kernel(
     QbDev c, const float4* __restrict__ g_tab, const float* __restrict__ x, const float* __restrict__ mask,
     const float* __restrict__ prior, const float* __restrict__ sigma, const float* __restrict__ q, GridArgs ga,
-    GhRule gh, float* __restrict__ out, float* __restrict__ box, double* __restrict__ partials, int64_t N) {
+    GhRule gh, float* __restrict__ out, float* __restrict__ box, double* __restrict__ partials, int64_t N, unsigned* ticket, double* sums) {
     static_assert(!GT || (FAST && SE >= 0 && qb::gtab_segs(T) > 0), "GT needs the fast path with a compile-time spin echo");
     static_assert(!MIR || (FAST && SE >= 0), "merged mirror pairs: fast path with a compile-time spin echo");
     constexpr bool kMir = GT || MIR;
@@ -501,6 +501,7 @@
         store_voxel(o, live, v, m, out, box, s_lp, s_el, s_m);
     }
     block_partials_d(red, s_lp, s_el, s_m, partials);
+    qb::partials_finish(red, partials, ticket, sums);
 }
 
 struct GenEval {
@@ -556,7 +557,7 @@
 __global__ __launch_bounds__(kBlock) void grid_generic_kernel(
     QbDev c, const float4* __restrict__ g_tab, const float* __restrict__ x, const float* __restrict__ mask,
     const float* __restrict__ prior, const float* __restrict__ sigma, const float* __restrict__ q, GridArgs ga,
-    GhRule gh, float* __restrict__ out, float* __restrict__ box, double* __restrict__ partials, int64_t N) {
+    GhRule gh, float* __restrict__ out, float* __restrict__ box, double* __restrict__ partials, int64_t N, unsigned* ticket, double* sums) {
     __shared__ qb::FwdLds L;
     __shared__ float rows[kWaves][2][kMaxN];
     __shared__ float yts[kWaves][2][QB_MAX_T];
@@ -601,6 +602,7 @@
         store_voxel(o, live, v, m, out, box, s_lp, s_el, s_m);
     }
     block_partials_d(red, s_lp, s_el, s_m, partials);
+    qb::partials_finish(red, partials, ticket, sums);
 }
 
 void gauss_hermite(int n, GhRule& r) {
@@ -677,17 +679,18 @@
     if (q && cfg->gh > 0) gauss_hermite(cfg->gh, gh);
     hipStream_t s = (hipStream_t)stream;
     double* partials = reinterpret_cast<double*>(workspace);
+    unsigned* ticket = qb::next_ticket(ctx);
     const int64_t nblk = (N + kWaves - 1) / kWaves;
     const int grid = (int)(nblk < qb::elbo_grid(ctx) ? (nblk > 0 ? nblk : 1) : qb::elbo_grid(ctx));
     const bool gt = ctx->gtab_ok && !(ctx->kernel_sel & 8) && qb::gtab_segs(T) > 0;
-#define QB_GRID_ARGS ctx->dev, ctx->d_tab, x, mask, prior, sigma, q, ga, gh, out, box, partials, N
+#define QB_GRID_ARGS ctx->dev, ctx->d_tab, x, mask, prior, sigma, q, ga, gh, out, box, partials, N, ticket, sums
 #define QB_LAUNCH_GRID(TT, SE, FAST, LIT) \
     hipLaunchKernelGGL((grid_kernel<TT, SE, FAST, LIT>), dim3(grid), dim3(kBlock), 0, s, QB_GRID_ARGS)
 #define QB_LAUNCH_GRID_MIR(TT, SE) \
     hipLaunchKernelGGL((grid_kernel<TT, SE, true, false, false, true>), dim3(grid), dim3(kBlock), 0, s, QB_GRID_ARGS)
 #define QB_LAUNCH_GRID_GT(TT, SE)                                                                                    \
     hipLaunchKernelGGL((grid_kernel<TT, SE, true, false, (qb::gtab_segs(TT) > 0)>), dim3(grid), dim3(kBlock), 0, s, \
-                       ctx->dev, ctx->d_gtab, x, mask, prior, sigma, q, ga, gh, out, box, partials, N)
+                       ctx->dev, ctx->d_gtab, x, mask, prior, sigma, q, ga, gh, out, box, partials, N, ticket, sums)
     switch (T) {
         case 11:
             if (fast && ctx->dev.se_idx == 2 && !ctx->dev.multi_norm && gt) QB_LAUNCH_GRID_GT(11, 2);
@@ -715,7 +718,5 @@
 #undef QB_LAUNCH_GRID_GT
 #undef QB_GRID_ARGS
     QB_HIP(hipGetLastError());
-    hipLaunchKernelGGL(qb::reduce_partials_kernel, dim3(1), dim3(192), 0, s, partials, grid, sums);
-    QB_HIP(hipGetLastError());
     return QBOLD_OK;
 }
diff --git a/qbold_vi_amd/csrc/iw_bwd_kernels.hip b/qbold_vi_amd/csrc/iw_bwd_kernels.hip
--- a/qbold_vi_amd/csrc/iw_bwd_kernels.hip
+++ b/qbold_vi_amd/csrc/iw_bwd_kernels.hip
@@ -194,7 +194,7 @@
     QbDev c, const float4* __restrict__ g_tab, const float* __restrict__ x, const float* __restrict__ mask,
     const float* __restrict__ q, const float* __restrict__ prior, const float* __restrict__ log_sigma,
     const float* __restrict__ z, int K, uint64_t seed, int64_t voxel0, float* __restrict__ g_q,
-    float* __restrict__ g_ls, float* __restrict__ out, double* __restrict__ partials, int64_t N) {
+    float* __restrict__ g_ls, float* __restrict__ out, double* __restrict__ partials, int64_t N, unsigned* ticket, double* sums) {
     __shared__ qb::FwdLds L;
     __shared__ double red[3 * (kBlock / 64)];
     qb::fwd_lds_fill(&L, g_tab, false);
@@ -303,6 +303,7 @@
         }
     }
     block_partials_d(red, s_lp, s_el, s_m, partials);
+    qb::partials_finish(red, partials, ticket, sums);
 }
 
 }
@@ -328,6 +329,7 @@
     }
     hipStream_t s = (hipStream_t)stream;
     double* partials = reinterpret_cast<double*>(workspace);
+    unsigned* ticket = qb::next_ticket(ctx);
     const int lpv = K <= QB_IW_BWD_LPV1_MAX_K ? 1 : QB_LANES_PER_VOXEL;
     const int vpb = kBlock / lpv;
     const int64_t ntile = (N + vpb - 1) / vpb;
@@ -336,11 +338,11 @@
     do {                                                                                                             \
         if (lpv == 1)                                                                                                \
             hipLaunchKernelGGL((iw_bwd_kernel<TT, SEC, 1>), dim3(grid), dim3(kBlock), 0, s, ctx->dev, ctx->d_tab, x,  \
-                               mask, q, prior, log_sigma, z, K, seed, voxel0, g_q, g_log_sigma, out, partials, N);   \
+                               mask, q, prior, log_sigma, z, K, seed, voxel0, g_q, g_log_sigma, out, partials, N, ticket, sums);   \
         else                                                                                                         \
             hipLaunchKernelGGL((iw_bwd_kernel<TT, SEC, QB_LANES_PER_VOXEL>), dim3(grid), dim3(kBlock), 0, s,         \
                                ctx->dev, ctx->d_tab, x, mask, q, prior, log_sigma, z, K, seed, voxel0, g_q,          \
-                               g_log_sigma, out, partials, N);                                                       \
+                               g_log_sigma, out, partials, N, ticket, sums);                                                       \
     } while (0)
     if (ctx->dev.T == 24) {
         QB_LAUNCH_IWB(24, -1);
@@ -351,7 +353,5 @@
     }
 #undef QB_LAUNCH_IWB
     QB_HIP(hipGetLastError());
-    hipLaunchKernelGGL(qb::reduce_partials_kernel, dim3(1), dim3(192), 0, s, partials, grid, sums);
-    QB_HIP(hipGetLastError());
     return QBOLD_OK;
 }
diff --git a/qbold_vi_amd/csrc/iw_kernels.hip b/qbold_vi_amd/csrc/iw_kernels.hip
--- a/qbold_vi_amd/csrc/iw_kernels.hip
+++ b/qbold_vi_amd/csrc/iw_kernels.hip
@@ -180,7 +180,7 @@
     QbDev c, const float4* __restrict__ g_tab, const float* __restrict__ x, const float* __restrict__ mask,
     const float* __restrict__ q, const float* __restrict__ prior, const float* __restrict__ sigma,
     const float* __restrict__ z, int K, uint64_t seed, int64_t voxel0, float* __restrict__ out,
-    float* __restrict__ is_means, double* __restrict__ partials, int64_t N) {
+    float* __restrict__ is_means, double* __restrict__ partials, int64_t N, unsigned* ticket, double* sums) {
     static_assert(!GT || (FAST && SE >= 0 && qb::gtab_segs(T) > 0), "GT needs the fast path with a compile-time spin echo");
     static_assert(!MIR || (FAST && SE >= 0), "merged mirror pairs: fast path with a compile-time spin echo");
     constexpr bool kMir = GT || MIR;
@@ -233,6 +233,7 @@
         }
     }
     block_partials_d(red, s_lp, s_el, s_m, partials);
+    qb::partials_finish(red, partials, ticket, sums);
 }
 
 constexpr int kGenBlock = 128;
@@ -282,7 +283,7 @@
     QbDev c, const float4* __restrict__ g_tab, const float* __restrict__ x, const float* __restrict__ mask,
     const float* __restrict__ q, const float* __restrict__ prior, const float* __restrict__ sigma,
     const float* __restrict__ z, int K, uint64_t seed, int64_t voxel0, float* __restrict__ out,
-    float* __restrict__ is_means, double* __restrict__ partials, int64_t N) {
+    float* __restrict__ is_means, double* __restrict__ partials, int64_t N, unsigned* ticket, double* sums) {
     extern __shared__ __align__(16) unsigned char smem[];
     qb::FwdLds* L = reinterpret_cast<qb::FwdLds*>(smem);
     float* yt = reinterpret_cast<float*>(smem + sizeof(qb::FwdLds));
@@ -361,6 +362,7 @@
         }
     }
     block_partials_d(red, s_lp, s_el, s_m, partials);
+    qb::partials_finish(red, partials, ticket, sums);
 }
 
 }
@@ -376,6 +378,7 @@
     QB_REQUIRE(N == 0 || (x && q && prior && sigma), "qbold_log_evidence_fwd: null input buffer");
     hipStream_t s = (hipStream_t)stream;
     double* partials = reinterpret_cast<double*>(workspace);
+    unsigned* ticket = qb::next_ticket(ctx);
     const int64_t ntile = (N + kVoxPerBlock - 1) / kVoxPerBlock;
     int grid = (int)(ntile < qb::elbo_grid(ctx) ? (ntile > 0 ? ntile : 1) : qb::elbo_grid(ctx));
     const bool lit = ctx->dev.tissue_mode == QBOLD_TISSUE_LITERAL;
@@ -383,14 +386,14 @@
     const bool gt = ctx->gtab_ok && !(ctx->kernel_sel & 8) && qb::gtab_segs(ctx->dev.T) > 0;
 #define QB_LAUNCH_IW(TT, SE, FAST, LIT)                                                                            \
     hipLaunchKernelGGL((iw_fwd_kernel<TT, SE, FAST, LIT>), dim3(grid), dim3(kBlock), 0, s, ctx->dev, ctx->d_tab, x, \
-                       mask, q, prior, sigma, z, K, seed, voxel0, out, is_means, partials, N)
+                       mask, q, prior, sigma, z, K, seed, voxel0, out, is_means, partials, N, ticket, sums)
 #define QB_LAUNCH_IW_MIR(TT, SE)                                                                                    \
     hipLaunchKernelGGL((iw_fwd_kernel<TT, SE, true, false, false, true>), dim3(grid), dim3(kBlock), 0, s, ctx->dev, \
-                       ctx->d_tab, x, mask, q, prior, sigma, z, K, seed, voxel0, out, is_means, partials, N)
+                       ctx->d_tab, x, mask, q, prior, sigma, z, K, seed, voxel0, out, is_means, partials, N, ticket, sums)
 #define QB_LAUNCH_IW_GT(TT, SE)                                                                                     \
     hipLaunchKernelGGL((iw_fwd_kernel<TT, SE, true, false, (qb::gtab_segs(TT) > 0)>), dim3(grid), dim3(kBlock), 0, \
                        s, ctx->dev, ctx->d_gtab, x, mask, q, prior, sigma, z, K, seed, voxel0, out, is_means,       \
-                       partials, N)
+                       partials, N, ticket, sums)
     switch (ctx->dev.T) {
         case 11:
             if (fast && ctx->dev.se_idx == 2 && !ctx->dev.multi_norm && gt) QB_LAUNCH_IW_GT(11, 2);
@@ -420,14 +423,12 @@
             grid = (int)(gtile < qb::elbo_grid(ctx) ? (gtile > 0 ? gtile : 1) : qb::elbo_grid(ctx));
             const size_t smem = sizeof(qb::FwdLds) + sizeof(float) * 2 * QB_MAX_T * kGenVox;
             hipLaunchKernelGGL(iw_fwd_generic_kernel, dim3(grid), dim3(kGenBlock), smem, s, ctx->dev, ctx->d_tab, x,
-                               mask, q, prior, sigma, z, K, seed, voxel0, out, is_means, partials, N);
+                               mask, q, prior, sigma, z, K, seed, voxel0, out, is_means, partials, N, ticket, sums);
         }
     }
 #undef QB_LAUNCH_IW
 #undef QB_LAUNCH_IW_MIR
 #undef QB_LAUNCH_IW_GT
-    QB_HIP(hipGetLastError());
-    hipLaunchKernelGGL(qb::reduce_partials_kernel, dim3(1), dim3(192), 0, s, partials, grid, sums);
     QB_HIP(hipGetLastError());
     return QBOLD_OK;
 }
diff --git a/qbold_vi_amd/csrc/qbold_ctx.h b/qbold_vi_amd/csrc/qbold_ctx.h
--- a/qbold_vi_amd/csrc/qbold_ctx.h
+++ b/qbold_vi_amd/csrc/qbold_ctx.h
@@ -2,6 +2,7 @@
 
 #include <hip/hip_runtime.h>
 
+#include <atomic>
 #include <string>
 #include <vector>
 
@@ -22,11 +23,20 @@
     int num_cus = 256;
     float dF_node0_ref = 0.0f;
     int kernel_sel = 0;
+    mutable unsigned* d_tickets = nullptr;
+    mutable std::atomic<unsigned> ticket_cursor{0};
 };
+
+#define QB_TICKET_SLOTS QBOLD_TICKET_RING_SLOTS
+#define QB_TICKET_STRIDE 16
 
 namespace qb {
 void set_error(const std::string& msg);
 int hip_fail(hipError_t e, const char* what);
+inline unsigned* next_ticket(const qbold_ctx* ctx) {
+    const unsigned i = ctx->ticket_cursor.fetch_add(1u, std::memory_order_relaxed) % QB_TICKET_SLOTS;
+    return ctx->d_tickets + (size_t)QB_TICKET_STRIDE * i;
+}
 }
 
 #define QB_HIP(call)                                              \
diff --git a/qbold_vi_amd/csrc/vi_kernels.hip b/qbold_vi_amd/csrc/vi_kernels.hip
--- a/qbold_vi_amd/csrc/vi_kernels.hip
+++ b/qbold_vi_amd/csrc/vi_kernels.hip
@@ -40,7 +40,7 @@
     QbDev c, const float4* __restrict__ g_tab, const float* __restrict__ packed,
     const float* __restrict__ x, const float* __restrict__ mask, const float* __restrict__ prior,
     int S, int K, uint64_t seed, int64_t voxel0, float* __restrict__ q_out,
-    float2* __restrict__ nll_kl, double* __restrict__ partials, int64_t N) {
+    float2* __restrict__ nll_kl, double* __restrict__ partials, int64_t N, unsigned* ticket, double* sums) {
     constexpr EncLayout e = qb::make_enc_layout(T, 64, NL);
     static_assert(!GT || (FAST && SE >= 0 && qb::gtab_segs(T) > 0), "GT needs the fast path with a compile-time spin echo");
     static_assert(!MIR || (FAST && SE >= 0), "merged mirror pairs: fast path with a compile-time spin echo");
@@ -126,7 +126,7 @@
             }
         }
     }
-    qb::block_partials(red, s_nll, s_kl, s_m, partials);
+    qb::block_partials_finish(red, s_nll, s_kl, s_m, partials, ticket, sums);
 }
 
 }
@@ -200,7 +200,8 @@
         QB_HIP(hipFuncSetAttribute(reinterpret_cast<const void*>(k),                              \
                                    hipFuncAttributeMaxDynamicSharedMemorySize, (int)smem));       \
         hipLaunchKernelGGL(k, dim3(grid), dim3(BLKT), smem, s, ctx->dev, tab, packed,              \
-                           x, mask, prior, S, K, seed, voxel0, q_out, out, partials, N);          \
+                           x, mask, prior, S, K, seed, voxel0, q_out, out, partials, N,           \
+                           qb::next_ticket(ctx), sums);                                           \
     } while (0)
     const bool fast = qb::elbo_fast_path(ctx);
 #define QB_DISPATCH_VI(TT, NL, SEC)                                               \
@@ -230,7 +231,5 @@
 #undef QB_LAUNCH_VI
 #undef QB_LAUNCH_VI_GT
     QB_HIP(hipGetLastError());
-    hipLaunchKernelGGL(qb::reduce_partials_kernel, dim3(1), dim3(192), 0, s, partials, grid, sums);
-    QB_HIP(hipGetLastError());
     return QBOLD_OK;
 }
```

Result: no change. 2.527 billion voxel-ELBO evals/s (-0.2%).
